# facebookresearch/vsc2022

Measured on AMD Instinct MI355X. Metric: query-videos localized/sec @ 512-d SSCD, higher is better.
Workload: dtype fp32 results; int8 / fp16 MFMA pre-filters; 1 GPU; BASELINE configs[3]: full pipeline incl. score normalisation + TN localisation, 40000 query videos split over 1 GPU(s), 2000000 reference + 2000000 noise frames; query_videos_per_gpu=40000, query_frames_per_gpu=1000000, ref_frames=2000000, dim=512, global_k=48000000, candidates=1000000, pairs_localized=200000, matches=446939, hits=48000000, score_normalisation_in_step=True, parallelism=single GPU

## Files before the change

### vsc2022_amd/csrc/api.hip

```cpp
#include "api_internal.h"

namespace vscmi {

static thread_local std::string g_err;
void set_error(const char* fmt, ...) {
    char buf[1024];
    va_list ap;
    va_start(ap, fmt);
    vsnprintf(buf, sizeof(buf), fmt, ap);
    va_end(ap);
    g_err = buf;
}

bool poison_mode() {
    static const bool on = [] {
        const char* e = getenv("VSC_POISON_ALLOC");
        return e && e[0] == '1';
    }();
    return on;
}

int check_device(int device) {
    int n = 0;
    if (hipGetDeviceCount(&n) != hipSuccess || n <= 0) {
        set_error("no HIP device visible (libvscmi needs an MI355X / gfx950 GPU)");
        return VSC_ERR_NODEVICE;
    }
    if (device < 0 || device >= n) {
        set_error("device %d out of range (have %d)", device, n);
        return VSC_ERR_INVALID;
    }
    hipDeviceProp_t p;
    VSC_HIP(hipGetDeviceProperties(&p, device));
    if (strncmp(p.gcnArchName, "gfx950", 6) != 0) {
        set_error("device %d is %s; libvscmi is built for gfx950 only", device, p.gcnArchName);
        return VSC_ERR_NODEVICE;
    }
    return VSC_OK;
}


int pack_half_any(const float* x, int64_t n, int dim, const HalfImage& h, int64_t r0, int64_t rows_out,
                         hipStream_t stream) {
    if (h.frag)
        return launch_pack_half_frag(x, n, dim, h.rows, h.norms + r0, h.row0 + r0, rows_out, h.dpadh, stream);
    return launch_pack_half(x, n, dim, h.rows + r0 * h.dpadh, h.norms + r0, rows_out, h.dpadh, stream);
}

int pack_into(const float* x, int64_t n, int dim, int mem, float* dst, int64_t rows_out, int dpad,
                     Workspace& ws, hipStream_t stream, const HalfImage& h) {
    if (mem == VSC_MEM_DEVICE || n == 0) {
        VSC_TRY(launch_pack_rows(x, n, dim, dst, rows_out, dpad, stream));
        if (h.rows) VSC_TRY(pack_half_any(x, n, dim, h, 0, h.rows_out, stream));
        return VSC_OK;
    }
    const int64_t chunk_rows = std::max<int64_t>(1, (int64_t)(256ll << 20) / ((int64_t)dim * 4));
    VSC_TRY(ws.stage.reserve((size_t)std::min(chunk_rows, n) * dim * 4));
    for (int64_t r0 = 0; r0 < n; r0 += chunk_rows) {
        const int64_t rows = std::min(chunk_rows, n - r0);
        VSC_HIP(hipMemcpyAsync(ws.stage.p, x + r0 * dim, (size_t)rows * dim * 4, hipMemcpyHostToDevice, stream));
        const bool last = (r0 + rows == n);
        const int64_t out_rows = last ? rows_out - r0 : rows;
        VSC_TRY(launch_pack_rows(ws.stage.as<float>(), rows, dim, dst + r0 * dpad, out_rows, dpad, stream));
        if (h.rows) VSC_TRY(pack_half_any(ws.stage.as<float>(), rows, dim, h, r0, last ? h.rows_out - r0 : rows, stream));
        VSC_HIP(hipStreamSynchronize(stream));
    }
    return VSC_OK;
}

}

int prof_begin(vsc_index* idx, hipEvent_t* stop_out, int cls) {
    *stop_out = nullptr;
    if (!idx->prof) return VSC_OK;
    if (idx->ev_used == idx->ev_pool.size()) {
        hipEvent_t a, b;
        VSC_HIP(hipEventCreate(&a));
        VSC_HIP(hipEventCreate(&b));
        idx->ev_pool.emplace_back(a, b);
        idx->ev_class.push_back(0);
    }
    idx->ev_class[idx->ev_used] = cls;
    auto& e = idx->ev_pool[idx->ev_used++];
    VSC_HIP(hipEventRecord(e.first, idx->stream));
    *stop_out = e.second;
    return VSC_OK;
}
int prof_end(vsc_index* idx, hipEvent_t stop, double work, int cls) {
    if (!stop) return VSC_OK;
    VSC_HIP(hipEventRecord(stop, idx->stream));
    idx->pending_work[cls] += work;
    return VSC_OK;
}
int prof_collect(vsc_index* idx) {
    for (size_t e = 0; e < idx->ev_used; ++e) {
        float ms = 0.0f;
        VSC_HIP(hipEventElapsedTime(&ms, idx->ev_pool[e].first, idx->ev_pool[e].second));
        idx->prof_ms[idx->ev_class[e]] += ms;
        idx->prof_launches[idx->ev_class[e]] += 1;
    }
    for (int c = 0; c < 7; ++c) {
        idx->prof_work[c] += idx->pending_work[c];
        idx->pending_work[c] = 0.0;
    }
    idx->ev_used = 0;
    return VSC_OK;
}


AuxProf g_aux;

struct OptionName { const char* name; const char* env; };
static const OptionName kOptions[] = {
    {"prefilter", "VSC_PREFILTER"}, {"prefilter_density", "VSC_PREFILTER_DENSITY"}, {"f16_kernel", "VSC_F16_KERNEL"},
    {"i8", "VSC_I8"}, {"i8_density", "VSC_I8_DENSITY"}, {"i8_max_rel", "VSC_I8_MAX_REL"}, {"i8_exclude", "VSC_I8_EXCLUDE"},
    {"i8_sort", "VSC_I8_SORT"}, {"i8_center", "VSC_I8_CENTER"}, {"i8_group", "VSC_I8_GROUP"}, {"i8p_order", "VSC_I8P_ORDER"}, {"i8p_slice", "VSC_I8P_SLICE"},
    {"i8p_pair", "VSC_I8P_PAIR"}, {"i8_screen", "VSC_I8_SCREEN"}, {"i8_knn", "VSC_I8_KNN"}, {"knn_step", "VSC_KNN_STEP"},
    {"knn_step_max", "VSC_KNN_STEP_MAX"}, {"knn_step_work", "VSC_KNN_STEP_WORK"}, {"rescore_sort", "VSC_RESCORE_SORT"},
    {"knn_levels", "VSC_KNN_LEVELS"}, {"knn_subset", "VSC_KNN_SUBSET"}, {"knn_s0div", "VSC_KNN_S0DIV"},
    {"knn_s0min", "VSC_KNN_S0MIN"}, {"knn_ratio", "VSC_KNN_RATIO"}, {"knn_nchunk", "VSC_KNN_NCHUNK"}, {"knn_first_tile", "VSC_KNN_FIRST_TILE"},
    {"cand_budget", "VSC_CAND_BUDGET"}, {"debug_i8", "VSC_DEBUG_I8"}, {"debug_screen", "VSC_DEBUG_SCREEN"},
    {"topk_shortcut", "VSC_TOPK_SHORTCUT"}, {"topk_sample", "VSC_TOPK_SAMPLE"}, {"sort_hits", "VSC_SORT_HITS"}, {"density_hint", "VSC_DENSITY_HINT"},
};

static int option_needs_empty(const vsc_index* idx, const char* name) {
    if (idx->ntotal == 0) return VSC_OK;
    set_error("vsc_index_set_option: '%s' decides which images of the reference rows exist and can only be set while "
              "the index is empty", name);
    return VSC_ERR_INVALID;
}

static int apply_option(vsc_index* idx, const char* name, double v) {
    auto is = [&](const char* n) { return strcmp(name, n) == 0; };
    const bool ip = idx->metric == VSC_METRIC_INNER_PRODUCT;
    if (is("prefilter")) {
        const int m = (int)v;
        if (m < 0 || m > 2) goto bad;
        if ((m != 0) != idx->prefilter) VSC_TRY(option_needs_empty(idx, name));
        idx->prefilter = ip && m != 0;
        idx->prefilter_force = idx->prefilter && m == 2;
        if (!idx->prefilter) idx->i8_mode = 0;
        return VSC_OK;
    }
    if (is("i8")) {
        const int m = (int)v;
        if (m < 0 || m > 2) goto bad;
        const int want = (idx->prefilter && idx->dpad8 <= I8P_MAX_DPAD8) ? m : 0;
        if ((want != 0) != (idx->i8_mode != 0)) VSC_TRY(option_needs_empty(idx, name));
        idx->i8_mode = want;
        return VSC_OK;
    }
    if (is("f16_kernel")) {
        const bool frag = !(v != 0.0) && idx->dpadh <= F16P_MAX_DPADH;
        if (frag != idx->frag) VSC_TRY(option_needs_empty(idx, name));
        idx->frag = frag;
        return VSC_OK;
    }
    if (is("i8_exclude")) {
        const bool e = v != 0.0;
        if (e != idx->i8_exclude) VSC_TRY(option_needs_empty(idx, name));
        idx->i8_exclude = e;
        return VSC_OK;
    }
    if (is("i8_center")) {
        const int m = (int)v;
        if (m < 0 || m > 2) goto bad;
        if (m != idx->i8_center) VSC_TRY(option_needs_empty(idx, name));
        idx->i8_center = m;
        return VSC_OK;
    }
    if (is("prefilter_density")) { if (!(v > 0.0)) goto bad; idx->prefilter_density = v; return VSC_OK; }
    if (is("i8_density")) { if (!(v > 0.0)) goto bad; idx->i8_density = v; return VSC_OK; }
    if (is("i8_max_rel")) { if (!(v > 0.0)) goto bad; idx->i8_max_rel = v; return VSC_OK; }
    if (is("i8_sort")) { idx->i8_sort_rows = v != 0.0; return VSC_OK; }
    if (is("i8_group")) { idx->i8_group_shift = std::max(0, std::min(16, (int)v)); return VSC_OK; }
    if (is("i8p_order")) { idx->i8p_order = (int)v == 1 ? 1 : 0; return VSC_OK; }
    if (is("i8p_slice")) { if (v < 0.0) goto bad; idx->i8p_slice = (int)v; return VSC_OK; }
    if (is("i8p_pair")) { idx->i8p_pair = std::max(0, std::min(2, (int)v)); return VSC_OK; }
    if (is("i8_screen")) { idx->i8_screen = v == 1.0; return VSC_OK; }
    if (is("i8_knn")) { idx->knn_i8 = v != 0.0; return VSC_OK; }
    if (is("knn_step")) { idx->knn_step = std::max<int64_t>(0, (int64_t)v) / 256 * 256; return VSC_OK; }
    if (is("knn_step_max")) { idx->knn_step_max = std::max<int64_t>(32768, (int64_t)v); return VSC_OK; }
    if (is("knn_step_work")) { idx->knn_step_work = std::max(0.0, v); return VSC_OK; }
    if (is("rescore_sort")) { idx->rescore_by_ref = v != 0.0; return VSC_OK; }
    if (is("knn_levels")) { idx->knn_two_level = v != 1.0; return VSC_OK; }
    if (is("knn_subset")) { if (!(v > 0.0)) goto bad; idx->knn_subset_factor = v; return VSC_OK; }
    if (is("knn_s0div")) { idx->knn_s0_div = v > 0.0 ? (int)v : 28; return VSC_OK; }
    if (is("knn_s0min")) { idx->knn_s0_min = v >= 64.0 ? (int)v : 1024; return VSC_OK; }
    if (is("knn_ratio")) { idx->knn_ratio = v; return VSC_OK; }
    if (is("knn_nchunk")) { idx->knn_nchunk = (int)v; return VSC_OK; }
    if (is("knn_first_tile")) { idx->knn_first_tile = v != 0.0; return VSC_OK; }
    if (is("cand_budget")) { if (!(v >= 1048576.0)) goto bad; idx->cand_budget = (int64_t)v; return VSC_OK; }
    if (is("debug_i8")) { idx->debug_i8 = v != 0.0; return VSC_OK; }
    if (is("debug_screen")) { idx->debug_screen = v != 0.0; return VSC_OK; }
    if (is("topk_shortcut")) { const int m = (int)v; if (m < 0 || m > 2) goto bad; idx->topk_shortcut = m; return VSC_OK; }
    if (is("topk_sample")) { if (!(v >= 2.0)) goto bad; idx->topk_sample_rows = (int64_t)v; return VSC_OK; }
    if (is("sort_hits")) { idx->sort_hits = v != 0.0; return VSC_OK; }
    if (is("density_hint")) { if (!(v >= 0.0)) goto bad; idx->density_hint = v; return VSC_OK; }
    set_error("vsc_index_set_option: unknown option '%s'", name);
    return VSC_ERR_INVALID;
bad:
    set_error("vsc_index_set_option: value %g is out of range for '%s'", v, name);
    return VSC_ERR_INVALID;
}

static int read_option(const vsc_index* idx, const char* name, double* out) {
    auto is = [&](const char* n) { return strcmp(name, n) == 0; };
    if (is("prefilter")) *out = idx->prefilter ? (idx->prefilter_force ? 2 : 1) : 0;
    else if (is("i8")) *out = idx->i8_mode;
    else if (is("f16_kernel")) *out = idx->frag ? 0 : 1;
    else if (is("i8_exclude")) *out = idx->i8_exclude;
    else if (is("prefilter_density")) *out = idx->prefilter_density;
    else if (is("i8_density")) *out = idx->i8_density;
    else if (is("i8_max_rel")) *out = idx->i8_max_rel;
    else if (is("i8_sort")) *out = idx->i8_sort_rows;
    else if (is("i8_group")) *out = idx->i8_group_shift;
    else if (is("i8p_order")) *out = idx->i8p_order;
    else if (is("i8p_slice")) *out = idx->i8p_slice;
    else if (is("i8p_pair")) *out = idx->i8p_pair;
    else if (is("i8_screen")) *out = idx->i8_screen;
    else if (is("i8_knn")) *out = idx->knn_i8;
    else if (is("knn_step")) *out = (double)idx->knn_step;
    else if (is("knn_step_max")) *out = (double)idx->knn_step_max;
    else if (is("knn_step_work")) *out = idx->knn_step_work;
    else if (is("rescore_sort")) *out = idx->rescore_by_ref;
    else if (is("knn_levels")) *out = idx->knn_two_level ? 0 : 1;
    else if (is("knn_subset")) *out = idx->knn_subset_factor;
    else if (is("knn_s0div")) *out = idx->knn_s0_div;
    else if (is("knn_s0min")) *out = idx->knn_s0_min;
    else if (is("knn_ratio")) *out = idx->knn_ratio;
    else if (is("knn_nchunk")) *out = idx->knn_nchunk;
    else if (is("knn_first_tile")) *out = idx->knn_first_tile;
    else if (is("cand_budget")) *out = (double)idx->cand_budget;
    else if (is("debug_i8")) *out = idx->debug_i8;
    else if (is("debug_screen")) *out = idx->debug_screen;
    else if (is("topk_shortcut")) *out = idx->topk_shortcut;
    else if (is("topk_sample")) *out = (double)idx->topk_sample_rows;
    else if (is("sort_hits")) *out = idx->sort_hits;
    else if (is("density_hint")) *out = idx->density_hint;
    else if (is("last_topk_route")) *out = idx->last_topk_route;
    else if (is("i8_center")) *out = idx->i8_center;
    else if (is("i8_center_on")) *out = idx->i8_mu_on;
    else if (is("i8_center_share")) *out = idx->i8_mu_ratio;
    else if (is("i8_fallbacks")) *out = (double)idx->stat_i8_fallbacks;
    else if (is("codec")) *out = idx->codec;
    else if (is("ref_bytes")) *out = (double)(idx->ref.bytes + idx->refh.bytes + idx->refn.bytes + idx->ref8.bytes + idx->ref8m.bytes);
    else {
        set_error("vsc_index_get_option: unknown option '%s'", name);
        return VSC_ERR_INVALID;
    }
    return VSC_OK;
}

extern "C" {

int vsc_aux_profile(int enable) {
    g_aux.on = enable != 0;
    return VSC_OK;
}
int vsc_aux_profile_read(int cls, double* ms, int64_t* calls, double* bytes, int reset) {
    if (cls < 0 || cls >= AUX_CLASSES) return VSC_ERR_INVALID;
    std::lock_guard<std::mutex> lk(g_aux.mu);
    if (ms) *ms = g_aux.ms[cls];
    if (calls) *calls = g_aux.n[cls];
    if (bytes) *bytes = g_aux.bytes[cls];
    if (reset) { g_aux.ms[cls] = 0.0; g_aux.bytes[cls] = 0.0; g_aux.n[cls] = 0; }
    return VSC_OK;
}

const char* vsc_last_error(void) { return g_err.c_str(); }
int vsc_version(void) { return 100; }

int vsc_device_count(void) {
    int n = 0;
    if (hipGetDeviceCount(&n) != hipSuccess) return 0;
    int ok = 0;
    for (int d = 0; d < n; ++d) {
        hipDeviceProp_t p;
        if (hipGetDeviceProperties(&p, d) == hipSuccess && strncmp(p.gcnArchName, "gfx950", 6) == 0) ++ok;
    }
    return ok;
}

int vsc_index_create(int dim, int metric, int device, vsc_index_t** out) {
    return vsc_index_create_codec(dim, metric, device, VSC_CODEC_FLAT, out);
}

int vsc_index_create_codec(int dim, int metric, int device, int codec, vsc_index_t** out) {
    if (!out || dim <= 0 || (metric != VSC_METRIC_INNER_PRODUCT && metric != VSC_METRIC_L2) ||
        (codec != VSC_CODEC_FLAT && codec != VSC_CODEC_SQFP16)) {
        set_error("vsc_index_create: invalid argument (dim=%d metric=%d codec=%d)", dim, metric, codec);
        return VSC_ERR_INVALID;
    }
    VSC_TRY(check_device(device));
    VSC_HIP(hipSetDevice(device));
    vsc_index* idx = new vsc_index();
    idx->dim = dim;
    idx->codec = codec;
    idx->dpad = round_up(dim, K_PAD);
    idx->dpadh = round_up(dim, 128);
    idx->frag = idx->dpadh <= F16P_MAX_DPADH;
    idx->metric = metric;
    idx->dpad8 = round_up(dim, 256);
    idx->prefilter = metric == VSC_METRIC_INNER_PRODUCT;
    idx->i8_mode = (idx->prefilter && idx->dpad8 <= I8P_MAX_DPAD8) ? 1 : 0;
    for (const OptionName& o : kOptions) {
        const char* v = getenv(o.env);
        if (!v || !v[0]) continue;
        double x = atof(v);
        if (strcmp(o.name, "f16_kernel") == 0) x = v[0] == 'r' ? 1.0 : 0.0;
        if (strcmp(o.name, "debug_i8") == 0 || strcmp(o.name, "debug_screen") == 0) x = 1.0;
        (void)apply_option(idx, o.name, x);
    }
    idx->device = device;
    hipError_t e = hipStreamCreateWithFlags(&idx->own_stream, hipStreamNonBlocking);
    if (e != hipSuccess) {
        set_error("hipStreamCreate failed: %s", hipGetErrorString(e));
        delete idx;
        return VSC_ERR_HIP;
    }
    idx->stream = idx->own_stream;
    int rc = set_thresh_kernel_attrs();
    if (rc != VSC_OK) {
        (void)hipStreamDestroy(idx->own_stream);
        delete idx;
        return rc;
    }
    *out = idx;
    return VSC_OK;
}

int vsc_index_destroy(vsc_index_t* idx) {
    if (!idx) return VSC_OK;
    (void)hipSetDevice(idx->device);
    if (idx->stream == idx->own_stream) (void)hipStreamSynchronize(idx->own_stream);
    else (void)hipDeviceSynchronize();
    idx->ref.release();
    idx->refh.release();
    idx->refn.release();
    idx->ref8.release();
    idx->ref8m.release();
    idx->i8_mu.release();
    for (auto& b : idx->cand) b.release();
    idx->ws.release();
    for (auto& e : idx->ev_pool) {
        (void)hipEventDestroy(e.first);
        (void)hipEventDestroy(e.second);
    }
    (void)hipStreamDestroy(idx->own_stream);
    delete idx;
    return VSC_OK;
}

int vsc_index_set_stream(vsc_index_t* idx, void* hip_stream, int own) {
    if (!idx) {
        set_error("vsc_index_set_stream: invalid argument");
        return VSC_ERR_INVALID;
    }
    VSC_HIP(hipSetDevice(idx->device));
    if (idx->stream == idx->own_stream) VSC_HIP(hipStreamSynchronize(idx->own_stream));
    else (void)hipDeviceSynchronize();
    VSC_TRY(prof_collect(idx));
    idx->stream = own ? idx->own_stream : (hipStream_t)hip_stream;
    return VSC_OK;
}

int vsc_index_set_option(vsc_index_t* idx, const char* name, double value) {
    if (!idx || !name) {
        set_error("vsc_index_set_option: invalid argument");
        return VSC_ERR_INVALID;
    }
    return apply_option(idx, name, value);
}

int vsc_index_get_option(const vsc_index_t* idx, const char* name, double* value) {
    if (!idx || !name || !value) {
        set_error("vsc_index_get_option: invalid argument");
        return VSC_ERR_INVALID;
    }
    return read_option(idx, name, value);
}

int64_t vsc_index_ntotal(const vsc_index_t* idx) { return idx ? idx->ntotal : 0; }
int vsc_index_dim(const vsc_index_t* idx) { return idx ? idx->dim : 0; }
int vsc_index_metric(const vsc_index_t* idx) { return idx ? idx->metric : 0; }

int vsc_index_set_hit_capacity(vsc_index_t* idx, int64_t cap) {
    if (!idx || cap < 0) {
        set_error("vsc_index_set_hit_capacity: invalid argument");
        return VSC_ERR_INVALID;
    }
    idx->hit_cap_user = cap;
    return VSC_OK;
}

int vsc_index_sync(vsc_index_t* idx) {
    if (!idx) return VSC_ERR_INVALID;
    VSC_HIP(hipSetDevice(idx->device));
    VSC_HIP(hipStreamSynchronize(idx->stream));
    return VSC_OK;
}

}

int decode_range(vsc_index* idx, int64_t r0, int64_t rows, float** out) {
    const int64_t rows_out = round_up64(rows, ROW_PAD_REF) + ROW_PAD_REF;
    VSC_TRY(idx->ws.dec.reserve((size_t)rows_out * idx->dpad * sizeof(float)));
    VSC_TRY(launch_decode_rows(idx->refh.as<_Float16>(), idx->dpadh, idx->frag, r0, rows_out,
                               std::min(r0 + rows, round_up64(idx->ntotal, ROW_PAD_REF)), idx->ws.dec.as<float>(), idx->dpad, true,
                               idx->stream));
    *out = idx->ws.dec.as<float>();
    return VSC_OK;
}

int ref_range_count(const vsc_index* idx, int64_t, int64_t rows) {
    return sq16(idx) ? (int)((rows + DEC_CHUNK_ROWS - 1) / DEC_CHUNK_ROWS) : 1;
}
int for_ref_ranges(vsc_index* idx, int64_t r0, int64_t rows, const RefRangeFn& fn) {
    if (!sq16(idx)) return fn(idx->ref.as<float>() + r0 * idx->dpad, r0, rows);
    for (int64_t c0 = r0; c0 < r0 + rows; c0 += DEC_CHUNK_ROWS) {
        const int64_t rc = std::min(DEC_CHUNK_ROWS, r0 + rows - c0);
        float* dec = nullptr;
        VSC_TRY(decode_range(idx, c0, rc, &dec));
        VSC_TRY(fn(dec, c0, rc));
    }
    return VSC_OK;
}

static int i8_upload_centre(vsc_index* idx) {
    if (!idx->i8_mu_on) return VSC_OK;
    std::vector<float> eff(idx->i8_mu_host);
    for (int c = 0; c < idx->i8_ex.n; ++c) eff[(size_t)k_slot(idx->i8_ex.idx[c])] = 0.0f;
    VSC_TRY(idx->i8_mu.reserve((size_t)idx->dpad * sizeof(float)));
    VSC_HIP(hipMemcpyAsync(idx->i8_mu.p, eff.data(), (size_t)idx->dpad * sizeof(float), hipMemcpyHostToDevice, idx->stream));
    VSC_HIP(hipStreamSynchronize(idx->stream));
    idx->i8_mu_ex = idx->i8_ex;
    return VSC_OK;
}

static int i8_decide_centre(vsc_index* idx, int64_t rows) {
    idx->i8_mu_decided = true;
    idx->i8_mu_on = false;
    if (idx->i8_center == 0 || rows <= 0) return VSC_OK;
    const int dpad = idx->dpad;
    VSC_TRY(idx->ws.sort.tmp.reserve((size_t)2 * dpad * sizeof(double)));
    double* d_sum = idx->ws.sort.tmp.as<double>();
    std::vector<double> h((size_t)2 * dpad), part(h.size());
    VSC_TRY(for_ref_ranges(idx, 0, rows, [&](const float* src, int64_t first, int64_t n) -> int {
        std::vector<double>& dst = first == 0 ? h : part;
        VSC_TRY(launch_col_sums(src, n, dpad, d_sum, d_sum + dpad, idx->stream));
        VSC_HIP(hipMemcpyAsync(dst.data(), d_sum, dst.size() * sizeof(double), hipMemcpyDeviceToHost, idx->stream));
        VSC_HIP(hipStreamSynchronize(idx->stream));
        if (first > 0)
            for (size_t e = 0; e < h.size(); ++e) h[e] += part[e];
        return VSC_OK;
    }));
    idx->i8_mu_host.assign((size_t)dpad, 0.0f);
    double mu2 = 0.0, e2 = 0.0;
    bool finite = true;
    for (int k = 0; k < idx->dim; ++k) {
        if (idx->i8_ex.holds(k)) continue;
        const int p = k_slot(k);
        const double m = h[(size_t)p] / (double)rows;
        finite = finite && std::isfinite(m) && std::isfinite(h[(size_t)dpad + p]);
        idx->i8_mu_host[(size_t)p] = (float)m;
        mu2 += m * m;
        e2 += h[(size_t)dpad + p] / (double)rows;
    }
    idx->i8_mu_ratio = e2 > 0.0 ? mu2 / e2 : 0.0;
    if (!finite) return VSC_OK;
    idx->i8_mu_on = idx->i8_center == 2 || idx->i8_mu_ratio >= 0.02;
    if (idx->debug_i8)
        fprintf(stderr, "[vscmi] int8 reference image: mean carries %.4f of the rows' energy over %lld rows -> %s\n", idx->i8_mu_ratio,
                (long long)rows, idx->i8_mu_on ? "centred" : "not centred");
    return i8_upload_centre(idx);
}

static int i8_quantise(vsc_index* idx, int64_t row0, int64_t rows, int64_t count_rows) {
    if (rows <= 0) return VSC_OK;
    if (idx->i8_mu_on) {
        bool same = idx->i8_mu_ex.n == idx->i8_ex.n;
        for (int c = 0; same && c < idx->i8_ex.n; ++c) same = idx->i8_mu_ex.idx[c] == idx->i8_ex.idx[c];
        if (!same) VSC_TRY(i8_upload_centre(idx));
    }
    VSC_TRY(for_ref_ranges(idx, row0, rows, [&](const float* src, int64_t first, int64_t n) -> int {
        return launch_quant_ref_frag(src - first * idx->dpad, idx->dpad, idx->ref8.p, idx->ref8m.as<float4>(), first, n, idx->dpad8,
                                     idx->i8_ex, idx->i8_mu_on ? idx->i8_mu.as<float>() : nullptr, idx->stream);
    }));
    const int64_t real = std::max<int64_t>(0, std::min(row0 + rows, count_rows) - row0);
    VSC_TRY(idx->ws.cnt.reserve(2 * sizeof(double)));
    VSC_TRY(launch_meta_looseness(idx->ref8m.as<float4>() + row0, real, idx->ws.cnt.as<double>(), idx->stream));
    double h2[2] = {0.0, 0.0};
    VSC_HIP(hipMemcpyAsync(h2, idx->ws.cnt.p, sizeof(h2), hipMemcpyDeviceToHost, idx->stream));
    VSC_HIP(hipStreamSynchronize(idx->stream));
    idx->i8_loose_sum += h2[0];
    idx->i8_loose_cnt += h2[1];
    idx->i8_rows = std::max(idx->i8_rows, row0 + rows);
    return VSC_OK;
}

static int i8_after_add(vsc_index* idx, int64_t first_new, int64_t n, int64_t need_rows) {
    const int dpad = idx->dpad;
    VSC_TRY(idx->ws.sort.tmp.reserve((size_t)2 * dpad * sizeof(unsigned)));
    unsigned* d_mn = idx->ws.sort.tmp.as<unsigned>();
    unsigned* d_mx = d_mn + dpad;
    std::vector<unsigned> mn((size_t)dpad), mx((size_t)dpad), pmn((size_t)dpad), pmx((size_t)dpad);
    VSC_TRY(for_ref_ranges(idx, first_new, n, [&](const float* src, int64_t first, int64_t rows) -> int {
        const bool head = first == first_new;
        VSC_TRY(launch_dim_minmax(src, rows, dpad, d_mn, d_mx, idx->stream));
        VSC_HIP(hipMemcpyAsync((head ? mn : pmn).data(), d_mn, (size_t)dpad * sizeof(unsigned), hipMemcpyDeviceToHost, idx->stream));
        VSC_HIP(hipMemcpyAsync((head ? mx : pmx).data(), d_mx, (size_t)dpad * sizeof(unsigned), hipMemcpyDeviceToHost, idx->stream));
        VSC_HIP(hipStreamSynchronize(idx->stream));
        if (!head)
            for (int p = 0; p < dpad; ++p) {
                mn[(size_t)p] = std::min(mn[(size_t)p], pmn[(size_t)p]);
                mx[(size_t)p] = std::max(mx[(size_t)p], pmx[(size_t)p]);
            }
        return VSC_OK;
    }));
    if (idx->cmin_key.empty()) {
        idx->cmin_key.assign((size_t)idx->dim, 0xffffffffu);
        idx->cmax_key.assign((size_t)idx->dim, 0u);
    }
    for (int k = 0; k < idx->dim; ++k) {
        const int p = k_slot(k);
        idx->cmin_key[(size_t)k] = std::min(idx->cmin_key[(size_t)k], mn[(size_t)p]);
        idx->cmax_key[(size_t)k] = std::max(idx->cmax_key[(size_t)k], mx[(size_t)p]);
    }
    std::vector<std::pair<float, int>> cst;
    for (int k = 0; k < idx->dim; ++k)
        if (idx->cmin_key[(size_t)k] == idx->cmax_key[(size_t)k]) {
            const float v = key2f(idx->cmin_key[(size_t)k]);
            if (std::isfinite(v) && v != 0.0f) cst.emplace_back(-std::fabs(v), k);
        }
    std::sort(cst.begin(), cst.end());
    ExcludedDims ex;
    const bool no_ex = !idx->i8_exclude;
    for (size_t c = 0; c < cst.size() && ex.n < I8_MAX_EXCLUDED && !no_ex; ++c) {
        ex.idx[ex.n] = cst[c].second;
        ex.val[ex.n] = key2f(idx->cmin_key[(size_t)cst[c].second]);
        ++ex.n;
    }
    bool same = ex.n == idx->i8_ex.n;
    for (int c = 0; same && c < ex.n; ++c) same = ex.idx[c] == idx->i8_ex.idx[c] && ex.val[c] == idx->i8_ex.val[c];
    idx->i8_ex = ex;
    if (!same && first_new > 0) idx->i8_dirty = true;
    if (!idx->i8_mu_decided && (idx->i8_center != 1 || first_new + n >= 1024)) {
        VSC_TRY(i8_decide_centre(idx, first_new + n));
        if (idx->i8_mu_on && first_new > 0) idx->i8_dirty = true;
    }
    if (idx->i8_dirty) return VSC_OK;
    return i8_quantise(idx, first_new, need_rows - first_new, first_new + n);
}

static int store_rows(vsc_index* idx, const void* x, bool src16, int64_t n, int x_mem, int64_t need_rows) {
    const size_t esz = src16 ? 2 : 4;
    Workspace& ws = idx->ws;
    VSC_TRY(ws.flag.reserve(16));
    int* d_bad = ws.flag.as<int>();
    VSC_HIP(hipMemsetAsync(d_bad, 0, sizeof(int), idx->stream));
    _Float16* image = idx->refh.as<_Float16>();
    float* norms = idx->refn.as<float>();
    const int64_t first = idx->ntotal, rows_out = need_rows - first;
    if (x_mem == VSC_MEM_DEVICE) {
        VSC_TRY(launch_encode_rows(x, src16, n, idx->dim, image, norms + first, first, rows_out, idx->dpadh, idx->frag, d_bad, idx->stream));
    } else {
        const int64_t chunk_rows = std::max<int64_t>(1, (int64_t)(256ll << 20) / ((int64_t)idx->dim * (int64_t)esz));
        VSC_TRY(ws.stage.reserve((size_t)std::min(chunk_rows, n) * idx->dim * esz));
        for (int64_t r0 = 0; r0 < n; r0 += chunk_rows) {
            const int64_t rows = std::min(chunk_rows, n - r0);
            VSC_HIP(hipMemcpyAsync(ws.stage.p, static_cast<const char*>(x) + (size_t)r0 * idx->dim * esz, (size_t)rows * idx->dim * esz,
                                   hipMemcpyHostToDevice, idx->stream));
            const bool last = r0 + rows == n;
            VSC_TRY(launch_encode_rows(ws.stage.p, src16, rows, idx->dim, image, norms + first + r0, first + r0,
                                       last ? rows_out - r0 : rows, idx->dpadh, idx->frag, d_bad, idx->stream));
            VSC_HIP(hipStreamSynchronize(idx->stream));
        }
    }
    int bad = 0;
    VSC_HIP(hipMemcpyAsync(&bad, d_bad, sizeof(int), hipMemcpyDeviceToHost, idx->stream));
    VSC_HIP(hipStreamSynchronize(idx->stream));
    if (bad) {
        VSC_TRY(launch_encode_rows(nullptr, src16, 0, idx->dim, image, norms + first, first, rows_out, idx->dpadh, idx->frag, d_bad, idx->stream));
        VSC_HIP(hipStreamSynchronize(idx->stream));
        set_error("vsc_index_add: a row holds NaN, +-inf or a value beyond +-65504, which the SQfp16 codec cannot store; nothing was added");
        return VSC_ERR_INVALID;
    }
    return VSC_OK;
}

static int pack_f16_rows(vsc_index* idx, const uint16_t* x, int64_t n, int x_mem, float* dst, int64_t rows_out, const HalfImage& h) {
    Workspace& ws = idx->ws;
    const int64_t chunk_rows = std::max<int64_t>(1, (int64_t)(64ll << 20) / ((int64_t)idx->dim * 4));
    VSC_TRY(ws.dec.reserve((size_t)std::min(chunk_rows, n) * idx->dim * 4));
    if (x_mem != VSC_MEM_DEVICE) VSC_TRY(ws.stage.reserve((size_t)std::min(chunk_rows, n) * idx->dim * 2));
    for (int64_t r0 = 0; r0 < n; r0 += chunk_rows) {
        const int64_t rows = std::min(chunk_rows, n - r0);
        const uint16_t* src = x + r0 * idx->dim;
        if (x_mem != VSC_MEM_DEVICE) {
            VSC_HIP(hipMemcpyAsync(ws.stage.p, src, (size_t)rows * idx->dim * 2, hipMemcpyHostToDevice, idx->stream));
            src = ws.stage.as<uint16_t>();
        }
        VSC_TRY(launch_half_to_float(reinterpret_cast<const _Float16*>(src), rows * idx->dim, ws.dec.as<float>(), idx->stream));
        const bool last = r0 + rows == n;
        VSC_TRY(launch_pack_rows(ws.dec.as<float>(), rows, idx->dim, dst + r0 * idx->dpad, last ? rows_out - r0 : rows, idx->dpad, idx->stream));
        if (h.rows) VSC_TRY(pack_half_any(ws.dec.as<float>(), rows, idx->dim, h, r0, last ? h.rows_out - r0 : rows, idx->stream));
        VSC_HIP(hipStreamSynchronize(idx->stream));
    }
    return VSC_OK;
}

static int index_add(vsc_index_t* idx, const void* x, bool src16, int64_t n, int x_mem) {
    if (!idx || n < 0 || (n > 0 && !x)) {
        set_error("vsc_index_add: invalid argument");
        return VSC_ERR_INVALID;
    }
    if (n == 0) return VSC_OK;
    if (idx->ntotal + n >= 0x7fffff00LL) {
        set_error("vsc_index_add: more than 2^31 reference rows");
        return VSC_ERR_INVALID;
    }
    VSC_HIP(hipSetDevice(idx->device));
    const int64_t need_rows = round_up64(idx->ntotal + n, ROW_PAD_REF);
    const bool keep_half = idx->prefilter || sq16(idx);
    if (need_rows > idx->cap_rows) {
        int64_t cap = std::max<int64_t>(need_rows, idx->cap_rows + idx->cap_rows / 2);
        cap = round_up64(cap, ROW_PAD_REF);
        DevBuf nb, nh, nn, n8, n8m;
        if (!sq16(idx)) VSC_TRY(nb.reserve((size_t)cap * idx->dpad * 4));
        if (keep_half) {
            VSC_TRY(nh.reserve((size_t)(cap + F16P_COL_STEP) * idx->dpadh * 2));
            VSC_TRY(nn.reserve((size_t)(cap + F16P_COL_STEP) * 4));
        }
        if (idx->i8_mode) {
            VSC_TRY(n8.reserve((size_t)(cap + F16P_COL_STEP) * idx->dpad8));
            VSC_TRY(n8m.reserve((size_t)(cap + F16P_COL_STEP) * sizeof(float4)));
        }
        if (idx->ntotal > 0) {
            if (!sq16(idx))
                VSC_HIP(hipMemcpyAsync(nb.p, idx->ref.p, (size_t)idx->ntotal * idx->dpad * 4,
                                       hipMemcpyDeviceToDevice, idx->stream));
            if (keep_half) {
                VSC_HIP(hipMemcpyAsync(nh.p, idx->refh.p, (size_t)round_up64(idx->ntotal, 64) * idx->dpadh * 2,
                                       hipMemcpyDeviceToDevice, idx->stream));
                VSC_HIP(hipMemcpyAsync(nn.p, idx->refn.p, (size_t)idx->ntotal * 4, hipMemcpyDeviceToDevice,
                                       idx->stream));
            }
            if (idx->i8_mode) {
                VSC_HIP(hipMemcpyAsync(n8.p, idx->ref8.p, (size_t)round_up64(idx->ntotal, 64) * idx->dpad8,
                                       hipMemcpyDeviceToDevice, idx->stream));
                VSC_HIP(hipMemcpyAsync(n8m.p, idx->ref8m.p, (size_t)idx->ntotal * sizeof(float4), hipMemcpyDeviceToDevice,
                                       idx->stream));
            }
            VSC_HIP(hipStreamSynchronize(idx->stream));
        }
        idx->ref.release();
        idx->refh.release();
        idx->refn.release();
        idx->ref8.release();
        idx->ref8m.release();
        idx->ref = nb;
        idx->refh = nh;
        idx->refn = nn;
        idx->ref8 = n8;
        idx->ref8m = n8m;
        idx->cap_rows = cap;
    }
    if (sq16(idx)) {
        VSC_TRY(store_rows(idx, x, src16, n, x_mem, need_rows));
        idx->ntotal += n;
        return VSC_OK;
    }
    float* dst = idx->ref.as<float>() + idx->ntotal * idx->dpad;
    HalfImage h;
    if (idx->prefilter) {
        h.frag = idx->frag;
        h.row0 = idx->ntotal;
        h.rows = idx->frag ? idx->refh.as<_Float16>() : idx->refh.as<_Float16>() + idx->ntotal * idx->dpadh;
        h.norms = idx->refn.as<float>() + idx->ntotal;
        h.rows_out = need_rows - idx->ntotal;
        h.dpadh = idx->dpadh;
    }
    if (src16) VSC_TRY(pack_f16_rows(idx, static_cast<const uint16_t*>(x), n, x_mem, dst, need_rows - idx->ntotal, h));
    else VSC_TRY(pack_into(static_cast<const float*>(x), n, idx->dim, x_mem, dst, need_rows - idx->ntotal, idx->dpad, idx->ws, idx->stream, h));
    VSC_HIP(hipStreamSynchronize(idx->stream));
    idx->ntotal += n;
    return VSC_OK;
}

extern "C" {

int vsc_index_add(vsc_index_t* idx, const float* x, int64_t n, int x_mem) { return index_add(idx, x, false, n, x_mem); }

int vsc_index_add_f16(vsc_index_t* idx, const uint16_t* x, int64_t n, int x_mem) { return index_add(idx, x, true, n, x_mem); }

int vsc_index_reconstruct(vsc_index_t* idx, int64_t i0, int64_t n, float* out, int out_mem) {
    if (!idx || i0 < 0 || n < 0 || i0 + n > idx->ntotal || (n > 0 && !out)) {
        set_error("vsc_index_reconstruct: invalid argument (rows [%lld, %lld) of %lld)", (long long)i0, (long long)(i0 + n),
                  (long long)(idx ? idx->ntotal : 0));
        return VSC_ERR_INVALID;
    }
    if (n == 0) return VSC_OK;
    VSC_HIP(hipSetDevice(idx->device));
    const int dim = idx->dim;
    for (int64_t c0 = 0; c0 < n; c0 += DEC_CHUNK_ROWS) {
        const int64_t rc = std::min(DEC_CHUNK_ROWS, n - c0);
        float* dst = out + c0 * dim;
        if (out_mem == VSC_MEM_HOST) {
            VSC_TRY(idx->ws.dec.reserve((size_t)rc * dim * sizeof(float)));
            dst = idx->ws.dec.as<float>();
        }
        if (sq16(idx))
            VSC_TRY(launch_decode_rows(idx->refh.as<_Float16>(), idx->dpadh, idx->frag, i0 + c0, rc, idx->ntotal, dst, dim, false, idx->stream));
        else
            VSC_TRY(launch_unpack_rows(idx->ref.as<float>() + (i0 + c0) * idx->dpad, idx->dpad, rc, dim, dst, idx->stream));
        if (out_mem == VSC_MEM_HOST)
            VSC_HIP(hipMemcpyAsync(out + c0 * dim, dst, (size_t)rc * dim * sizeof(float), hipMemcpyDeviceToHost, idx->stream));
        VSC_HIP(hipStreamSynchronize(idx->stream));
    }
    return VSC_OK;
}

}

int i8_prepare(vsc_index* idx) {
    if (!idx->i8_mode) return VSC_OK;
    if (idx->i8_seen < idx->ntotal) {
        const int64_t first_new = idx->i8_seen;
        const int rc = i8_after_add(idx, first_new, idx->ntotal - first_new, round_up64(idx->ntotal, ROW_PAD_REF));
        if (rc != VSC_OK) {
            idx->i8_dirty = true;
            return rc;
        }
        idx->i8_seen = idx->ntotal;
    }
    if (!idx->i8_dirty) return VSC_OK;
    idx->i8_loose_sum = idx->i8_loose_cnt = 0.0;
    VSC_TRY(i8_quantise(idx, 0, round_up64(idx->ntotal, ROW_PAD_REF), idx->ntotal));
    idx->i8_dirty = false;
    return VSC_OK;
}

bool i8_usable(const vsc_index* idx) {
    if (idx->i8_mode == 2) return true;
    if (idx->i8_mode != 1) return false;
    if (idx->i8_loose_cnt <= 0.0) return true;
    return std::sqrt((double)idx->dim) * (idx->i8_loose_sum / idx->i8_loose_cnt) <= idx->i8_max_rel;
}

int pack_queries(vsc_index* idx, const float* q, int64_t nq, int q_mem, float** out, bool with_half) {
    const int64_t rows = round_up64(nq, ROW_PAD) + ROW_PAD;
    VSC_TRY(idx->ws.qbuf.reserve((size_t)rows * idx->dpad * 4));
    HalfImage h;
    if (with_half) {
        h.rows_out = round_up64(nq, ROW_PAD_H) + ROW_PAD_H;
        h.dpadh = idx->dpadh;
        VSC_TRY(idx->ws.qh.reserve((size_t)h.rows_out * idx->dpadh * 2));
        VSC_TRY(idx->ws.qn.reserve((size_t)h.rows_out * 4));
        h.rows = idx->ws.qh.as<_Float16>();
        h.norms = idx->ws.qn.as<float>();
    }
    VSC_TRY(pack_into(q, nq, idx->dim, q_mem, idx->ws.qbuf.as<float>(), rows, idx->dpad, idx->ws, idx->stream, h));
    *out = idx->ws.qbuf.as<float>();
    return VSC_OK;
}

int ensure_hit_buffers(vsc_index* idx, int64_t cap, int64_t ccap, bool need_b) {
    if (ccap < 0) ccap = cap;
    for (int c = 0; c < 3; ++c) {
        VSC_TRY(idx->ws.hA[c].reserve((size_t)cap * 4 + 16));
        if (need_b) VSC_TRY(idx->ws.hB[c].reserve((size_t)cap * 4 + 16));
    }
    if (idx->prefilter) {
        VSC_TRY(idx->ws.ci.reserve((size_t)cand_entries(ccap) * 4));
        VSC_TRY(idx->ws.cj.reserve((size_t)cand_entries(ccap) * 4));
        VSC_TRY(idx->ws.segcnt.reserve(2048 * sizeof(int)));
    }
    VSC_TRY(idx->ws.ctl.reserve(sizeof(SelectCtl)));
    return VSC_OK;
}


extern "C" {

int vsc_index_profile(vsc_index_t* idx, int enable) {
    if (!idx) return VSC_ERR_INVALID;
    idx->prof = enable != 0;
    return VSC_OK;
}

int vsc_index_profile_read_class(vsc_index_t* idx, int cls, double* ms, int64_t* launches, double* work,
                                 int reset) {
    if (!idx || cls < 0 || cls > 6) return VSC_ERR_INVALID;
    if (ms) *ms = idx->prof_ms[cls];
    if (launches) *launches = idx->prof_launches[cls];
    if (work) *work = idx->prof_work[cls];
    if (reset) {
        idx->prof_ms[cls] = 0.0;
        idx->prof_work[cls] = 0.0;
        idx->prof_launches[cls] = 0;
    }
    return VSC_OK;
}

int vsc_index_profile_read(vsc_index_t* idx, double* sim_ms, int64_t* sim_launches, double* sim_flops,
                           int reset) {
    return vsc_index_profile_read_class(idx, 0, sim_ms, sim_launches, sim_flops, reset);
}

int vsc_index_search_stats(vsc_index_t* idx, int64_t* candidates, int64_t* hits) {
    if (!idx) return VSC_ERR_INVALID;
    if (candidates) *candidates = (int64_t)idx->stat_candidates;
    if (hits) *hits = (int64_t)idx->stat_hits;
    return VSC_OK;
}

}
```

### vsc2022_amd/csrc/api_internal.h

```cpp
#pragma once
#include <algorithm>
#include <cmath>
#include <cstdarg>
#include <cstring>
#include <functional>
#include <mutex>
#include <string>
#include <vector>

#include "kernels.h"

namespace vscmi {

int check_device(int device);

struct Workspace {
    DevBuf stage;
    DevBuf qbuf;
    DevBuf hA[3], hB[3];
    DevBuf ctl;
    SortScratch sort;
    DevBuf cnt;
    DevBuf out[4];
    DevBuf parts, partj, mat, maps0, maps1;
    DevBuf qh, qn;
    DevBuf ci, cj, segcnt;
    DevBuf rowthr;
    DevBuf slices;
    DevBuf q8, pstat;
    DevBuf cs[4], cstmp, csn;
    DevBuf tailfill;
    DevBuf rt8c;
    DevBuf rt8d;
    DevBuf rt8, rt8b;
    DevBuf dec, flag, kparts, kpartj;
    DevBuf sample, sk[3], tk[3];
    HitView hits_a() const { return {hA[0].as<int32_t>(), hA[1].as<int32_t>(), hA[2].as<float>()}; }
    HitView hits_b() const { return {hB[0].as<int32_t>(), hB[1].as<int32_t>(), hB[2].as<float>()}; }
    HitView hits_out() const { return {out[0].as<int32_t>(), out[1].as<int32_t>(), out[2].as<float>()}; }
    void release() {
        stage.release(); qbuf.release(); sample.release();
        dec.release(); flag.release(); kparts.release(); kpartj.release();
        for (auto& b : sk) b.release();
        for (auto& b : tk) b.release();
        qh.release(); qn.release(); ci.release(); cj.release(); segcnt.release(); rowthr.release(); slices.release();
        q8.release(); pstat.release(); rt8.release(); rt8b.release(); rt8c.release(); rt8d.release(); tailfill.release();
        for (auto& b : cs) b.release();
        cstmp.release(); csn.release();
        for (auto& b : hA) b.release();
        for (auto& b : hB) b.release();
        ctl.release(); sort.release(); cnt.release();
        for (auto& b : out) b.release();
        parts.release(); partj.release(); mat.release(); maps0.release(); maps1.release();
    }
};

struct HalfImage {
    _Float16* rows = nullptr;
    float* norms = nullptr;
    int64_t rows_out = 0;
    int dpadh = 0;
    bool frag = false;
    int64_t row0 = 0;
};

int pack_half_any(const float* x, int64_t n, int dim, const HalfImage& h, int64_t r0, int64_t rows_out, hipStream_t stream);
int pack_into(const float* x, int64_t n, int dim, int mem, float* dst, int64_t rows_out, int dpad, Workspace& ws,
              hipStream_t stream, const HalfImage& h = HalfImage());

}

using namespace vscmi;

struct vsc_index {
    int dim = 0, dpad = 0, metric = 0, device = 0;
    int codec = VSC_CODEC_FLAT;
    int64_t ntotal = 0, cap_rows = 0;
    DevBuf ref;
    DevBuf refh, refn;
    int dpadh = 0;
    bool frag = false;
    DevBuf ref8, ref8m;
    int dpad8 = 0, i8_mode = 0;
    double i8_density = 5e-4;
    double i8_loose_sum = 0.0, i8_loose_cnt = 0.0, i8_max_rel = 0.35;
    std::vector<unsigned> cmin_key, cmax_key;
    ExcludedDims i8_ex;
    int i8_center = 1;
    bool i8_mu_decided = false, i8_mu_on = false;
    double i8_mu_ratio = 0.0;
    std::vector<float> i8_mu_host;
    DevBuf i8_mu;
    ExcludedDims i8_mu_ex;
    bool i8_dirty = false;
    int64_t i8_rows = 0;
    int64_t i8_seen = 0;
    unsigned long long stat_i8_fallbacks = 0;
    bool i8_exclude = true;
    int i8p_order = 1;
    int i8p_pair = 1;
    int64_t knn_step = 0;
    double knn_step_work = 64.0;
    int64_t knn_step_max = 262144;
    int i8p_slice = 0;
    bool i8_sort_rows = true;
    int i8_group_shift = 9;
    bool rescore_by_ref = true;
    bool i8_screen = false;
    bool knn_i8 = true;
    bool knn_two_level = true;
    double knn_subset_factor = 300.0;
    int knn_s0_div = 28;
    int knn_s0_min = 1024;
    double knn_ratio = 0.0;
    bool knn_first_tile = true;
    int knn_nchunk = 0;
    bool debug_i8 = false, debug_screen = false;
    int topk_shortcut = 0;
    double density_hint = 0.0;
    bool sort_hits = true;
    int64_t topk_sample_rows = 4096;
    int last_topk_route = 0;
    bool prefilter = false, prefilter_force = false;
    double prefilter_density = 0.05;
    unsigned long long stat_candidates = 0, stat_hits = 0;
    DevBuf cand[3];
    hipStream_t stream = nullptr;
    hipStream_t own_stream = nullptr;
    int64_t cand_budget = (int64_t)1 << 28;
    Workspace ws;
    int64_t hit_cap_user = 0;
    int64_t hit_cap_learned = 0;
    bool prof = false;
    std::vector<std::pair<hipEvent_t, hipEvent_t>> ev_pool;
    std::vector<int> ev_class;
    size_t ev_used = 0;
    double prof_ms[7] = {}, prof_work[7] = {}, pending_work[7] = {};
    int64_t prof_launches[7] = {};
};

int prof_begin(vsc_index* idx, hipEvent_t* stop_out, int cls = 0);
int prof_end(vsc_index* idx, hipEvent_t stop, double work, int cls = 0);
int prof_collect(vsc_index* idx);

constexpr int AUX_CLASSES = 4;
struct AuxProf {
    bool on = false;
    std::mutex mu;
    double ms[AUX_CLASSES] = {}, bytes[AUX_CLASSES] = {};
    int64_t n[AUX_CLASSES] = {};
};
extern AuxProf g_aux;
struct AuxTimer {
    hipEvent_t a = nullptr, b = nullptr;
    int cls = 0;
    double bytes = 0.0;
    void begin(int c, hipStream_t s) {
        cls = c;
        if (!g_aux.on) return;
        if (hipEventCreate(&a) != hipSuccess || hipEventCreate(&b) != hipSuccess) { a = b = nullptr; return; }
        (void)hipEventRecord(a, s);
    }
    void end(double by, hipStream_t s) {
        if (a && b) { (void)hipEventRecord(b, s); bytes += by; }
    }
    void collect() {
        if (!a || !b) return;
        float t = 0.0f;
        if (hipEventElapsedTime(&t, a, b) == hipSuccess) {
            std::lock_guard<std::mutex> lk(g_aux.mu);
            g_aux.ms[cls] += t;
            g_aux.bytes[cls] += bytes;
            g_aux.n[cls] += 1;
        }
        (void)hipEventDestroy(a);
        (void)hipEventDestroy(b);
        a = b = nullptr;
    }
};

constexpr int64_t DEC_CHUNK_ROWS = 65536;
inline bool sq16(const vsc_index* idx) { return idx->codec == VSC_CODEC_SQFP16; }
int decode_range(vsc_index* idx, int64_t r0, int64_t rows, float** out);
using RefRangeFn = std::function<int(const float* packed_rows, int64_t first_row, int64_t n_rows)>;
int for_ref_ranges(vsc_index* idx, int64_t r0, int64_t rows, const RefRangeFn& fn);
int ref_range_count(const vsc_index* idx, int64_t r0, int64_t rows);

int i8_prepare(vsc_index* idx);
bool i8_usable(const vsc_index* idx);
int pack_queries(vsc_index* idx, const float* q, int64_t nq, int q_mem, float** out, bool with_half = false);
inline int64_t cand_entries(int64_t ccap) { return 4 * ccap + 2048 * 128; }
int ensure_hit_buffers(vsc_index* idx, int64_t cap, int64_t ccap = -1, bool need_b = true);

int enqueue_f16(vsc_index* idx, const float* qpacked, int64_t i0, int64_t i1, int64_t cap, const float* row_thr,
                int64_t ccap = -1, int64_t nr_limit = -1, bool use_i8 = false, int64_t nr_begin = 0);
int init_ctl(vsc_index* idx, float radius_score_space);
```

### vsc2022_amd/csrc/api_search.hip

```cpp
#include "api_internal.h"

struct F16Batch {
    const float* qpacked;
    int64_t i0;
    int nq;
    const float* row_thr;
    int64_t nr_begin, nr_end;
    int64_t nrefs() const { return nr_end - nr_begin; }
};

struct F16Bound { float c1, c2, c3; };
static F16Bound f16_bound(int dpadh) {
    const double D = (double)dpadh;
    return {(float)(ldexp(1.0, -10) + ldexp(1.0, -22) + (2.0 * D + D / 16.0 + 16.0) * ldexp(1.0, -23)),
            (float)(ldexp(1.0, -25) * 1.001 * sqrt(D)), (float)(D * ldexp(1.0, -50))};
}

static int cand_list_plan(vsc_index* idx, int64_t ccap, int grid, CandList& l) {
    SelectCtl* ctl = idx->ws.ctl.as<SelectCtl>();
    l.i = idx->ws.ci.as<int32_t>();
    l.j = idx->ws.cj.as<int32_t>();
    l.n_seg = grid * 8;
    l.seg_cap = (int)std::min<int64_t>(ccap / l.n_seg, 0x7fffffff);
    l.seg_count = idx->ws.segcnt.as<int>();
    l.tail_base = (int64_t)l.seg_cap * l.n_seg;
    l.tail_cap = cand_entries(ccap) - l.tail_base;
    l.tail_shift = tail_chunk_shift_for(l.tail_cap, l.n_seg);
    VSC_TRY(idx->ws.tailfill.reserve((size_t)((l.tail_cap >> l.tail_shift) + 2) * sizeof(int)));
    l.tail_fill = idx->ws.tailfill.as<int>();
    l.tail_count = &ctl->n_tail;
    l.overflow = &ctl->overflow;
    return VSC_OK;
}


static int prefilter_f16_ring(vsc_index* idx, const F16Batch& b, int64_t ccap, const F16Bound& fb, CandList& cl, hipEvent_t* stop) {
    SimF16Args f;
    f.Q = idx->ws.qh.as<_Float16>() + b.i0 * idx->dpadh;
    f.R = idx->refh.as<_Float16>() + b.nr_begin * idx->dpadh;
    f.qn = idx->ws.qn.as<float>() + b.i0;
    f.rn = idx->refn.as<float>() + b.nr_begin;
    f.dpadh = idx->dpadh;
    f.nq = b.nq;
    f.i0 = (int)b.i0;
    f.nr = (int)b.nrefs();
    f.tq = (b.nq + 255) / 256;
    f.tr = (int)((b.nrefs() + 255) / 256);
    f.c1 = fb.c1; f.c2 = fb.c2; f.c3 = fb.c3;
    f.radius = &idx->ws.ctl.as<SelectCtl>()->radius;
    f.row_thr = b.row_thr ? b.row_thr + b.i0 : nullptr;
    VSC_TRY(cand_list_plan(idx, ccap, sim_f16_grid(f.tq, f.tr), cl));
    f.list = cl;
    VSC_TRY(prof_begin(idx, stop, 1));
    return launch_sim_f16(f, idx->stream);
}

static int prefilter_f16_panel(vsc_index* idx, const F16Batch& b, int64_t ccap, const F16Bound& fb, CandList& cl, hipEvent_t* stop) {
    SimF16PArgs f;
    int grid = 0;
    sim_f16p_plan(b.nq, b.nrefs(), &f.npanel, &f.nsteps, &f.slice, &grid);
    VSC_TRY(idx->ws.slices.reserve((size_t)f.npanel * sizeof(int)));
    f.Q = idx->ws.qh.as<_Float16>() + b.i0 * idx->dpadh;
    f.Rf = static_cast<const char*>(idx->refh.p) + b.nr_begin * idx->dpadh * 2;
    f.qn = idx->ws.qn.as<float>() + b.i0;
    f.rn = idx->refn.as<float>() + b.nr_begin;
    f.dpadh = idx->dpadh;
    f.nq = b.nq;
    f.i0 = (int)b.i0;
    f.nr = (int)b.nrefs();
    f.next_slice = idx->ws.slices.as<int>();
    f.c1 = fb.c1; f.c2 = fb.c2; f.c3 = fb.c3;
    f.radius = &idx->ws.ctl.as<SelectCtl>()->radius;
    f.row_thr = b.row_thr ? b.row_thr + b.i0 : nullptr;
    VSC_TRY(cand_list_plan(idx, ccap, grid, cl));
    f.list = cl;
    VSC_TRY(prof_begin(idx, stop, 1));
    return launch_sim_f16p(f, grid, idx->stream);
}

static int i8_preamble(vsc_index* idx, const F16Batch& b, int npanel_q, const int32_t** perm_out, float** rt_pos_out) {
    SelectCtl* ctl = idx->ws.ctl.as<SelectCtl>();
    Workspace& ws = idx->ws;
    const float* q = b.qpacked + b.i0 * idx->dpad;
    const int nqb = b.nq;
    const int32_t* perm = nullptr;
    float* rt_pos = nullptr;
    const float* thr_src = b.row_thr ? b.row_thr + b.i0 : nullptr;
    if (idx->i8_ex.n > 0 || idx->i8_mu_on) {
        VSC_TRY(ws.rt8b.reserve((size_t)nqb * sizeof(float)));
        const float *cen = nullptr, *cmag = nullptr;
        if (idx->i8_mu_on) {
            VSC_TRY(ws.rt8d.reserve((size_t)2 * nqb * sizeof(float)));
            VSC_TRY(launch_row_center(q, idx->dpad, nqb, idx->i8_mu.as<float>(), ws.rt8d.as<float>(), ws.rt8d.as<float>() + nqb,
                                      idx->stream));
            cen = ws.rt8d.as<float>();
            cmag = cen + nqb;
        }
        VSC_TRY(launch_row_bias_thresholds(q, idx->dpad, nqb, thr_src, &ctl->radius, idx->i8_ex, cen, cmag, ws.rt8b.as<float>(),
                                           idx->stream));
        thr_src = ws.rt8b.as<float>();
    }
    const bool sort_rows = idx->i8_sort_rows;
    if (thr_src) {
        VSC_TRY(ws.rt8.reserve((size_t)npanel_q * F16P_PANEL_ROWS * sizeof(float)));
        rt_pos = ws.rt8.as<float>();
    }
    if (thr_src && sort_rows) {
        if (idx->i8_group_shift > 0 && !b.row_thr && nqb >= (4 << idx->i8_group_shift)) {
            VSC_TRY(ws.rt8c.reserve((size_t)nqb * sizeof(float)));
            VSC_TRY(launch_row_absmax(q, idx->dpad, nqb, idx->i8_ex, ws.rt8c.as<float>(), idx->stream));
            VSC_TRY(sort_rows_by_threshold_then_scale(thr_src, ws.rt8c.as<float>(), nqb, idx->i8_group_shift, ws.sort, &perm,
                                                      idx->stream));
        } else {
            VSC_TRY(sort_rows_by_threshold(thr_src, nqb, ws.sort, &perm, idx->stream));
        }
    } else if (!thr_src && sort_rows && nqb >= 2 * F16P_PANEL_ROWS) {
        VSC_TRY(ws.rt8b.reserve((size_t)nqb * sizeof(float)));
        VSC_TRY(launch_row_absmax(q, idx->dpad, nqb, idx->i8_ex, ws.rt8b.as<float>(), idx->stream));
        VSC_TRY(sort_rows_by_threshold(ws.rt8b.as<float>(), nqb, ws.sort, &perm, idx->stream));
    }
    VSC_TRY(launch_quant_query_panels(q, idx->dpad, nqb, npanel_q, ws.q8.p, idx->dpad8, ws.pstat.as<float4>(), perm, thr_src,
                                      rt_pos, idx->i8_ex, idx->stream));
    *perm_out = perm;
    *rt_pos_out = rt_pos;
    return VSC_OK;
}

static int prefilter_i8(vsc_index* idx, const F16Batch& b, int64_t ccap, CandList& cl, const int32_t** perm, hipEvent_t* stop) {
    SimI8PArgs f;
    int grid = 0;
    sim_f16p_plan(b.nq, b.nrefs(), &f.npanel, &f.nsteps, &f.slice, &grid);
    {
        const int slice_env = idx->i8p_slice;
        f.order = idx->i8p_order;
        if (f.order == 1) f.slice = std::max(1, std::min(f.nsteps, slice_env > 0 ? slice_env : 32));
        else if (slice_env > 0) f.slice = std::max(1, std::min(f.nsteps, slice_env));
    }
    f.pair = idx->i8p_pair && sim_i8p_pairs(idx->dpad8, f.npanel, f.nsteps, f.slice, idx->i8p_pair == 2) ? 1 : 0;
    const int npanel_q = f.pair ? (f.npanel + 1) & ~1 : f.npanel;
    VSC_TRY(idx->ws.slices.reserve(((size_t)f.npanel + 1) * sizeof(int)));
    VSC_TRY(idx->ws.q8.reserve((size_t)npanel_q * F16P_PANEL_ROWS * idx->dpad8));
    VSC_TRY(idx->ws.pstat.reserve((size_t)npanel_q * sizeof(float4)));
    hipEvent_t prep_stop;
    VSC_TRY(prof_begin(idx, &prep_stop, 6));
    float* rt_pos = nullptr;
    VSC_TRY(i8_preamble(idx, b, npanel_q, perm, &rt_pos));
    f.Q = idx->ws.q8.p;
    f.pstat = idx->ws.pstat.as<float4>();
    f.Rf = static_cast<const char*>(idx->ref8.p) + b.nr_begin * idx->dpad8;
    f.rmeta = idx->ref8m.as<float4>() + b.nr_begin;
    f.dpad8 = idx->dpad8;
    f.nq = b.nq;
    f.i0 = (int)b.i0;
    f.nr = (int)b.nrefs();
    f.next_slice = idx->ws.slices.as<int>();
    f.c_acc = (float)(((double)idx->dpad + 2.0) * ldexp(1.0, -23));
    f.radius = &idx->ws.ctl.as<SelectCtl>()->radius;
    f.row_thr = rt_pos;
    VSC_TRY(cand_list_plan(idx, ccap, grid, cl));
    f.list = cl;
    VSC_TRY(prof_end(idx, prep_stop, 0.0, 6));
    VSC_TRY(prof_begin(idx, stop, 5));
    return launch_sim_i8p(f, grid, idx->stream);
}

static int exact_stage(vsc_index* idx, const F16Batch& b, int64_t cap, const CandList& cl, const int32_t* perm,
                       const F16Bound& fb, bool from_i8) {
    SelectCtl* ctl = idx->ws.ctl.as<SelectCtl>();
    Workspace& ws = idx->ws;
    const HitView kept = ws.hits_a();
    RescoreArgs r;
    r.Q = b.qpacked;
    r.R = idx->ref.as<float>();
    r.dpad = idx->dpad;
    r.list = cl;
    r.perm = perm;
    r.perm_i0 = (int)b.i0;
    r.n_cand_total = &ctl->n_cand_total;
    r.radius = &ctl->radius;
    r.out_i = kept.i;
    r.out_j = kept.j;
    r.out_s = kept.s;
    r.counter = &ctl->n;
    r.cap = cap;
    r.row_thr = b.row_thr;
    r.j0 = (int)b.nr_begin;
    if (sq16(idx)) {
        r.R = nullptr;
        r.Rh = idx->refh.as<_Float16>();
        r.dpadh = idx->dpadh;
        r.rsrc = idx->frag ? 2 : 1;
    }
    if (!idx->rescore_by_ref) return launch_rescore(r, idx->stream);
    VSC_TRY(ws.csn.reserve(3 * sizeof(unsigned long long)));
    unsigned long long* csn = ws.csn.as<unsigned long long>();
    const int n_chunks_max = (int)std::min<long long>((cl.tail_cap >> cl.tail_shift) + 1, 1 << 20);
    VSC_TRY(launch_cand_count(r, n_chunks_max, csn + 2, idx->stream));
    unsigned long long n_c = 0;
    VSC_HIP(hipMemcpyAsync(&n_c, csn + 2, sizeof(n_c), hipMemcpyDeviceToHost, idx->stream));
    VSC_HIP(hipStreamSynchronize(idx->stream));
    const size_t cap_e = (size_t)(n_c + n_c / 4 + 4096);
    for (auto& buf : ws.cs)
        if (buf.bytes < (size_t)(n_c + 1) * sizeof(uint32_t)) VSC_TRY(buf.reserve(cap_e * sizeof(uint32_t)));
    uint32_t* cs[4] = {ws.cs[0].as<uint32_t>(), ws.cs[1].as<uint32_t>(), ws.cs[2].as<uint32_t>(), ws.cs[3].as<uint32_t>()};
    VSC_TRY(launch_cand_compact(r, n_chunks_max, cs[0], cs[2], csn, idx->stream));
    const uint32_t *sj = nullptr, *si = nullptr;
    VSC_TRY(sort_candidates_by_ref(cs[0], cs[1], cs[2], cs[3], (int64_t)n_c, b.nr_end, ws.cstmp, &sj, &si, idx->stream));
    if (!(from_i8 && idx->i8_screen && n_c > 0)) return launch_rescore_dense(r, sj, si, (long long)n_c, idx->stream);
    ScreenArgs sa;
    sa.Qh = ws.qh.as<_Float16>();
    sa.qn = ws.qn.as<float>();
    sa.Rh = idx->refh.as<_Float16>();
    sa.rn = idx->refn.as<float>();
    sa.dpadh = idx->dpadh;
    sa.frag = idx->frag ? 1 : 0;
    sa.c1 = fb.c1; sa.c2 = fb.c2; sa.c3 = fb.c3;
    sa.radius = &ctl->radius;
    sa.row_thr = b.row_thr;
    sa.sj = sj;
    sa.si = si;
    sa.n = (long long)n_c;
    sa.out_j = sj == cs[0] ? cs[1] : cs[0];
    sa.out_i = si == cs[2] ? cs[3] : cs[2];
    sa.n_out = csn + 1;
    sa.n_cand_total = &ctl->n_cand_total;
    sa.overflow = &ctl->overflow;
    VSC_TRY(launch_f16_screen(sa, idx->stream));
    VSC_TRY(launch_rescore_dense(r, sa.out_j, sa.out_i, (long long)n_c, idx->stream, sa.n_out));
    if (idx->debug_screen) {
        unsigned long long n_s = 0;
        VSC_HIP(hipMemcpyAsync(&n_s, sa.n_out, sizeof(n_s), hipMemcpyDeviceToHost, idx->stream));
        VSC_HIP(hipStreamSynchronize(idx->stream));
        fprintf(stderr, "[vscmi] fp16 screen: %llu of %llu int8 candidates left (rows %d)\n", n_s, n_c, b.nq);
    }
    return VSC_OK;
}

int enqueue_f16(vsc_index* idx, const float* qpacked, int64_t i0, int64_t i1, int64_t cap,
                const float* row_thr, int64_t ccap, int64_t nr_limit, bool use_i8, int64_t nr_begin) {
    if (ccap < 0) ccap = cap;
    const int64_t nr_end = nr_limit >= 0 ? std::min<int64_t>(nr_limit, idx->ntotal) : idx->ntotal;
    if (nr_begin < 0 || nr_begin % 64 != 0 || nr_begin > nr_end) {
        set_error("enqueue_f16: reference range [%lld, %lld) does not start on a 64-row tile", (long long)nr_begin, (long long)nr_end);
        return VSC_ERR_INVALID;
    }
    const F16Batch b{qpacked, i0, (int)(i1 - i0), row_thr, nr_begin, nr_end};
    const F16Bound fb = f16_bound(idx->dpadh);
    const bool i8 = use_i8 && idx->i8_mode;
    CandList cl;
    const int32_t* perm = nullptr;
    hipEvent_t stop;
    if (i8) VSC_TRY(prefilter_i8(idx, b, ccap, cl, &perm, &stop));
    else if (idx->frag) VSC_TRY(prefilter_f16_panel(idx, b, ccap, fb, cl, &stop));
    else VSC_TRY(prefilter_f16_ring(idx, b, ccap, fb, cl, &stop));
    VSC_TRY(prof_end(idx, stop, 2.0 * (double)b.nq * (double)b.nrefs() * (double)idx->dim, i8 ? 5 : 1));
    VSC_TRY(prof_begin(idx, &stop, 2));
    VSC_TRY(exact_stage(idx, b, cap, cl, perm, fb, i8));
    return prof_end(idx, stop, 0.0, 2);
}

static int enqueue_batch(vsc_index* idx, const float* qpacked, int64_t i0, int64_t i1, int64_t cap,
                         bool use_f16 = false, bool use_i8 = false) {
    SelectCtl* ctl = idx->ws.ctl.as<SelectCtl>();
    const int nqb = (int)(i1 - i0);
    const HitView kept = idx->ws.hits_a();
    if (use_f16) return enqueue_f16(idx, qpacked, i0, i1, cap, nullptr, -1, -1, use_i8);
    if (idx->metric == VSC_METRIC_INNER_PRODUCT) {
        SimThreshArgs a;
        a.Q = qpacked + i0 * idx->dpad;
        a.dpad = idx->dpad;
        a.nq = nqb;
        a.i0 = (int)i0;
        a.tq = (nqb + 127) / 128;
        a.radius = &ctl->radius;
        a.out_i = kept.i;
        a.out_j = kept.j;
        a.out_s = kept.s;
        a.counter = &ctl->n;
        a.cap = cap;
        a.overflow = &ctl->overflow;
        return for_ref_ranges(idx, 0, idx->ntotal, [&](const float* rows, int64_t j0, int64_t n) -> int {
            unsigned long long* mark = nullptr;
            if (j0 > 0) {
                VSC_TRY(idx->ws.flag.reserve(16));
                mark = idx->ws.flag.as<unsigned long long>() + 1;
                VSC_TRY(launch_hits_mark(&ctl->n, mark, idx->stream));
            }
            a.R = rows;
            a.nr = (int)n;
            a.tr = (int)((n + 127) / 128);
            hipEvent_t stop;
            VSC_TRY(prof_begin(idx, &stop));
            VSC_TRY(launch_sim_thresh(a, idx->stream));
            VSC_TRY(prof_end(idx, stop, 2.0 * (double)nqb * (double)n * (double)idx->dim));
            if (j0 > 0) VSC_TRY(launch_hits_add_offset(a.out_j, mark, &ctl->n, cap, (int)j0, idx->stream));
            return VSC_OK;
        });
    }
    const int64_t nr = idx->ntotal;
    const int64_t chunk = std::max<int64_t>(1, std::min<int64_t>(nqb, (int64_t)(1ll << 28) / std::max<int64_t>(nr, 1)));
    VSC_TRY(idx->ws.mat.reserve((size_t)chunk * nr * 4));
    for (int64_t r0 = i0; r0 < i1; r0 += chunk) {
        const int rows = (int)std::min(chunk, i1 - r0);
        ScoreMatArgs m{qpacked + r0 * idx->dpad, idx->ref.as<float>(), idx->dpad, idx->dim, rows, (int)nr,
                       idx->metric, idx->ws.mat.as<float>()};
        if (sq16(idx)) VSC_TRY(launch_score_matrix_h16(m, idx->refh.as<_Float16>(), idx->dpadh, idx->frag, idx->stream));
        else VSC_TRY(launch_score_matrix(m, idx->stream));
        MatThreshArgs t{idx->ws.mat.as<float>(), rows, (int)nr, (int)r0, &ctl->radius, kept.i, kept.j, kept.s,
                        &ctl->n, cap, &ctl->overflow};
        VSC_TRY(launch_matrix_thresh(t, idx->stream));
    }
    return VSC_OK;
}

int init_ctl(vsc_index* idx, float radius_score_space) {
    return launch_ctl_init(idx->ws.ctl.as<SelectCtl>(), radius_score_space, idx->stream);
}


static int global_topk_impl(vsc_index_t* idx, const float* q, int64_t nq, int q_mem, int64_t K, bool seeded,
                            float radius0, int32_t* out_i, int32_t* out_j, float* out_s, int64_t cap_out, int out_mem,
                            int64_t* n_out, float* final_radius) {
    if (!idx || nq < 0 || K < 0 || !n_out || (nq > 0 && !q)) {
        set_error("vsc_index_global_topk: invalid argument");
        return VSC_ERR_INVALID;
    }
    *n_out = 0;
    const bool ip = idx->metric == VSC_METRIC_INNER_PRODUCT;
    if (final_radius) *final_radius = ip ? -1e10f : 1e10f;
    if (nq == 0 || idx->ntotal == 0) return VSC_OK;
    VSC_HIP(hipSetDevice(idx->device));
    float* qp = nullptr;
    VSC_TRY(pack_queries(idx, q, nq, q_mem, &qp, idx->prefilter));
    VSC_TRY(i8_prepare(idx));
    const int64_t cap_max = nq * idx->ntotal + 1024;
    int64_t cap = idx->hit_cap_user;
    if (cap <= 0) cap = std::max(std::max<int64_t>(32 * idx->ntotal, 2 * K) + 2 * K + 1024, idx->hit_cap_learned);
    cap = std::min<int64_t>(cap, cap_max);
    SelectCtl h;
    bool allow_i8 = i8_usable(idx);
    for (;;) {
        bool used_i8 = false;
        VSC_TRY(ensure_hit_buffers(idx, cap));
        VSC_TRY(init_ctl(idx, seeded ? (ip ? radius0 : -radius0) : -1e10f));
        SelectCtl* ctl = idx->ws.ctl.as<SelectCtl>();
        int64_t bs = seeded ? 32768 : 32, i0 = 0;
        while (i0 < nq) {
            const int64_t i1 = std::min(nq, i0 + bs);
            const double seen = seeded ? (double)nq : (double)i0;
            const double dens = idx->density_hint > 0.0 ? idx->density_hint
                                                         : (seen > 0 ? (double)K / (seen * (double)idx->ntotal) : 1.0);
            const bool f16 = idx->prefilter_force || (idx->prefilter && (seen > 0 || idx->density_hint > 0.0) && dens < idx->prefilter_density);
            const bool i8 = f16 && allow_i8 && (idx->i8_mode == 2 || dens < idx->i8_density);
            used_i8 |= i8;
            VSC_TRY(enqueue_batch(idx, qp, i0, i1, cap, f16, i8));
            if (i1 < nq) {
                hipEvent_t stop;
                VSC_TRY(prof_begin(idx, &stop, 3));
                VSC_TRY(enqueue_rethreshold(ctl, idx->ws.hits_a(), idx->ws.hits_b(), (unsigned long long)K, idx->stream));
                VSC_TRY(prof_end(idx, stop, 0.0, 3));
            }
            if (!seeded && bs < 20000) bs *= 2;
            i0 = i1;
        }
        VSC_HIP(hipMemcpyAsync(&h, ctl, sizeof(h), hipMemcpyDeviceToHost, idx->stream));
        VSC_HIP(hipStreamSynchronize(idx->stream));
        if (!h.overflow && h.n > 2ull * (unsigned long long)K) {
            hipEvent_t stop;
            VSC_TRY(prof_begin(idx, &stop, 3));
            VSC_TRY(enqueue_rethreshold(ctl, idx->ws.hits_a(), idx->ws.hits_b(), (unsigned long long)K, idx->stream));
            VSC_TRY(prof_end(idx, stop, 0.0, 3));
            VSC_HIP(hipMemcpyAsync(&h, ctl, sizeof(h), hipMemcpyDeviceToHost, idx->stream));
            VSC_HIP(hipStreamSynchronize(idx->stream));
        }
        VSC_TRY(prof_collect(idx));
        idx->stat_candidates = h.n_cand_total;
        if (!h.overflow) break;
        if (used_i8 && (h.overflow & 2) && idx->i8_mode != 2) {
            allow_i8 = false;
            idx->stat_i8_fallbacks += 1;
            if (idx->debug_i8)
                fprintf(stderr, "[vscmi] int8 batches overflowed the candidate list (cap %lld, candidates so far %llu, tail %llu, "
                        "kept %llu): fp16 pre-filter for this search\n", (long long)cap, h.n_cand_total, h.n_tail, h.n);
            continue;
        }
        if (idx->hit_cap_user > 0 || cap >= cap_max) {
            set_error("global_topk: kept-hit buffer (%lld entries) overflowed; raise it with "
                      "vsc_index_set_hit_capacity", (long long)cap);
            return VSC_ERR_OVERFLOW;
        }
        cap = std::min<int64_t>(cap * 4, cap_max);
        idx->hit_cap_learned = cap;
    }
    if (final_radius) *final_radius = ip ? h.radius : -h.radius;
    const int64_t n = (int64_t)h.n;
    const int64_t m = std::min(n, K);
    if (m > cap_out) {
        *n_out = m;
        set_error("global_topk: output capacity %lld < %lld", (long long)cap_out, (long long)m);
        return VSC_ERR_CAPACITY;
    }
    HitView d{out_i, out_j, out_s};
    if (out_mem == VSC_MEM_HOST) {
        for (int c = 0; c < 3; ++c) VSC_TRY(idx->ws.out[c].reserve((size_t)std::max<int64_t>(m, 1) * 4));
        d = idx->ws.hits_out();
    }
    int64_t mm = 0;
    hipEvent_t sort_stop;
    VSC_TRY(prof_begin(idx, &sort_stop, 4));
    if (idx->sort_hits || !ip) {
        VSC_TRY(sort_hits_topk(idx->ws.hits_a(), n, K, nq, idx->ntotal, idx->ws.sort, d, ip ? 0 : 1, &mm, idx->stream));
    } else {
        mm = m;
        if (mm > 0) {
            VSC_HIP(hipMemcpyAsync(d.i, idx->ws.hA[0].p, (size_t)mm * 4, hipMemcpyDeviceToDevice, idx->stream));
            VSC_HIP(hipMemcpyAsync(d.j, idx->ws.hA[1].p, (size_t)mm * 4, hipMemcpyDeviceToDevice, idx->stream));
            VSC_HIP(hipMemcpyAsync(d.s, idx->ws.hA[2].p, (size_t)mm * 4, hipMemcpyDeviceToDevice, idx->stream));
        }
    }
    VSC_TRY(prof_end(idx, sort_stop, 12.0 * (double)n, 4));
    if (out_mem == VSC_MEM_HOST && mm > 0) {
        VSC_HIP(hipMemcpyAsync(out_i, d.i, (size_t)mm * 4, hipMemcpyDeviceToHost, idx->stream));
        VSC_HIP(hipMemcpyAsync(out_j, d.j, (size_t)mm * 4, hipMemcpyDeviceToHost, idx->stream));
        VSC_HIP(hipMemcpyAsync(out_s, d.s, (size_t)mm * 4, hipMemcpyDeviceToHost, idx->stream));
    }
    VSC_HIP(hipStreamSynchronize(idx->stream));
    VSC_TRY(prof_collect(idx));
    *n_out = mm;
    return VSC_OK;
}


static int global_topk_proven(vsc_index_t* idx, const float* q, int64_t nq, int q_mem, int64_t K, int32_t* out_i,
                              int32_t* out_j, float* out_s, int64_t cap_out, int out_mem, int64_t* n_out,
                              float* final_radius, bool* done) {
    *done = false;
    const int64_t nr = idx->ntotal;
    const bool force = idx->topk_shortcut == 2;
    if (idx->metric != VSC_METRIC_INNER_PRODUCT || idx->hit_cap_user > 0 || K < 1 || nq < 4 || nr < 1) return VSC_OK;
    const double pairs = (double)nq * (double)nr;
    if ((double)K + 1.0 > (force ? pairs - 1.0 : 0.25 * pairs) || cap_out < K) return VSC_OK;
    if (!force && (nq < 65536 || pairs < 4e10 || nq < 16 * idx->topk_sample_rows)) return VSC_OK;
    VSC_HIP(hipSetDevice(idx->device));
    Workspace& ws = idx->ws;
    const int64_t stride = std::max<int64_t>(2, nq / std::max<int64_t>(2, std::min(idx->topk_sample_rows, nq / 2)));
    const int64_t ns = (nq + stride - 1) / stride;
    VSC_TRY(ws.sample.reserve((size_t)ns * idx->dim * sizeof(float)));
    VSC_HIP(hipMemcpy2DAsync(ws.sample.p, (size_t)idx->dim * sizeof(float), q, (size_t)stride * idx->dim * sizeof(float),
                             (size_t)idx->dim * sizeof(float), (size_t)ns, q_mem == VSC_MEM_HOST ? hipMemcpyHostToDevice : hipMemcpyDeviceToDevice,
                             idx->stream));
    const double share = (double)ns / (double)nq;
    const double x = (double)K * share;
    const int64_t k_tot = std::max<int64_t>(1, (int64_t)std::ceil(1.25 * x + 4.0 * std::sqrt(x) + 8.0));
    const int64_t k_s = (int64_t)std::min((double)ns * (double)nr, std::ceil(2.0 * x + 8.0 * std::sqrt(x)) + 1024.0);
    for (auto& b : ws.sk) VSC_TRY(b.reserve((size_t)std::max<int64_t>(k_s, 1) * 4));
    int64_t n_s = 0;
    float r_s = -1e10f;
    int rc = global_topk_impl(idx, ws.sample.as<float>(), ns, VSC_MEM_DEVICE, k_s, false, 0.0f, ws.sk[0].as<int32_t>(),
                              ws.sk[1].as<int32_t>(), ws.sk[2].as<float>(), k_s, VSC_MEM_DEVICE, &n_s, &r_s);
    if (rc == VSC_ERR_OVERFLOW || rc == VSC_ERR_CAPACITY) return VSC_OK;
    VSC_TRY(rc);
    const unsigned long long cand_sample = idx->stat_candidates;
    float seed = -1e10f;
    if (n_s >= k_tot) {
        float tau = 0.0f;
        VSC_HIP(hipMemcpyAsync(&tau, ws.sk[2].as<float>() + (k_tot - 1), sizeof(float), hipMemcpyDeviceToHost, idx->stream));
        VSC_HIP(hipStreamSynchronize(idx->stream));
        if (tau == tau && std::fabs(tau) < 1e10f) seed = std::nextafterf(tau, -INFINITY);
    } else if (r_s == r_s && std::fabs(r_s) < 1e10f) {
        seed = r_s;
    }
    for (auto& b : ws.tk) VSC_TRY(b.reserve((size_t)(K + 1) * 4));
    int64_t n2 = 0;
    float r2 = -1e10f;
    rc = global_topk_impl(idx, q, nq, q_mem, K + 1, true, seed, ws.tk[0].as<int32_t>(), ws.tk[1].as<int32_t>(),
                          ws.tk[2].as<float>(), K + 1, VSC_MEM_DEVICE, &n2, &r2);
    idx->stat_candidates += cand_sample;
    idx->last_topk_route = 2;
    if (rc == VSC_ERR_OVERFLOW || rc == VSC_ERR_CAPACITY) return VSC_OK;
    VSC_TRY(rc);
    if (idx->debug_i8)
        fprintf(stderr, "[vscmi] proven top-K route: %lld sample rows (stride %lld), %lld sample hits, seed %.9g (the %lld-th best); "
                "steady run: %lld hits, radius %.9g (K = %lld)\n", (long long)ns, (long long)stride, (long long)n_s, (double)seed,
                (long long)k_tot, (long long)n2, (double)r2, (long long)K);
    if (n2 < K + 1) return VSC_OK;
    float cut[2] = {0.0f, 0.0f};
    VSC_HIP(hipMemcpyAsync(cut, ws.tk[2].as<float>() + (K - 1), 2 * sizeof(float), hipMemcpyDeviceToHost, idx->stream));
    VSC_HIP(hipStreamSynchronize(idx->stream));
    if (idx->debug_i8) fprintf(stderr, "[vscmi] proven top-K route: s_K = %.9g, s_(K+1) = %.9g\n", (double)cut[0], (double)cut[1]);
    if (!(cut[0] > cut[1])) return VSC_OK;
    const hipMemcpyKind kind = out_mem == VSC_MEM_HOST ? hipMemcpyDeviceToHost : hipMemcpyDeviceToDevice;
    VSC_HIP(hipMemcpyAsync(out_i, ws.tk[0].p, (size_t)K * 4, kind, idx->stream));
    VSC_HIP(hipMemcpyAsync(out_j, ws.tk[1].p, (size_t)K * 4, kind, idx->stream));
    VSC_HIP(hipMemcpyAsync(out_s, ws.tk[2].p, (size_t)K * 4, kind, idx->stream));
    VSC_HIP(hipStreamSynchronize(idx->stream));
    *n_out = K;
    if (final_radius) *final_radius = r2;
    idx->last_topk_route = 1;
    *done = true;
    return VSC_OK;
}

extern "C" {

int vsc_index_global_topk(vsc_index_t* idx, const float* q, int64_t nq, int q_mem, int64_t K,
                          int32_t* out_i, int32_t* out_j, float* out_s, int64_t cap_out, int out_mem,
                          int64_t* n_out, float* final_radius) {
    if (idx) idx->last_topk_route = 0;
    if (idx && idx->topk_shortcut && nq > 0 && q && n_out && K >= 0 && out_i && out_j && out_s) {
        bool done = false;
        VSC_TRY(global_topk_proven(idx, q, nq, q_mem, K, out_i, out_j, out_s, cap_out, out_mem, n_out, final_radius, &done));
        if (done) return VSC_OK;
    }
    return global_topk_impl(idx, q, nq, q_mem, K, false, 0.0f, out_i, out_j, out_s, cap_out, out_mem, n_out, final_radius);
}

int vsc_index_global_topk_seeded(vsc_index_t* idx, const float* q, int64_t nq, int q_mem, int64_t K, float radius0,
                                 int32_t* out_i, int32_t* out_j, float* out_s, int64_t cap_out, int out_mem,
                                 int64_t* n_out, float* final_radius) {
    if (!(radius0 == radius0) || std::fabs(radius0) > 1e10f) {
        set_error("vsc_index_global_topk_seeded: the seed radius must be a finite score (got %g)", (double)radius0);
        return VSC_ERR_INVALID;
    }
    return global_topk_impl(idx, q, nq, q_mem, K, true, radius0, out_i, out_j, out_s, cap_out, out_mem, n_out, final_radius);
}

int vsc_index_candidates(vsc_index_t* idx, const float* q, int64_t nq, int q_mem, int64_t K,
                         const int32_t* row2q, const int32_t* row2r, int32_t* out_q, int32_t* out_r,
                         float* out_s, int64_t cap_out, int64_t* n_pairs, int64_t* n_hits) {
    if (!idx || nq < 0 || K < 0 || !n_pairs || (nq > 0 && (!q || !row2q || !row2r))) {
        set_error("vsc_index_candidates: invalid argument");
        return VSC_ERR_INVALID;
    }
    *n_pairs = 0;
    if (n_hits) *n_hits = 0;
    if (idx->metric != VSC_METRIC_INNER_PRODUCT) {
        set_error("vsc_index_candidates: max aggregation needs a larger-is-better metric (inner product)");
        return VSC_ERR_INVALID;
    }
    if (nq == 0 || idx->ntotal == 0 || K == 0) return VSC_OK;
    VSC_HIP(hipSetDevice(idx->device));
    const int64_t hcap = std::max<int64_t>(1, std::min<int64_t>(K, nq * idx->ntotal));
    for (int c = 0; c < 3; ++c) VSC_TRY(idx->cand[c].reserve((size_t)hcap * 4));
    int64_t n = 0;
    float radius = 0.0f;
    VSC_TRY(vsc_index_global_topk(idx, q, nq, q_mem, K, idx->cand[0].as<int32_t>(), idx->cand[1].as<int32_t>(),
                                  idx->cand[2].as<float>(), hcap, VSC_MEM_DEVICE, &n, &radius));
    if (n_hits) *n_hits = n;
    if (n == 0) return VSC_OK;
    Workspace& ws = idx->ws;
    VSC_TRY(ws.maps0.reserve((size_t)nq * 4));
    VSC_TRY(ws.maps1.reserve((size_t)idx->ntotal * 4));
    VSC_HIP(hipMemcpyAsync(ws.maps0.p, row2q, (size_t)nq * 4, hipMemcpyHostToDevice, idx->stream));
    VSC_HIP(hipMemcpyAsync(ws.maps1.p, row2r, (size_t)idx->ntotal * 4, hipMemcpyHostToDevice, idx->stream));
    for (int c = 0; c < 3; ++c) VSC_TRY(ws.out[c].reserve((size_t)n * 4));
    VSC_TRY(ws.out[3].reserve((size_t)n * 8));
    int64_t np = 0;
    VSC_TRY(pair_max_device(idx->cand[0].as<int32_t>(), idx->cand[1].as<int32_t>(), idx->cand[2].as<float>(), n,
                            ws.maps0.as<int32_t>(), ws.maps1.as<int32_t>(), nq, idx->ntotal, ws.sort,
                            ws.cnt, ws.out[0].as<int32_t>(), ws.out[1].as<int32_t>(), ws.out[2].as<float>(),
                            ws.out[3].as<int64_t>(), n, &np, idx->stream));
    *n_pairs = np;
    if (np > cap_out) {
        set_error("vsc_index_candidates: output capacity %lld < %lld pairs", (long long)cap_out, (long long)np);
        return VSC_ERR_CAPACITY;
    }
    if (np > 0) {
        VSC_HIP(hipMemcpyAsync(out_q, ws.out[0].p, (size_t)np * 4, hipMemcpyDeviceToHost, idx->stream));
        VSC_HIP(hipMemcpyAsync(out_r, ws.out[1].p, (size_t)np * 4, hipMemcpyDeviceToHost, idx->stream));
        VSC_HIP(hipMemcpyAsync(out_s, ws.out[2].p, (size_t)np * 4, hipMemcpyDeviceToHost, idx->stream));
    }
    VSC_HIP(hipStreamSynchronize(idx->stream));
    return VSC_OK;
}

int vsc_index_range_search(vsc_index_t* idx, const float* q, int64_t nq, int q_mem, float radius,
                           int64_t* lims, float* D, int64_t* I, int64_t cap_out, int64_t* n_out) {
    if (!idx || nq < 0 || !lims || !n_out || (nq > 0 && !q)) {
        set_error("vsc_index_range_search: invalid argument");
        return VSC_ERR_INVALID;
    }
    *n_out = 0;
    for (int64_t i = 0; i <= nq; ++i) lims[i] = 0;
    if (nq == 0 || idx->ntotal == 0) return VSC_OK;
    const bool ip = idx->metric == VSC_METRIC_INNER_PRODUCT;
    VSC_HIP(hipSetDevice(idx->device));
    float* qp = nullptr;
    VSC_TRY(pack_queries(idx, q, nq, q_mem, &qp, idx->prefilter));
    VSC_TRY(i8_prepare(idx));
    int64_t cap = idx->hit_cap_user > 0 ? idx->hit_cap_user : std::min<int64_t>(nq * idx->ntotal, (int64_t)1 << 28);
    cap = std::max<int64_t>(cap, 1024);
    VSC_TRY(ensure_hit_buffers(idx, cap));
    VSC_TRY(init_ctl(idx, ip ? radius : -radius));
    SelectCtl* ctl = idx->ws.ctl.as<SelectCtl>();
    const int64_t step = 32768;
    for (int64_t i0 = 0; i0 < nq; i0 += step)
        VSC_TRY(enqueue_batch(idx, qp, i0, std::min(nq, i0 + step), cap, idx->prefilter, idx->i8_mode == 2));
    SelectCtl h;
    VSC_HIP(hipMemcpyAsync(&h, ctl, sizeof(h), hipMemcpyDeviceToHost, idx->stream));
    VSC_HIP(hipStreamSynchronize(idx->stream));
    VSC_TRY(prof_collect(idx));
    if (h.overflow) {
        set_error("range_search: more than %lld hits; raise vsc_index_set_hit_capacity", (long long)cap);
        return VSC_ERR_OVERFLOW;
    }
    const int64_t n = (int64_t)h.n;
    *n_out = n;
    if (n == 0) return VSC_OK;
    VSC_TRY(sort_hits_rowcol(idx->ws.hits_a(), n, idx->ws.sort, idx->ws.hits_b(), ip ? 0 : 1, idx->stream));
    std::vector<int32_t> hi((size_t)n);
    VSC_HIP(hipMemcpyAsync(hi.data(), idx->ws.hB[0].p, (size_t)n * 4, hipMemcpyDeviceToHost, idx->stream));
    VSC_HIP(hipStreamSynchronize(idx->stream));
    for (int64_t x = 0; x < n; ++x) lims[hi[(size_t)x] + 1] += 1;
    for (int64_t i = 0; i < nq; ++i) lims[i + 1] += lims[i];
    if (!D || !I || cap_out < n) {
        if (D || I) {
            set_error("range_search: output capacity %lld < %lld", (long long)cap_out, (long long)n);
            return VSC_ERR_CAPACITY;
        }
        return VSC_OK;
    }
    std::vector<int32_t> hj((size_t)n);
    VSC_HIP(hipMemcpyAsync(hj.data(), idx->ws.hB[1].p, (size_t)n * 4, hipMemcpyDeviceToHost, idx->stream));
    VSC_HIP(hipMemcpyAsync(D, idx->ws.hB[2].p, (size_t)n * 4, hipMemcpyDeviceToHost, idx->stream));
    VSC_HIP(hipStreamSynchronize(idx->stream));
    for (int64_t x = 0; x < n; ++x) I[x] = hj[(size_t)x];
    return VSC_OK;
}


}
```

### vsc2022_amd/csrc/kernels.h

```cpp
#pragma once
#include "vscmi_common.h"
#include "cand_list.h"

namespace vscmi {

struct SortScratch {
    DevBuf w0, w1, w2, w3, tmp;
    void release() { w0.release(); w1.release(); w2.release(); w3.release(); tmp.release(); }
};
struct HitView { int32_t* i; int32_t* j; float* s; };
struct ConstHitView {
    const int32_t* i; const int32_t* j; const float* s;
    ConstHitView(const int32_t* i_, const int32_t* j_, const float* s_) : i(i_), j(j_), s(s_) {}
    ConstHitView(const HitView& v) : i(v.i), j(v.j), s(v.s) {}
};

struct SimThreshArgs {
    const float* Q; const float* R; int dpad; int nq; int i0; int nr; int tq; int tr;
    const float* radius; int32_t* out_i; int32_t* out_j; float* out_s;
    unsigned long long* counter; long long cap; int* overflow;
};
struct SimF16Args {
    const _Float16* Q; const _Float16* R;
    const float* qn; const float* rn;
    int dpadh; int nq; int i0; int nr; int tq; int tr;
    float c1, c2, c3;
    const float* radius;
    const float* row_thr;
    CandList list;
};
constexpr int F16P_PANEL_ROWS = 128;
constexpr int F16P_COL_STEP = 512;
constexpr int F16P_MAX_DPADH = 512;
template <typename Row>
__host__ __device__ __forceinline__ int64_t frag_piece(Row row, int piece, int dpadh) {
    return (int64_t)(row >> 6) * (dpadh / 16) * 128 + ((row >> 5) & 1) * 64 + (row & 31) + (piece >> 1) * 128 + (piece & 1) * 32;
}
struct SimF16PArgs {
    const _Float16* Q; const void* Rf;
    const float* qn; const float* rn;
    int dpadh; int nq; int i0; int nr;
    int npanel; int nsteps; int slice;
    int* next_slice;
    float c1, c2, c3;
    const float* radius; const float* row_thr;
    CandList list;
};
constexpr int I8P_MAX_DPAD8 = 1024;
constexpr int I8_MAX_EXCLUDED = 8;
struct ExcludedDims {
    int n = 0;
    int idx[I8_MAX_EXCLUDED] = {};
    float val[I8_MAX_EXCLUDED] = {};
    __host__ __device__ bool holds(int k) const {
        bool h = false;
#pragma unroll
        for (int c = 0; c < I8_MAX_EXCLUDED; ++c) h |= c < n && idx[c] == k;
        return h;
    }
};
struct SimI8PArgs {
    const void* Q; const float4* pstat;
    const void* Rf; const float4* rmeta;
    int dpad8; int nq; int i0; int nr;
    int npanel; int nsteps; int slice;
    int* next_slice;
    int order;
    int pair;
    float c_acc;
    const float* radius; const float* row_thr;
    CandList list;
};
struct RescoreArgs {
    const float* Q; const float* R; int dpad;
    CandList list;
    const int32_t* perm; int perm_i0;
    unsigned long long* n_cand_total;
    const float* radius; int32_t* out_i; int32_t* out_j; float* out_s;
    unsigned long long* counter; long long cap;
    const float* row_thr;
    int j0 = 0;
    const _Float16* Rh = nullptr; int dpadh = 0; int rsrc = 0;
};
struct ScreenArgs {
    const _Float16* Qh; const float* qn;
    const _Float16* Rh; const float* rn;
    int dpadh; int frag;
    float c1, c2, c3;
    const float* radius; const float* row_thr;
    const uint32_t* sj; const uint32_t* si; long long n;
    uint32_t* out_j; uint32_t* out_i; unsigned long long* n_out;
    unsigned long long* n_cand_total;
    const int* overflow;
};
struct SimKnnArgs {
    const float* Q; const float* R; int dpad; int nq; int nr; int tq; int tr; int nchunk; int k;
    float* part_s; int32_t* part_j;
    int no_first_tile_select;
};
struct KnnMergeArgs {
    const float* part_s; const int32_t* part_j; int nq; int nchunk; int k; float* out_s; int64_t* out_j; int l2;
};
struct ScoreMatArgs { const float* Q; const float* R; int dpad; int dim; int nq; int nr; int metric; float* S; };
struct MatThreshArgs {
    const float* S; int nq; int nr; int i0; const float* radius; int32_t* out_i; int32_t* out_j; float* out_s;
    unsigned long long* counter; long long cap; int* overflow;
};
struct MatKnnArgs { const float* S; int nq; int nr; int k; float* part_s; int32_t* part_j; };
struct SelectCtl {
    unsigned long long n; unsigned long long n_tmp; float radius; int overflow; int active;
    unsigned int prefix; unsigned int prefix_mask; unsigned long long rank; unsigned int hist[256];
    unsigned long long n_rethreshold;
    unsigned long long n_cand_total;
    unsigned long long n_tail;
};
struct TnPairArgs {
    const float* qfeat; const float* rfeat; const int64_t* q_off; const int64_t* r_off; int dpad;
    const int32_t* pair_q; const int32_t* pair_r; const int32_t* work; int n_work; vsc_tn_params prm;
    float bias; int max_lq; int lds_tile_floats; float* slab; int64_t slab_floats;
    int32_t* out_nbox; int32_t* out_boxes; float* out_boxmax;
    const float* sims_in; const int64_t* sims_off; const int32_t* sims_lq; const int32_t* sims_lr;
    char* state; int64_t state_bytes;
    const _Float16* rfeat_h;
};
struct TnSimsArgs {
    const float* qfeat; const float* rfeat; int64_t qrow0, rrow0; int lq, lr, dpad; float bias; float* out;
    const _Float16* rfeat_h;
};

struct AlignArgs {
    const float* qfeat; const float* rfeat; const int64_t* q_off; const int64_t* r_off; int dpad;
    const int32_t* pair_q; const int32_t* pair_r; const int32_t* work; int n_work; vsc_align_params prm;
    float bias;
    int32_t* out_nbox; int32_t* out_boxes; float* out_boxmax; int32_t* out_status;
    const float* sims_in; const int64_t* sims_off; const int32_t* sims_lq; const int32_t* sims_lr;
    const _Float16* rfeat_h;
};
struct MatchRowsArgs {
    const int32_t* pair_q; const int32_t* pair_r; int64_t n_pairs;
    const int32_t* nbox; const int32_t* boxes; const float* boxmax;
    const int64_t* q_off; const int64_t* r_off; int64_t n_qvid, n_rvid;
    const double* q_ts; const double* r_ts;
    int32_t* pair_off;
    int64_t* tile_off;
    int64_t* ctl;
    int32_t* out_pair; int32_t* out_box; float* out_score; double* out_times;
};
struct MetricScratch {
    DevBuf buf[24];
};
struct MetricIn {
    const int32_t* gt_pair; const double* gt_times; int64_t n_gt;
    const int32_t* gt_first; int64_t n_gt_pairs;
    const int32_t* pred_pair; const double* pred_score; const double* pred_times; int64_t n_pred;
    int64_t n_pairs;
};
struct MetricOut {
    double* scores; double* sums; int64_t cap;
    int64_t n_groups;
    double* gt_len;
    int64_t stats[8];
};
struct AlignLayout { size_t f64, runs, tile, kept, u16, bytes, total; };
__host__ __device__ inline AlignLayout align_layout(int method, int lq, int lr, bool tile_in_lds) {
    const size_t cells = (size_t)lq * lr, edge = (size_t)lq + lr;
    const bool dtw = method == VSC_ALIGN_DTW;
    AlignLayout L;
    size_t off = 0;
    L.f64 = off;
    off += dtw ? 3 * ((size_t)(lq < lr ? lq : lr) + 1) * 8 : cells * 8;
    L.runs = off;
    off += dtw ? (edge / 2 + 1) * 16 : (size_t)VSC_TN_MAX_BOXES * 16;
    L.tile = off;
    off += tile_in_lds ? cells * 4 : 0;
    L.kept = off;
    off += (size_t)VSC_TN_MAX_BOXES * 16;
    L.u16 = off;
    off += dtw ? 0 : cells * 2;
    L.bytes = off;
    off += dtw ? cells + edge : edge;
    L.total = (off + 15) & ~(size_t)15;
    return L;
}
constexpr size_t ALIGN_LDS_MAX = 150 * 1024;
static_assert(14 * (size_t)VSC_ALIGN_MAX_CELLS + (VSC_ALIGN_MAX_CELLS + 1) + 3072 <= ALIGN_LDS_MAX, "DP state of the largest pair");
static_assert(5 * (size_t)VSC_ALIGN_MAX_CELLS + 9 * (VSC_ALIGN_MAX_CELLS + 1) + 3072 <= ALIGN_LDS_MAX, "DTW state of the largest pair");
static_assert(VSC_ALIGN_MAX_CELLS < 32768, "frame indices are kept in 16 bits");

int launch_sim_thresh(const SimThreshArgs&, hipStream_t);
int launch_sim_f16(const SimF16Args&, hipStream_t);
int sim_f16_grid(int tq, int tr);
int launch_rescore(const RescoreArgs&, hipStream_t);
int launch_cand_count(const RescoreArgs&, int, unsigned long long*, hipStream_t);
int launch_cand_compact(const RescoreArgs&, int, uint32_t*, uint32_t*, unsigned long long*, hipStream_t);
int launch_rescore_dense(const RescoreArgs&, const uint32_t*, const uint32_t*, long long, hipStream_t,
                         const unsigned long long* n_dev = nullptr);
int launch_f16_screen(const ScreenArgs&, hipStream_t);
int sort_candidates_by_ref(uint32_t*, uint32_t*, uint32_t*, uint32_t*, int64_t, int64_t, DevBuf&, const uint32_t**,
                           const uint32_t**, hipStream_t);
void sim_f16p_plan(int64_t nq, int64_t nr, int* npanel, int* nsteps, int* slice, int* grid);
int launch_sim_f16p(const SimF16PArgs&, int grid, hipStream_t);
int launch_sim_i8p(const SimI8PArgs&, int grid, hipStream_t);
bool sim_i8p_pairs(int dpad8, int npanel, int nsteps, int slice, bool force);
int launch_quant_ref_frag(const float*, int, void*, float4*, int64_t, int64_t, int, const ExcludedDims&, const float*, hipStream_t);
int launch_col_sums(const float*, int64_t, int, double*, double*, hipStream_t);
int launch_row_center(const float*, int, int, const float*, float*, float*, hipStream_t);
int launch_dim_minmax(const float*, int64_t, int, unsigned*, unsigned*, hipStream_t);
int launch_meta_looseness(const float4*, int64_t, double*, hipStream_t);
int launch_quant_query_panels(const float*, int, int, int, void*, int, float4*, const int32_t*, const float*, float*,
                              const ExcludedDims&, hipStream_t);
int launch_row_absmax(const float*, int, int, const ExcludedDims&, float*, hipStream_t);
int launch_row_bias_thresholds(const float*, int, int, const float*, const float*, const ExcludedDims&, const float*, const float*, float*,
                               hipStream_t);
int sort_rows_by_threshold(const float*, int64_t, SortScratch&, const int32_t**, hipStream_t);
int argsort_scores_desc(const float*, int64_t, SortScratch&, const int32_t**, hipStream_t);
int launch_ctl_init(SelectCtl*, float, hipStream_t);
int launch_filter_hits(ConstHitView, long long, float, HitView, unsigned long long*, hipStream_t);
int launch_score_hist(const float*, long long, const long long*, int, long long*, hipStream_t);
int launch_score_pick(const long long*, long long*, int, hipStream_t);
int launch_merge_topk(const float*, const long long*, long long, int, int, float*, long long*, hipStream_t);
int sort_rows_by_threshold_then_scale(const float*, const float*, int64_t, int, SortScratch&, const int32_t**, hipStream_t);
int launch_pack_half_frag(const float*, int64_t, int, _Float16*, float*, int64_t, int64_t, int, hipStream_t);
int launch_pack_half(const float*, int64_t, int, _Float16*, float*, int64_t, int, hipStream_t);
int launch_sim_knn(const SimKnnArgs&, hipStream_t);
int launch_knn_merge(const KnnMergeArgs&, hipStream_t);
int knn_from_hits(ConstHitView, int64_t, int64_t, int, SortScratch&, float*, int64_t*, hipStream_t);
int launch_knn_row_thr(const float*, int64_t, int, float*, int64_t, hipStream_t);
int launch_knn_seed_hits(const float*, const int64_t*, int64_t, int, HitView, unsigned long long*, hipStream_t);
int launch_score_matrix(const ScoreMatArgs&, hipStream_t);
int launch_matrix_thresh(const MatThreshArgs&, hipStream_t);
int launch_matrix_knn(const MatKnnArgs&, hipStream_t);
int set_thresh_kernel_attrs();
int enqueue_rethreshold(SelectCtl*, HitView, HitView, unsigned long long, hipStream_t);
int sort_hits_topk(ConstHitView, int64_t, int64_t, int64_t, int64_t, SortScratch&, HitView, int, int64_t*, hipStream_t);
int sort_hits_rowcol(ConstHitView, int64_t, SortScratch&, HitView, int, hipStream_t);
int pair_max_device(const int32_t*, const int32_t*, const float*, int64_t, const int32_t*, const int32_t*, int64_t, int64_t,
                    SortScratch&, DevBuf&, int32_t*, int32_t*, float*, int64_t*, int64_t, int64_t*, hipStream_t);
int launch_pack_rows(const float*, int64_t, int, float*, int64_t, int, hipStream_t);
int launch_row_normalize(const float*, int64_t, int, float*, hipStream_t);
size_t tn_state_bytes_host(int, int, int, int idx_bytes = 2);
int launch_tn_pairs(const TnPairArgs&, size_t, hipStream_t);
int launch_tn_sims(const TnSimsArgs&, hipStream_t);
int launch_align_pairs(const AlignArgs&, size_t, hipStream_t);
int64_t match_rows_tiles(int64_t n_pairs);
int launch_match_rows_scan(const MatchRowsArgs&, hipStream_t);
int launch_match_rows_emit(const MatchRowsArgs&, hipStream_t);
int match_metric_device(const MetricIn&, MetricScratch&, MetricOut&, hipStream_t);
int launch_encode_rows(const void*, bool, int64_t, int, _Float16*, float*, int64_t, int64_t, int, bool, int*, hipStream_t);
int launch_decode_rows(const _Float16*, int, bool, int64_t, int64_t, int64_t, float*, int, bool, hipStream_t);
int launch_unpack_rows(const float*, int, int64_t, int, float*, hipStream_t);
int launch_half_to_float(const _Float16*, int64_t, float*, hipStream_t);
int launch_score_matrix_h16(const ScoreMatArgs&, const _Float16*, int, bool, hipStream_t);
int launch_hits_mark(const unsigned long long*, unsigned long long*, hipStream_t);
int launch_hits_add_offset(int32_t*, const unsigned long long*, const unsigned long long*, long long, int, hipStream_t);
int launch_knn_parts_scatter(const float*, const int32_t*, int64_t, int, int, int, int, int, float*, int32_t*, hipStream_t);


}
```

### vsc2022_amd/csrc/rescore.hip

```cpp
#include <algorithm>

#include "prefilter_dev.h"

namespace vscmi {

__device__ __forceinline__ float quad_rotate(float v) {
    return __builtin_bit_cast(float, __builtin_amdgcn_mov_dpp(__builtin_bit_cast(int, v), 0x93, 0xf, 0xf, true));
}

struct WaveHits {
    int i[64];
    int j[64];
    float s[64];
};

__device__ __forceinline__ void flush_hits(const RescoreArgs& a, WaveHits& buf, int& pend) {
    if (pend == 0) return;
    const int lane = threadIdx.x & 63;
    asm volatile("s_waitcnt lgkmcnt(0)" ::: "memory");
    unsigned long long base = 0;
    if (lane == 0) base = atomicAdd(a.counter, (unsigned long long)pend);
    base = __shfl(base, 0);
    if ((long long)(base + pend) > a.cap) {
        if (lane == 0) atomicOr(a.list.overflow, 1);
    } else if (lane < pend) {
        a.out_i[base + lane] = buf.i[lane];
        a.out_j[base + lane] = buf.j[lane];
        a.out_s[base + lane] = buf.s[lane];
    }
    asm volatile("s_waitcnt lgkmcnt(0)" ::: "memory");
    pend = 0;
}

__device__ __forceinline__ void half_piece(const f16x8 h, f32x4& even, f32x4& odd) {
#pragma unroll
    for (int s = 0; s < 4; ++s) {
        even[s] = (float)h[2 * s];
        odd[s] = (float)h[2 * s + 1];
    }
}

template <int SRC>
__device__ __forceinline__ void rescore_list(const RescoreArgs& a, float radius, const int32_t* ci,
                                             const int32_t* cj, long long n, long long x0, long long step,
                                             WaveHits& buf, int& pend, const int* fill = nullptr, int shift = 0) {
    const int lane = threadIdx.x & 63, g = lane & 3;
    const long long n_thr = (4 * n + 63) & ~63ll;
    const int rounds = a.dpad / 32;
    for (long long x = x0; x < n_thr; x += step) {
        const long long c = x >> 2;
        const bool valid = c < n && (fill == nullptr || (int)(c & ((1ll << shift) - 1)) < fill[c >> shift]);
        int i = valid ? ci[c] : 0;
        const int j = valid ? cj[c] + a.j0 : 0;
        if (a.perm && valid) i = a.perm_i0 + a.perm[i - a.perm_i0];
        const f32x4* q = reinterpret_cast<const f32x4*>(a.Q + (int64_t)i * a.dpad) + 2 * g;
        const f32x4* r = reinterpret_cast<const f32x4*>(a.R + (int64_t)j * a.dpad) + 2 * g;
        const f16x8* rh = reinterpret_cast<const f16x8*>(a.Rh) +
                            (SRC == 2 ? (int64_t)(j >> 6) * (a.dpadh / 16) * 128 + ((j >> 5) & 1) * 64 + (j & 31) + (g >> 1) * 128 + (g & 1) * 32
                                      : (int64_t)j * (a.dpadh / 8) + g);
        constexpr int RH_STEP = SRC == 2 ? 256 : 4;
        float acc = 0.0f;
        f32x4 qe = q[0], qo = q[1], re, ro;
        if constexpr (SRC == 0) {
            re = r[0];
            ro = r[1];
        } else {
            half_piece(rh[0], re, ro);
        }
        for (int rd = 0; rd < rounds; ++rd) {
            const int nx = rd + 1 < rounds ? rd + 1 : rd;
            const f32x4 nqe = q[8 * nx], nqo = q[8 * nx + 1];
            f32x4 nre, nro;
            f16x8 nrh;
            if constexpr (SRC == 0) {
                nre = r[8 * nx];
                nro = r[8 * nx + 1];
            } else {
                nrh = rh[(int64_t)RH_STEP * nx];
            }
#pragma unroll
            for (int gp = 0; gp < 4; ++gp) {
                float v = acc;
#pragma unroll
                for (int s = 0; s < 4; ++s) {
                    v = __fmaf_rn(qe[s], re[s], v);
                    v = __fmaf_rn(qo[s], ro[s], v);
                }
                const float passed = quad_rotate(v);
                acc = (g == ((gp + 1) & 3)) ? passed : acc;
            }
            qe = nqe;
            qo = nqo;
            if constexpr (SRC == 0) {
                re = nre;
                ro = nro;
            } else {
                half_piece(nrh, re, ro);
            }
        }
        const bool hit = valid && g == 0 && (a.row_thr ? acc >= a.row_thr[i] : acc > radius);
        const unsigned long long m = __ballot(hit);
        if (hit) {
            const int p = pend + __popcll(m & ((1ull << lane) - 1));
            buf.i[p] = i;
            buf.j[p] = j;
            buf.s[p] = acc;
        }
        pend += __popcll(m);
        if (pend > 48) flush_hits(a, buf, pend);
    }
}

#ifndef VSC_RESCORE_SHARE
#define VSC_RESCORE_SHARE 4
#endif
constexpr int RESCORE_SHARE = VSC_RESCORE_SHARE;

template <int SRC>
__global__ __launch_bounds__(256) void rescore_kernel(RescoreArgs a) {
    if (*a.list.overflow) return;
    __shared__ WaveHits wave_hits[4];
    WaveHits& buf = wave_hits[threadIdx.x >> 6];
    int pend = 0;
    const float radius = a.row_thr ? 0.0f : *a.radius;
    unsigned long long seen = 0;
    {
        const int seg = blockIdx.x / RESCORE_SHARE, part = blockIdx.x % RESCORE_SHARE;
        const int n = min(a.list.seg_count[seg], a.list.seg_cap);
        if (part == 0) seen += (unsigned long long)n;
        rescore_list<SRC>(a, radius, a.list.i + (int64_t)seg * a.list.seg_cap, a.list.j + (int64_t)seg * a.list.seg_cap, n,
                     part * 256 + threadIdx.x, 256 * RESCORE_SHARE, buf, pend);
    }
    const unsigned long long nt_all = *a.list.tail_count;
    const long long nt = nt_all < (unsigned long long)a.list.tail_cap ? (long long)nt_all : a.list.tail_cap;
    if (nt > 0) {
        rescore_list<SRC>(a, radius, a.list.i + a.list.tail_base, a.list.j + a.list.tail_base, nt,
                     (long long)blockIdx.x * 256 + threadIdx.x, (long long)gridDim.x * 256, buf, pend, a.list.tail_fill,
                     a.list.tail_shift);
        if (blockIdx.x == 0) seen += (unsigned long long)nt;
    }
    flush_hits(a, buf, pend);
    if (threadIdx.x == 0 && seen) atomicAdd(a.n_cand_total, seen);
}

__global__ void tail_reset_kernel(unsigned long long* tail_count) { *tail_count = 0; }

__global__ __launch_bounds__(256) void cand_compact_kernel(RescoreArgs a, uint32_t* __restrict__ key_j,
                                                           uint32_t* __restrict__ val_i, unsigned long long* n_out) {
    __shared__ unsigned long long base_sh;
    if (*a.list.overflow) return;
    const int b = blockIdx.x;
    const int32_t *ci, *cj;
    int n;
    if (b < a.list.n_seg) {
        n = min(a.list.seg_count[b], a.list.seg_cap);
        ci = a.list.i + (int64_t)b * a.list.seg_cap;
        cj = a.list.j + (int64_t)b * a.list.seg_cap;
    } else {
        const long long chunk = b - a.list.n_seg;
        const unsigned long long nt = *a.list.tail_count;
        if ((unsigned long long)(chunk << a.list.tail_shift) >= nt || (long long)nt > a.list.tail_cap) return;
        n = a.list.tail_fill[chunk];
        ci = a.list.i + a.list.tail_base + (chunk << a.list.tail_shift);
        cj = a.list.j + a.list.tail_base + (chunk << a.list.tail_shift);
    }
    if (n <= 0) return;
    if (threadIdx.x == 0) base_sh = atomicAdd(n_out, (unsigned long long)n);
    __syncthreads();
    const unsigned long long base = base_sh;
    for (int x = threadIdx.x; x < n; x += 256) {
        int i = ci[x];
        if (a.perm) i = a.perm_i0 + a.perm[i - a.perm_i0];
        key_j[base + x] = (uint32_t)(cj[x] + a.j0);
        val_i[base + x] = (uint32_t)i;
    }
}

struct WavePairs {
    uint32_t i[64];
    uint32_t j[64];
};

template <bool FRAG>
__global__ __launch_bounds__(256) void f16_screen_kernel(ScreenArgs a) {
    if (*a.overflow) return;
    __shared__ WavePairs wave_pairs[4];
    WavePairs& buf = wave_pairs[threadIdx.x >> 6];
    int pend = 0;
    const int lane = threadIdx.x & 63, g = lane & 3;
    const long long n_thr = (4 * a.n + 63) & ~63ll;
    const int npiece = a.dpadh / 8, nks = a.dpadh / 16;
    const float radius = a.row_thr ? 0.0f : *a.radius;
    const f16x8* __restrict__ Rp = reinterpret_cast<const f16x8*>(a.Rh);
    auto flush = [&]() {
        if (pend == 0) return;
        asm volatile("s_waitcnt lgkmcnt(0)" ::: "memory");
        unsigned long long base = 0;
        if (lane == 0) base = atomicAdd(a.n_out, (unsigned long long)pend);
        base = __shfl(base, 0);
        if (lane < pend) {
            a.out_i[base + lane] = buf.i[lane];
            a.out_j[base + lane] = buf.j[lane];
        }
        asm volatile("s_waitcnt lgkmcnt(0)" ::: "memory");
        pend = 0;
    };
    for (long long x = (long long)blockIdx.x * 256 + threadIdx.x; x < n_thr; x += (long long)gridDim.x * 256) {
        const long long c = x >> 2;
        const bool valid = c < a.n;
        const uint32_t i = valid ? a.si[c] : 0u, j = valid ? a.sj[c] : 0u;
        const f16x8* __restrict__ q = reinterpret_cast<const f16x8*>(a.Qh + (int64_t)i * a.dpadh);
        const int64_t rbase = FRAG ? (int64_t)(j >> 6) * nks * 128 + ((j >> 5) & 1) * 64 + (j & 31)
                                   : (int64_t)j * npiece;
        float s0 = 0.0f, s1 = 0.0f;
#pragma unroll 8
        for (int p = g; p < npiece; p += 4) {
            const f16x8 qv = q[p];
            const f16x8 rv = FRAG ? Rp[rbase + (int64_t)(p >> 1) * 128 + (p & 1) * 32] : Rp[rbase + p];
#pragma unroll
            for (int e = 0; e < 8; e += 2) {
                s0 = __fmaf_rn((float)qv[e], (float)rv[e], s0);
                s1 = __fmaf_rn((float)qv[e + 1], (float)rv[e + 1], s1);
            }
        }
        float acc = s0 + s1;
        acc += __shfl_xor(acc, 1);
        acc += __shfl_xor(acc, 2);
        const float eps = (a.c1 * a.qn[i] * a.rn[j] + a.c2 * (a.qn[i] + a.rn[j]) + a.c3) * 1.001f;
        const bool pass = valid && g == 0 &&
                          (!(eps < INFINITY) || (a.row_thr ? acc >= candidate_edge(a.row_thr[i], eps) : acc > candidate_edge(radius, eps)));
        const unsigned long long m = __ballot(pass);
        if (pass) {
            const int p = pend + __popcll(m & ((1ull << lane) - 1));
            buf.i[p] = i;
            buf.j[p] = j;
        }
        pend += __popcll(m);
        if (pend > 48) flush();
    }
    flush();
    if (blockIdx.x == 0 && threadIdx.x == 0) atomicAdd(a.n_cand_total, (unsigned long long)a.n);
}

int launch_f16_screen(const ScreenArgs& a, hipStream_t stream) {
    VSC_HIP(hipMemsetAsync(a.n_out, 0, sizeof(unsigned long long), stream));
    if (a.n > 0) {
        const unsigned grid = (unsigned)std::min<long long>(16384, (a.n * 4 + 255) / 256);
        if (a.frag) hipLaunchKernelGGL(f16_screen_kernel<true>, dim3(grid), dim3(256), 0, stream, a);
        else hipLaunchKernelGGL(f16_screen_kernel<false>, dim3(grid), dim3(256), 0, stream, a);
        VSC_HIP(hipGetLastError());
    }
    return VSC_OK;
}

template <int SRC>
__global__ __launch_bounds__(256) void rescore_dense_kernel(RescoreArgs a, const uint32_t* __restrict__ sj,
                                                            const uint32_t* __restrict__ si, long long n,
                                                            const unsigned long long* __restrict__ n_dev) {
    if (*a.list.overflow) return;
    if (n_dev) n = (long long)*n_dev;
    __shared__ WaveHits wave_hits[4];
    WaveHits& buf = wave_hits[threadIdx.x >> 6];
    int pend = 0;
    const float radius = a.row_thr ? 0.0f : *a.radius;
    a.perm = nullptr;
    a.j0 = 0;
    rescore_list<SRC>(a, radius, reinterpret_cast<const int32_t*>(si), reinterpret_cast<const int32_t*>(sj), n,
                 (long long)blockIdx.x * 256 + threadIdx.x, (long long)gridDim.x * 256, buf, pend);
    flush_hits(a, buf, pend);
    if (blockIdx.x == 0 && threadIdx.x == 0 && !n_dev) atomicAdd(a.n_cand_total, (unsigned long long)n);
}

__global__ __launch_bounds__(1024) void cand_count_kernel(RescoreArgs a, int n_chunks_max, unsigned long long* n_out) {
    __shared__ unsigned long long red[16];
    unsigned long long s = 0;
    if (!*a.list.overflow) {
        for (int b = threadIdx.x; b < a.list.n_seg; b += 1024) s += (unsigned long long)max(0, min(a.list.seg_count[b], a.list.seg_cap));
        const unsigned long long nt = *a.list.tail_count;
        if ((long long)nt <= a.list.tail_cap) {
            const long long used = (long long)((nt + (1ull << a.list.tail_shift) - 1) >> a.list.tail_shift);
            for (long long c = threadIdx.x; c < used && c < n_chunks_max; c += 1024) s += (unsigned long long)max(0, a.list.tail_fill[c]);
        }
    }
#pragma unroll
    for (int off = 32; off > 0; off >>= 1) s += __shfl_xor(s, off);
    if ((threadIdx.x & 63) == 0) red[threadIdx.x >> 6] = s;
    __syncthreads();
    if (threadIdx.x == 0) {
        unsigned long long t = 0;
        for (int w = 0; w < 16; ++w) t += red[w];
        *n_out = t;
    }
}

int launch_cand_count(const RescoreArgs& a, int n_chunks_max, unsigned long long* n_out, hipStream_t stream) {
    hipLaunchKernelGGL(cand_count_kernel, dim3(1), dim3(1024), 0, stream, a, n_chunks_max, n_out);
    VSC_HIP(hipGetLastError());
    return VSC_OK;
}

int launch_cand_compact(const RescoreArgs& a, int n_chunks_max, uint32_t* key_j, uint32_t* val_i, unsigned long long* n_out,
                        hipStream_t stream) {
    VSC_HIP(hipMemsetAsync(n_out, 0, sizeof(unsigned long long), stream));
    hipLaunchKernelGGL(cand_compact_kernel, dim3((unsigned)(a.list.n_seg + n_chunks_max)), dim3(256), 0, stream, a, key_j, val_i, n_out);
    VSC_HIP(hipGetLastError());
    return VSC_OK;
}

int launch_rescore_dense(const RescoreArgs& a, const uint32_t* sj, const uint32_t* si, long long n, hipStream_t stream,
                         const unsigned long long* n_dev) {
    if (n > 0) {
        const unsigned grid = (unsigned)std::min<long long>(16384, (n * 4 + 255) / 256);
        if (a.rsrc == 0) hipLaunchKernelGGL(rescore_dense_kernel<0>, dim3(grid), dim3(256), 0, stream, a, sj, si, n, n_dev);
        else if (a.rsrc == 1) hipLaunchKernelGGL(rescore_dense_kernel<1>, dim3(grid), dim3(256), 0, stream, a, sj, si, n, n_dev);
        else hipLaunchKernelGGL(rescore_dense_kernel<2>, dim3(grid), dim3(256), 0, stream, a, sj, si, n, n_dev);
    }
    hipLaunchKernelGGL(tail_reset_kernel, dim3(1), dim3(1), 0, stream, a.list.tail_count);
    VSC_HIP(hipGetLastError());
    return VSC_OK;
}

int launch_rescore(const RescoreArgs& a, hipStream_t stream) {
    if (a.list.n_seg <= 0) return VSC_OK;
    const dim3 grid((unsigned)a.list.n_seg * RESCORE_SHARE);
    if (a.rsrc == 0) hipLaunchKernelGGL(rescore_kernel<0>, grid, dim3(256), 0, stream, a);
    else if (a.rsrc == 1) hipLaunchKernelGGL(rescore_kernel<1>, grid, dim3(256), 0, stream, a);
    else hipLaunchKernelGGL(rescore_kernel<2>, grid, dim3(256), 0, stream, a);
    hipLaunchKernelGGL(tail_reset_kernel, dim3(1), dim3(1), 0, stream, a.list.tail_count);
    VSC_HIP(hipGetLastError());
    return VSC_OK;
}

}
```

### vsc2022_amd/csrc/select.hip

```cpp
#include <cfloat>
#include "kernels.h"

namespace vscmi {


__global__ void select_begin_kernel(SelectCtl* c, unsigned long long max_results,
                                    unsigned long long min_results) {
    if (threadIdx.x < 256) c->hist[threadIdx.x] = 0;
    if (threadIdx.x == 0) {
        const bool act = !c->overflow && c->n > max_results;
        c->active = act ? 1 : 0;
        c->prefix = 0;
        c->prefix_mask = 0;
        c->rank = min_results;
        c->n_tmp = 0;
        if (act) c->n_rethreshold += 1;
    }
}

__global__ __launch_bounds__(256) void select_hist_kernel(SelectCtl* c, const float* s, int shift) {
    if (!c->active) return;
    __shared__ unsigned int lh[256];
    lh[threadIdx.x] = 0;
    __syncthreads();
    const unsigned long long n = c->n;
    const unsigned int prefix = c->prefix, pmask = c->prefix_mask;
    const int lane = threadIdx.x & 63;
    const unsigned long long n4 = (n + 3) / 4;
    for (unsigned long long q = (unsigned long long)blockIdx.x * 256 + threadIdx.x; q < ((n4 + 255) & ~255ull);
         q += (unsigned long long)gridDim.x * 256) {
        float v[4] = {0.0f, 0.0f, 0.0f, 0.0f};
        if (q < n4) {
            const float4 t = *reinterpret_cast<const float4*>(s + q * 4);
            v[0] = t.x; v[1] = t.y; v[2] = t.z; v[3] = t.w;
        }
#pragma unroll
        for (int e = 0; e < 4; ++e) {
            const unsigned int key = f2key(v[e]);
            const bool valid = q * 4 + e < n && (key & pmask) == prefix;
            const unsigned int bin = (key >> shift) & 255u;
            if (shift == 24) {
                unsigned long long todo = __ballot(valid);
                while (todo) {
                    const int leader = __ffsll((long long)todo) - 1;
                    const unsigned int lb = __shfl(bin, leader);
                    const unsigned long long same = __ballot(valid && bin == lb);
                    if (lane == leader) atomicAdd(&lh[lb], (unsigned int)__popcll(same));
                    todo &= ~same;
                }
            } else if (valid) {
                atomicAdd(&lh[bin], 1u);
            }
        }
    }
    __syncthreads();
    if (lh[threadIdx.x]) atomicAdd(&c->hist[threadIdx.x], lh[threadIdx.x]);
}

__global__ void select_pick_kernel(SelectCtl* c, int shift) {
    if (!c->active) return;
    __shared__ unsigned int h[256];
    h[threadIdx.x] = c->hist[threadIdx.x];
    __syncthreads();
    if (threadIdx.x == 0) {
        unsigned long long rank = c->rank;
        int d = 255;
        for (; d > 0; --d) {
            if (rank < h[d]) break;
            rank -= h[d];
        }
        c->rank = rank;
        c->prefix |= (unsigned int)d << shift;
        c->prefix_mask |= 255u << shift;
        if (shift == 0) c->radius = key2f(c->prefix);
    }
    __syncthreads();
    c->hist[threadIdx.x] = 0;
}

__global__ __launch_bounds__(256) void select_compact_kernel(SelectCtl* c, const int32_t* ai,
                                                             const int32_t* aj, const float* as,
                                                             int32_t* bi, int32_t* bj, float* bs) {
    if (!c->active) return;
    constexpr int PER_THREAD = 8, CHUNK = 256 * PER_THREAD;
    __shared__ unsigned int wave_cnt[4];
    __shared__ unsigned long long chunk_base;
    const unsigned long long n = c->n;
    const float radius = c->radius;
    const int lane = threadIdx.x & 63, wave = threadIdx.x >> 6;
    const unsigned long long n_chunks = (n + CHUNK - 1) / CHUNK;
    for (unsigned long long ch = blockIdx.x; ch < n_chunks; ch += gridDim.x) {
        const unsigned long long x0 = ch * CHUNK + threadIdx.x;
        float s[PER_THREAD];
        unsigned int keep_bits = 0;
#pragma unroll
        for (int e = 0; e < PER_THREAD; ++e) {
            const unsigned long long x = x0 + (unsigned long long)e * 256;
            s[e] = x < n ? as[x] : 0.0f;
            keep_bits |= (unsigned int)((x < n) && (s[e] > radius)) << e;
        }
        unsigned long long bal[PER_THREAD];
        unsigned int wave_total = 0;
#pragma unroll
        for (int e = 0; e < PER_THREAD; ++e) {
            bal[e] = __ballot((keep_bits >> e) & 1u);
            wave_total += (unsigned int)__popcll(bal[e]);
        }
        if (lane == 0) wave_cnt[wave] = wave_total;
        __syncthreads();
        if (threadIdx.x == 0) {
            const unsigned int tot = wave_cnt[0] + wave_cnt[1] + wave_cnt[2] + wave_cnt[3];
            chunk_base = tot ? atomicAdd(&c->n_tmp, (unsigned long long)tot) : 0ull;
        }
        __syncthreads();
        unsigned long long pos = chunk_base;
        for (int w = 0; w < wave; ++w) pos += wave_cnt[w];
        const unsigned long long below = (1ull << lane) - 1ull;
#pragma unroll
        for (int e = 0; e < PER_THREAD; ++e) {
            if ((keep_bits >> e) & 1u) {
                const unsigned long long x = x0 + (unsigned long long)e * 256;
                const unsigned long long p = pos + (unsigned int)__popcll(bal[e] & below);
                bi[p] = ai[x];
                bj[p] = aj[x];
                bs[p] = s[e];
            }
            pos += (unsigned int)__popcll(bal[e]);
        }
        __syncthreads();
    }
}

__global__ __launch_bounds__(256) void select_copyback_kernel(SelectCtl* c, const int32_t* bi,
                                                              const int32_t* bj, const float* bs,
                                                              int32_t* ai, int32_t* aj, float* as) {
    if (!c->active) return;
    const unsigned long long n = c->n_tmp;
    for (unsigned long long x = (unsigned long long)blockIdx.x * 256 + threadIdx.x; x < n;
         x += (unsigned long long)gridDim.x * 256) {
        ai[x] = bi[x];
        aj[x] = bj[x];
        as[x] = bs[x];
    }
}

__global__ void select_end_kernel(SelectCtl* c) {
    if (c->active) c->n = c->n_tmp;
}

__global__ void ctl_init_kernel(SelectCtl* c, float radius) {
    unsigned int* w = reinterpret_cast<unsigned int*>(c);
    for (unsigned x = threadIdx.x; x < sizeof(SelectCtl) / 4; x += blockDim.x) w[x] = 0u;
    __syncthreads();
    if (threadIdx.x == 0) c->radius = radius;
}
int launch_ctl_init(SelectCtl* ctl, float radius, hipStream_t stream) {
    static_assert(sizeof(SelectCtl) % 4 == 0, "SelectCtl is cleared word by word");
    hipLaunchKernelGGL(ctl_init_kernel, dim3(1), dim3(256), 0, stream, ctl, radius);
    VSC_HIP(hipGetLastError());
    return VSC_OK;
}

int enqueue_rethreshold(SelectCtl* ctl, HitView a, HitView b, unsigned long long K, hipStream_t stream) {
    constexpr int GRID = 1024;
    hipLaunchKernelGGL(select_begin_kernel, dim3(1), dim3(256), 0, stream, ctl, 2 * K, K);
    for (int shift = 24; shift >= 0; shift -= 8) {
        hipLaunchKernelGGL(select_hist_kernel, dim3(GRID), dim3(256), 0, stream, ctl, a.s, shift);
        hipLaunchKernelGGL(select_pick_kernel, dim3(1), dim3(256), 0, stream, ctl, shift);
    }
    hipLaunchKernelGGL(select_compact_kernel, dim3(GRID), dim3(256), 0, stream, ctl, a.i, a.j, a.s, b.i, b.j, b.s);
    hipLaunchKernelGGL(select_copyback_kernel, dim3(GRID), dim3(256), 0, stream, ctl, b.i, b.j, b.s, a.i, a.j, a.s);
    hipLaunchKernelGGL(select_end_kernel, dim3(1), dim3(1), 0, stream, ctl);
    VSC_HIP(hipGetLastError());
    return VSC_OK;
}

__global__ __launch_bounds__(256) void score_hist_kernel(const float* __restrict__ s, long long n, const long long* __restrict__ state,
                                                         int shift, unsigned long long* __restrict__ hist) {
    __shared__ unsigned int lh[256];
    lh[threadIdx.x] = 0;
    __syncthreads();
    const unsigned int prefix = (unsigned int)state[0], pmask = (unsigned int)state[1];
    const int lane = threadIdx.x & 63;
    const long long head = min(n, (long long)(((16 - ((uintptr_t)s & 15)) & 15) >> 2));
    const long long n4 = (n - head) / 4;
    const float4* s4 = reinterpret_cast<const float4*>(s + head);
    const long long rounds = (n4 + 255) & ~255ll;
    for (long long q = (long long)blockIdx.x * 256 + threadIdx.x; q < rounds; q += (long long)gridDim.x * 256) {
        float v[4] = {0.0f, 0.0f, 0.0f, 0.0f};
        const bool in = q < n4;
        if (in) {
            const float4 t = s4[q];
            v[0] = t.x; v[1] = t.y; v[2] = t.z; v[3] = t.w;
        }
#pragma unroll
        for (int e = 0; e < 4; ++e) {
            const unsigned int key = f2key(v[e] + 0.0f);
            const bool valid = in && (key & pmask) == prefix;
            const unsigned int bin = (key >> shift) & 255u;
            if (shift == 24) {
                unsigned long long todo = __ballot(valid);
                while (todo) {
                    const int leader = __ffsll((long long)todo) - 1;
                    const unsigned int lb = __shfl(bin, leader);
                    const unsigned long long same = __ballot(valid && bin == lb);
                    if (lane == leader) atomicAdd(&lh[lb], (unsigned int)__popcll(same));
                    todo &= ~same;
                }
            } else if (valid) {
                atomicAdd(&lh[bin], 1u);
            }
        }
    }
    if (blockIdx.x == 0) {
        const long long tail0 = head + n4 * 4;
        const long long extra = head + (n - tail0);
        if ((long long)threadIdx.x < extra) {
            const long long x = (long long)threadIdx.x < head ? threadIdx.x : tail0 + (threadIdx.x - head);
            const unsigned int key = f2key(s[x] + 0.0f);
            if ((key & pmask) == prefix) atomicAdd(&lh[(key >> shift) & 255u], 1u);
        }
    }
    __syncthreads();
    if (lh[threadIdx.x]) atomicAdd(&hist[threadIdx.x], (unsigned long long)lh[threadIdx.x]);
}

__global__ void score_pick_kernel(const long long* __restrict__ hist, long long* __restrict__ state, int shift) {
    if (threadIdx.x != 0 || blockIdx.x != 0) return;
    long long need = state[2], above = state[3];
    int d = 255;
    for (; d > 0; --d) {
        if (need <= hist[d]) break;
        need -= hist[d];
        above += hist[d];
    }
    state[0] = (long long)((unsigned int)state[0] | ((unsigned int)d << shift));
    state[1] = (long long)((unsigned int)state[1] | (255u << shift));
    state[2] = need;
    state[3] = above;
}

__global__ __launch_bounds__(256) void filter_hits_kernel(const int32_t* __restrict__ ai, const int32_t* __restrict__ aj,
                                                          const float* __restrict__ as, long long n, float radius,
                                                          int32_t* __restrict__ bi, int32_t* __restrict__ bj, float* __restrict__ bs,
                                                          unsigned long long* __restrict__ n_out) {
    constexpr int PER_THREAD = 8, CHUNK = 256 * PER_THREAD;
    __shared__ unsigned int wave_cnt[4];
    __shared__ unsigned long long chunk_base;
    const int lane = threadIdx.x & 63, wave = threadIdx.x >> 6;
    const long long n_chunks = (n + CHUNK - 1) / CHUNK;
    for (long long ch = blockIdx.x; ch < n_chunks; ch += gridDim.x) {
        const long long x0 = ch * CHUNK + threadIdx.x;
        float s[PER_THREAD];
        unsigned int keep_bits = 0;
#pragma unroll
        for (int e = 0; e < PER_THREAD; ++e) {
            const long long x = x0 + (long long)e * 256;
            s[e] = x < n ? as[x] : 0.0f;
            keep_bits |= (unsigned int)((x < n) && (s[e] > radius)) << e;
        }
        unsigned long long bal[PER_THREAD];
        unsigned int wave_total = 0;
#pragma unroll
        for (int e = 0; e < PER_THREAD; ++e) {
            bal[e] = __ballot((keep_bits >> e) & 1u);
            wave_total += (unsigned int)__popcll(bal[e]);
        }
        if (lane == 0) wave_cnt[wave] = wave_total;
        __syncthreads();
        if (threadIdx.x == 0) {
            const unsigned int tot = wave_cnt[0] + wave_cnt[1] + wave_cnt[2] + wave_cnt[3];
            chunk_base = tot ? atomicAdd(n_out, (unsigned long long)tot) : 0ull;
        }
        __syncthreads();
        unsigned long long pos = chunk_base;
        for (int w = 0; w < wave; ++w) pos += wave_cnt[w];
        const unsigned long long below = (1ull << lane) - 1ull;
#pragma unroll
        for (int e = 0; e < PER_THREAD; ++e) {
            if ((keep_bits >> e) & 1u) {
                const long long x = x0 + (long long)e * 256;
                const unsigned long long p = pos + (unsigned int)__popcll(bal[e] & below);
                bi[p] = ai[x];
                bj[p] = aj[x];
                bs[p] = s[e];
            }
            pos += (unsigned int)__popcll(bal[e]);
        }
        __syncthreads();
    }
}

int launch_filter_hits(ConstHitView a, long long n, float radius, HitView b, unsigned long long* n_out, hipStream_t stream) {
    VSC_HIP(hipMemsetAsync(n_out, 0, sizeof(unsigned long long), stream));
    if (n <= 0) return VSC_OK;
    const int grid = (int)std::min<long long>(1024, (n + 2047) / 2048);
    hipLaunchKernelGGL(filter_hits_kernel, dim3(grid), dim3(256), 0, stream, a.i, a.j, a.s, n, radius, b.i, b.j, b.s, n_out);
    VSC_HIP(hipGetLastError());
    return VSC_OK;
}

int launch_score_hist(const float* s, long long n, const long long* state, int shift, long long* hist, hipStream_t stream) {
    VSC_HIP(hipMemsetAsync(hist, 0, 256 * sizeof(long long), stream));
    if (n > 0) {
        const int grid = (int)std::min<long long>(1024, (n / 4 + 255) / 256 + 1);
        hipLaunchKernelGGL(score_hist_kernel, dim3(grid), dim3(256), 0, stream, s, n, state, shift,
                           reinterpret_cast<unsigned long long*>(hist));
        VSC_HIP(hipGetLastError());
    }
    return VSC_OK;
}

int launch_score_pick(const long long* hist, long long* state, int shift, hipStream_t stream) {
    hipLaunchKernelGGL(score_pick_kernel, dim3(1), dim3(64), 0, stream, hist, state, shift);
    VSC_HIP(hipGetLastError());
    return VSC_OK;
}

__global__ __launch_bounds__(256) void merge_topk_kernel(const float* __restrict__ s, const long long* __restrict__ ids, long long nq,
                                                         int m, int k, float* __restrict__ out_s, long long* __restrict__ out_ids) {
    extern __shared__ unsigned char lds_raw[];
    const int wave = threadIdx.x >> 6, lane = threadIdx.x & 63;
    float* ls = reinterpret_cast<float*>(lds_raw) + (size_t)wave * m;
    long long* li = reinterpret_cast<long long*>(lds_raw + (size_t)4 * m * 4) + (size_t)wave * m;
    const long long row = (long long)blockIdx.x * 4 + wave;
    if (row >= nq) return;
    for (int e = lane; e < m; e += 64) {
        const long long id = ids[row * m + e];
        ls[e] = id < 0 ? -INFINITY : s[row * m + e];
        li[e] = id < 0 ? 0x7fffffffffffffffLL : id;
    }
    __builtin_amdgcn_wave_barrier();
    __builtin_amdgcn_s_waitcnt(0);
    for (int e = lane; e < m; e += 64) {
        const float se = ls[e];
        const long long ie = li[e];
        int rank = 0;
        for (int f = 0; f < m; ++f) {
            const float sf = ls[f];
            const long long jf = li[f];
            rank += (sf > se) || (sf == se && (jf < ie || (jf == ie && f < e)));
        }
        if (rank < k) {
            const bool empty = ie == 0x7fffffffffffffffLL;
            out_s[row * k + rank] = empty ? -FLT_MAX : se;
            out_ids[row * k + rank] = empty ? -1 : ie;
        }
    }
}

int launch_merge_topk(const float* s, const long long* ids, long long nq, int m, int k, float* out_s, long long* out_ids,
                      hipStream_t stream) {
    if (nq <= 0) return VSC_OK;
    const size_t lds = (size_t)4 * m * (4 + 8);
    hipLaunchKernelGGL(merge_topk_kernel, dim3((unsigned)((nq + 3) / 4)), dim3(256), lds, stream, s, ids, nq, m, k, out_s, out_ids);
    VSC_HIP(hipGetLastError());
    return VSC_OK;
}

}
```

### vsc2022_amd/csrc/sim_f16p.hip

```cpp
#include "prefilter_dev.h"

namespace vscmi {

namespace f16p {

constexpr int PR = F16P_PANEL_ROWS;
constexpr int CSW = F16P_COL_STEP;
#ifndef VSC_F16P_PF
#define VSC_F16P_PF 4
#endif
constexpr int PF = VSC_F16P_PF;

__device__ __forceinline__ f16x8 bload(__amdgpu_buffer_rsrc_t rs, int voff, int soff) {
    return __builtin_bit_cast(f16x8, __builtin_amdgcn_raw_buffer_load_b128(rs, voff, soff, 0));
}

template <int NKC>
__device__ __forceinline__ void tile_mma(const char* smem, const int (&abase)[8], f16x8 (&a)[4], f16x8 (&ring)[PF][2],
                                         __amdgpu_buffer_rsrc_t rs, int so_tile, int so_next, int lane16,
                                         f32x16 (&acc)[4][2]) {
    const f32x16 zero = {0.f, 0.f, 0.f, 0.f, 0.f, 0.f, 0.f, 0.f, 0.f, 0.f, 0.f, 0.f, 0.f, 0.f, 0.f, 0.f};
    constexpr int NKS = NKC * 8;
#pragma unroll
    for (int ks = 0; ks < NKS; ++ks) {
        const int t = ks + PF - 1;
        const int so = (t < NKS) ? so_tile + t * 2048 : so_next + (t - NKS) * 2048;
        const int kn = (ks + 1) % NKS;
        const char* anext = smem + (kn >> 3) * 32768 + abase[kn & 7];
#pragma unroll
        for (int m = 0; m < 4; ++m) {
            acc[m][0] = __builtin_amdgcn_mfma_f32_32x32x16_f16(a[m], ring[ks % PF][0], ks == 0 ? zero : acc[m][0], 0, 0, 0);
            acc[m][1] = __builtin_amdgcn_mfma_f32_32x32x16_f16(a[m], ring[ks % PF][1], ks == 0 ? zero : acc[m][1], 0, 0, 0);
            a[m] = *reinterpret_cast<const f16x8*>(anext + m * 8192);
            if (m < 2) ring[(ks + PF - 1) % PF][m] = bload(rs, lane16 + m * 1024, so);
        }
#pragma unroll
        for (int m = 0; m < 4; ++m) {
            __builtin_amdgcn_sched_group_barrier(0x008, 2, 0);
            __builtin_amdgcn_sched_group_barrier(0x100, 1, 0);
            if (m < 2) __builtin_amdgcn_sched_group_barrier(0x020, 1, 0);
        }
    }
}

template <bool ROWTHR>
__device__ __forceinline__ void emit_candidates(const SimF16PArgs& a, const bool (&all)[2], const float (&thr)[2],
                                                const float (&eps)[2], const float* rt, const float (&rtmin)[4],
                                                int row0, int col0, bool interior, const f32x16 (&acc)[4][2],
                                                const float (&bm)[4][2], int64_t seg_base, int& count, TailExt* ext) {
#pragma unroll
    for (int m = 0; m < 4; ++m)
#pragma unroll
        for (int n = 0; n < 2; ++n) {
            const bool blk = all[n] || (ROWTHR ? bm[m][n] >= candidate_edge(rtmin[m], eps[n]) : bm[m][n] > thr[n]);
            if (!__any(blk)) continue;
            const int ln_blk = ROWTHR ? lane_now() : 0;
#pragma unroll
            for (int r = 0; r < 16; ++r) {
                const int rb = m * 32 + (r & 3) + 8 * (r >> 2);
                bool cand;
                if (ROWTHR)
                    cand = acc[m][n][r] >= candidate_edge(rt[rb + 4 * (ln_blk >> 5)], eps[n]);
                else
                    cand = acc[m][n][r] > thr[n];
                const bool hit = all[n] || cand;
                const unsigned long long hits = __ballot(hit);
                if (hits == 0ull) continue;
                const int ln = ROWTHR ? ln_blk : lane_now();
                const int i = row0 + rb + 4 * (ln >> 5);
                const int j = col0 + n * 32 + (ln & 31);
                const bool mine = hit && (interior || (i < a.nq && j < a.nr));
                const unsigned long long ok = interior ? hits : __ballot(mine);
                if (ok == 0ull) continue;
                const int total = __popcll(ok);
                int64_t pos;
                if (!cand_reserve(a.list, seg_base, count, total, ln, ext, pos)) continue;
                if (mine) {
                    pos += lanes_below(ok);
                    a.list.i[pos] = a.i0 + i;
                    a.list.j[pos] = j;
                }
            }
        }
}

__device__ __forceinline__ void emit_candidates_seg(const SimF16PArgs& a, const float (&thr)[2], int row0, int col0,
                                                    const f32x16 (&acc)[4][2], const float (&bm)[4][2],
                                                    __amdgpu_buffer_rsrc_t rs_i, __amdgpu_buffer_rsrc_t rs_j, int& count) {
#pragma unroll
    for (int m = 0; m < 4; ++m)
#pragma unroll
        for (int n = 0; n < 2; ++n) {
            if (!__any(bm[m][n] > thr[n])) continue;
            const int ln = lane_now();
            const int ibase = a.i0 + row0 + m * 32 + 4 * (ln >> 5);
            const int j = col0 + n * 32 + (ln & 31);
#pragma unroll
            for (int r = 0; r < 16; ++r) {
                const bool cand = acc[m][n][r] > thr[n];
                const unsigned long long hits = __ballot(cand);
                if (hits == 0ull) continue;
                if (cand) {
                    const int off = (count + (int)lanes_below(hits)) << 2;
                    __builtin_amdgcn_raw_buffer_store_b32(ibase + (r & 3) + 8 * (r >> 2), rs_i, off, 0, 0);
                    __builtin_amdgcn_raw_buffer_store_b32(j, rs_j, off, 0, 0);
                }
                count += __popcll(hits);
            }
        }
}

}

template <int NKC, bool ROWTHR>
__global__ __launch_bounds__(512) void sim_f16p_kernel(SimF16PArgs a) {
    using namespace f16p;
    extern __shared__ __attribute__((aligned(16))) char smem[];
    __shared__ float qn_max_w[8];
    __shared__ float rt_sh[ROWTHR ? PR : 1];
    __shared__ int item_sh[2];
    __shared__ TailExt tail_sh[8];
    const int tid = threadIdx.x, lane = tid & 63;
    const int wave = __builtin_amdgcn_readfirstlane(tid >> 6);
    constexpr int NKS = NKC * 8;
    constexpr int ROWB = NKC * 256;
    constexpr int TILEB = NKS * 2048;
    const int lane16 = lane * 16;
    int abase[8];
    {
        const int hi = lane >> 5, r15 = lane & 15, rl = lane & 31;
#pragma unroll
        for (int u = 0; u < 8; ++u) abase[u] = rl * 256 + ((((2 * u) | hi) ^ r15) << 4);
    }
    const float radius = ROWTHR ? 0.0f : *a.radius;
    const int seg = blockIdx.x * 8 + wave;
    const int64_t seg_base = (int64_t)seg * a.list.seg_cap;
    int count = 0;
    tail_init(&tail_sh[wave], lane);
    const __amdgpu_buffer_rsrc_t rs_ci = __builtin_amdgcn_make_buffer_rsrc(
        (void*)uniform_ptr(reinterpret_cast<const char*>(a.list.i + seg_base)), 0, a.list.seg_cap * 4, 0x00020000);
    const __amdgpu_buffer_rsrc_t rs_cj = __builtin_amdgcn_make_buffer_rsrc(
        (void*)uniform_ptr(reinterpret_cast<const char*>(a.list.j + seg_base)), 0, a.list.seg_cap * 4, 0x00020000);
    const int nslice = (a.nsteps + a.slice - 1) / a.slice;
    int cur_panel = -1;
    float nq_max = 0.f;
    float rtmin[4] = {0.f, 0.f, 0.f, 0.f};
    int panel = blockIdx.x % a.npanel;
    for (;;) {
        __syncthreads();
        if (wave == 0) {
            int p = panel, s = 0;
            const bool lost = __hip_atomic_load(a.list.overflow, __ATOMIC_RELAXED, __HIP_MEMORY_SCOPE_AGENT) != 0;
            for (;;) {
                if (lost) { p = -1; break; }
                if (lane == 0) s = atomicAdd(&a.next_slice[p], 1);
                s = __shfl(s, 0);
                if (s < nslice) break;
                int best = 0x7fffffff, bp = 0x7fffffff;
                for (int q0 = 0; q0 < a.npanel; q0 += 64) {
                    const int q = q0 + lane;
                    const int pp = (q + (int)blockIdx.x) % a.npanel;
                    const int v = q < a.npanel ? __hip_atomic_load(&a.next_slice[pp], __ATOMIC_RELAXED, __HIP_MEMORY_SCOPE_AGENT)
                                               : 0x7fffffff;
                    if (v < best) { best = v; bp = pp; }
                }
#pragma unroll
                for (int off = 32; off > 0; off >>= 1) {
                    const int ob = __shfl_xor(best, off), op = __shfl_xor(bp, off);
                    if (ob < best || (ob == best && op < bp)) { best = ob; bp = op; }
                }
                if (best >= nslice) { p = -1; break; }
                p = bp;
            }
            if (lane == 0) { item_sh[0] = p; item_sh[1] = s; }
        }
        __syncthreads();
        panel = item_sh[0];
        const int sl = item_sh[1];
        if (panel < 0) break;
        const int cs0 = sl * a.slice, cs1 = min(a.nsteps, cs0 + a.slice);
        if (panel != cur_panel) {
            __syncthreads();
            const __amdgpu_buffer_rsrc_t qrs = __builtin_amdgcn_make_buffer_rsrc(
                (void*)uniform_ptr(reinterpret_cast<const char*>(a.Q) + (int64_t)panel * PR * ROWB), 0, PR * ROWB, 0x00020000);
#pragma unroll
            for (int n = 0; n < NKC * 4; ++n) {
                const int p = n * 512 + tid;
                const int kc = p >> 11, row = (p >> 4) & 127, slot = p & 15;
                const int c = kc * 16 + (slot ^ (row & 15));
                dma16(qrs, row * ROWB + c * 16, 0, smem + (n * 512 + wave * 64) * 16);
            }
            const bool in_batch = tid < PR && panel * PR + tid < a.nq;
            float nv = in_batch ? a.qn[(int64_t)panel * PR + tid] : 0.f;
#pragma unroll
            for (int off = 32; off > 0; off >>= 1) nv = fmaxf(nv, __shfl_xor(nv, off));
            if (lane == 0) qn_max_w[wave] = nv;
            if (ROWTHR && tid < PR) rt_sh[tid] = in_batch ? a.row_thr[(int64_t)panel * PR + tid] : INFINITY;
            asm volatile("s_waitcnt vmcnt(0)" ::: "memory");
            __syncthreads();
            nq_max = fmaxf(qn_max_w[0], qn_max_w[1]);
            if (ROWTHR) {
                float v0 = rt_sh[lane], v1 = rt_sh[64 + lane];
#pragma unroll
                for (int off = 16; off > 0; off >>= 1) {
                    v0 = fminf(v0, __shfl_xor(v0, off));
                    v1 = fminf(v1, __shfl_xor(v1, off));
                }
                rtmin[0] = __builtin_bit_cast(float, __builtin_amdgcn_readlane(__builtin_bit_cast(int, v0), 0));
                rtmin[1] = __builtin_bit_cast(float, __builtin_amdgcn_readlane(__builtin_bit_cast(int, v0), 32));
                rtmin[2] = __builtin_bit_cast(float, __builtin_amdgcn_readlane(__builtin_bit_cast(int, v1), 0));
                rtmin[3] = __builtin_bit_cast(float, __builtin_amdgcn_readlane(__builtin_bit_cast(int, v1), 32));
            }
            cur_panel = panel;
        }
        const __amdgpu_buffer_rsrc_t rs = __builtin_amdgcn_make_buffer_rsrc(
            (void*)uniform_ptr(reinterpret_cast<const char*>(a.Rf) + (int64_t)cs0 * 8 * TILEB), 0, (cs1 - cs0) * 8 * TILEB,
            0x00020000);
        int so_tile = wave * TILEB;
        f16x8 ring[PF][2];
#pragma unroll
        for (int dd = 0; dd < PF - 1; ++dd) {
            ring[dd][0] = bload(rs, lane16, so_tile + dd * 2048);
            ring[dd][1] = bload(rs, lane16 + 1024, so_tile + dd * 2048);
        }
        f16x8 afr[4];
#pragma unroll
        for (int m = 0; m < 4; ++m) afr[m] = *reinterpret_cast<const f16x8*>(smem + abase[0] + m * 8192);
        for (int cs = cs0; cs < cs1; ++cs) {
            const int col0 = cs * CSW + wave * 64;
            const float rn0 = a.rn[col0 + (lane & 31)], rn1 = a.rn[col0 + 32 + (lane & 31)];
            f32x16 acc[4][2];
            tile_mma<NKC>(smem, abase, afr, ring, rs, so_tile, so_tile + 8 * TILEB, lane16, acc);
            so_tile += 8 * TILEB;
            const float eps[2] = {(a.c1 * nq_max * rn0 + a.c2 * (nq_max + rn0) + a.c3) * 1.001f,
                                  (a.c1 * nq_max * rn1 + a.c2 * (nq_max + rn1) + a.c3) * 1.001f};
            const bool all[2] = {!(eps[0] < INFINITY), !(eps[1] < INFINITY)};
            const float thr[2] = {candidate_edge(radius, eps[0]), candidate_edge(radius, eps[1])};
            float bm[4][2];
#pragma unroll
            for (int m = 0; m < 4; ++m)
#pragma unroll
                for (int n = 0; n < 2; ++n) {
                    float x = fmaxf(fmaxf(acc[m][n][0], acc[m][n][1]), acc[m][n][2]);
#pragma unroll
                    for (int r = 3; r < 15; r += 2) x = fmaxf(fmaxf(x, acc[m][n][r]), acc[m][n][r + 1]);
                    bm[m][n] = fmaxf(x, acc[m][n][15]);
                }
            bool any_blk = all[0] || all[1];
            if (ROWTHR) {
#pragma unroll
                for (int m = 0; m < 4; ++m)
                    any_blk |= bm[m][0] >= candidate_edge(rtmin[m], eps[0]) || bm[m][1] >= candidate_edge(rtmin[m], eps[1]);
            } else {
                const float x0 = fmaxf(fmaxf(bm[0][0], bm[1][0]), fmaxf(bm[2][0], bm[3][0]));
                const float x1 = fmaxf(fmaxf(bm[0][1], bm[1][1]), fmaxf(bm[2][1], bm[3][1]));
                any_blk |= x0 > thr[0] || x1 > thr[1];
            }
            if (__any(any_blk)) {
                const bool interior = panel * PR + PR <= a.nq && col0 + 64 <= a.nr;
                if (!ROWTHR && interior && !all[0] && !all[1] && count + 8192 <= a.list.seg_cap)
                    emit_candidates_seg(a, thr, panel * PR, col0, acc, bm, rs_ci, rs_cj, count);
                else
                    emit_candidates<ROWTHR>(a, all, thr, eps, rt_sh, rtmin, panel * PR, col0, interior, acc, bm,
                                            seg_base, count, &tail_sh[wave]);
            }
        }
    }
    tail_close(a.list, lane, &tail_sh[wave]);
    if (lane == 0) a.list.seg_count[seg] = count;
}

void sim_f16p_plan(int64_t nq, int64_t nr, int* npanel, int* nsteps, int* slice, int* grid) {
    using namespace f16p;
    const int64_t P = (nq + PR - 1) / PR, S = (nr + CSW - 1) / CSW;
    int64_t sl = (S * P) / (256 * 16);
    sl = std::max<int64_t>(4, std::min<int64_t>(64, sl));
    sl = std::min(sl, std::max<int64_t>(S, 1));
    const int64_t items = P * ((S + sl - 1) / sl);
    *npanel = (int)P;
    *nsteps = (int)S;
    *slice = (int)sl;
    *grid = (int)std::max<int64_t>(1, std::min<int64_t>(256, items));
}

template <int NKC>
static int launch_nkc(const SimF16PArgs& a, int grid, hipStream_t stream) {
    const int lds = NKC * 32768;
    static PerDeviceOnce once;
    if (once.first()) {
        VSC_HIP(hipFuncSetAttribute((const void*)sim_f16p_kernel<NKC, false>, hipFuncAttributeMaxDynamicSharedMemorySize, lds));
        VSC_HIP(hipFuncSetAttribute((const void*)sim_f16p_kernel<NKC, true>, hipFuncAttributeMaxDynamicSharedMemorySize, lds));
        once.commit();
    }
    if (a.row_thr)
        hipLaunchKernelGGL((sim_f16p_kernel<NKC, true>), dim3((unsigned)grid), dim3(512), lds, stream, a);
    else
        hipLaunchKernelGGL((sim_f16p_kernel<NKC, false>), dim3((unsigned)grid), dim3(512), lds, stream, a);
    VSC_HIP(hipGetLastError());
    return VSC_OK;
}

int launch_sim_f16p(const SimF16PArgs& a, int grid, hipStream_t stream) {
    if (grid <= 0 || a.npanel <= 0 || a.nsteps <= 0) {
        if (grid > 0) VSC_HIP(hipMemsetAsync(a.list.seg_count, 0, (size_t)a.list.n_seg * sizeof(int), stream));
        return VSC_OK;
    }
    VSC_HIP(hipMemsetAsync(a.next_slice, 0, (size_t)a.npanel * sizeof(int), stream));
    switch (a.dpadh) {
        case 128: return launch_nkc<1>(a, grid, stream);
        case 256: return launch_nkc<2>(a, grid, stream);
        case 384: return launch_nkc<3>(a, grid, stream);
        case 512: return launch_nkc<4>(a, grid, stream);
    }
    set_error("sim_f16p: dpadh %d is not one of 128, 256, 384, 512", a.dpadh);
    return VSC_ERR_INVALID;
}

}
```

### vsc2022_amd/vsc/index.py

```python
import logging
from dataclasses import dataclass
from typing import Iterable, Iterator, List, NamedTuple, Optional, Sequence, Tuple

import ctypes
import numpy as np

from vsc2022_amd import _lib

METRIC_INNER_PRODUCT = _lib.METRIC_INNER_PRODUCT
METRIC_L2 = _lib.METRIC_L2

SearchIndices = Tuple[int, int, float]


@dataclass
class VideoMetadata:

    video_id: str
    timestamps: np.ndarray

    def __len__(self):
        return self.timestamps.shape[0]

    def get_timestamps(self, idx: int) -> Tuple[float, float]:
        t = self.timestamps[idx]
        if len(self.timestamps.shape) == 1:
            return (t, t)
        return (t[0], t[1])


@dataclass
class VideoFeature(VideoMetadata):

    feature: np.ndarray

    def __post_init__(self):
        assert self.feature.shape[0] == len(self.timestamps), "Mismatched timestamps / feature size"

    def metadata(self):
        return VideoMetadata(video_id=self.video_id, timestamps=self.timestamps)

    def dimensions(self):
        return self.feature.shape[1]


class PairMatch(NamedTuple):

    query_timestamps: Tuple[float, float]
    ref_timestamps: Tuple[float, float]
    score: float


class _MatchView(Sequence):

    __slots__ = ("_q_meta", "_r_meta", "_q_idx", "_r_idx", "_scores")

    def __init__(self, q_meta, r_meta, q_idx, r_idx, scores):
        self._q_meta, self._r_meta = q_meta, r_meta
        self._q_idx, self._r_idx, self._scores = q_idx, r_idx, scores

    def __len__(self):
        return len(self._scores)

    def __getitem__(self, k):
        if isinstance(k, slice):
            return [self[x] for x in range(*k.indices(len(self)))]
        return PairMatch(
            query_timestamps=self._q_meta.get_timestamps(self._q_idx[k]),
            ref_timestamps=self._r_meta.get_timestamps(self._r_idx[k]),
            score=self._scores[k],
        )

    def __eq__(self, other):
        return list(self) == list(other)

    def __repr__(self):
        return repr(list(self))

    @property
    def scores(self) -> np.ndarray:
        return self._scores


@dataclass
class PairMatches:

    query_id: str
    ref_id: str
    matches: List[PairMatch]

    def records(self):
        for match in self.matches:
            yield {
                "query_id": self.query_id,
                "ref_id": self.ref_id,
                "query_start": match.query_timestamps[0],
                "query_end": match.query_timestamps[1],
                "ref_start": match.ref_timestamps[0],
                "ref_end": match.ref_timestamps[1],
                "score": match.score,
            }


class FlatIndex:

    def __init__(self, d: int, metric: int = METRIC_INNER_PRODUCT, device: Optional[int] = None,
                 options: Optional[dict] = None, codec: str = "Flat"):
        if metric not in (METRIC_INNER_PRODUCT, METRIC_L2):
            raise ValueError(f"unsupported metric {metric}")
        codec_id = _lib.codec_id(codec)
        self.codec = codec
        self.d = int(d)
        self.metric_type = metric
        self.device = _lib.default_device() if device is None else int(device)
        self._h = ctypes.c_void_p()
        self._stream = None
        _lib.check(_lib.lib().vsc_index_create_codec(self.d, metric, self.device, codec_id, ctypes.byref(self._h)))
        for name, value in (options or {}).items():
            self.set_option(name, value)

    def __del__(self):
        h = getattr(self, "_h", None)
        if h is not None and h.value:
            try:
                _lib.lib().vsc_index_destroy(h)
            except Exception:
                pass
            self._h = None

    @property
    def handle(self):
        return self._h

    @property
    def ntotal(self) -> int:
        return int(_lib.lib().vsc_index_ntotal(self._h))

    def set_option(self, name: str, value: float):
        _lib.check(_lib.lib().vsc_index_set_option(self._h, name.encode(), float(value)))

    def get_option(self, name: str) -> float:
        v = ctypes.c_double(0.0)
        _lib.check(_lib.lib().vsc_index_get_option(self._h, name.encode(), ctypes.byref(v)))
        return v.value

    def use_stream(self, hip_stream: Optional[int]):
        if hip_stream is None:
            _lib.check(_lib.lib().vsc_index_set_stream(self._h, None, 1))
        else:
            _lib.check(_lib.lib().vsc_index_set_stream(self._h, ctypes.c_void_p(int(hip_stream)), 0))
        self._stream = None if hip_stream is None else int(hip_stream)

    def use_torch_stream(self):
        import torch

        self.use_stream(torch.cuda.current_stream(torch.device("cuda", self.device)).cuda_stream)

    def _after_torch(self, dev=None):
        import torch

        dev = torch.device("cuda", self.device) if dev is None else dev
        if self._stream is not None and torch.cuda.current_stream(dev).cuda_stream == self._stream:
            return
        torch.cuda.synchronize(dev)

    def _rows(self, x):
        if isinstance(x, np.ndarray) or not hasattr(x, "data_ptr"):
            x = _lib.f32c(x)
        else:
            import torch

            x = x.to(torch.float32).contiguous()
            if x.is_cuda:
                self._after_torch(x.device)
        if x.ndim != 2 or x.shape[1] != self.d:
            raise ValueError(f"expected [n, {self.d}] features, got {tuple(x.shape)}")
        p, mem = _lib.ptr(x)
        return p, mem, int(x.shape[0]), x

    def _half_rows(self, x):
        if isinstance(x, np.ndarray):
            if x.dtype != np.float16:
                return None
            x = np.ascontiguousarray(x)
        elif hasattr(x, "data_ptr"):
            import torch

            if x.dtype != torch.float16:
                return None
            x = x.contiguous()
            if x.is_cuda:
                self._after_torch(x.device)
        else:
            return None
        if x.ndim != 2 or x.shape[1] != self.d:
            raise ValueError(f"expected [n, {self.d}] features, got {tuple(x.shape)}")
        p, mem = _lib.ptr(x)
        return p, mem, int(x.shape[0]), x

    def add(self, x):
        half = self._half_rows(x)
        if half is not None:
            p, mem, n, keep = half
            _lib.check(_lib.lib().vsc_index_add_f16(self._h, p, n, mem))
            return
        p, mem, n, keep = self._rows(x)
        _lib.check(_lib.lib().vsc_index_add(self._h, p, n, mem))

    def reconstruct_n(self, i0: int = 0, n: Optional[int] = None) -> np.ndarray:
        i0 = int(i0)
        n = self.ntotal - i0 if n is None else int(n)
        if i0 < 0 or n < 0 or i0 + n > self.ntotal:
            raise ValueError(f"rows [{i0}, {i0 + n}) are not inside the index ({self.ntotal} rows)")
        out = np.empty((n, self.d), dtype=np.float32)
        _lib.check(_lib.lib().vsc_index_reconstruct(self._h, i0, n, out.ctypes.data, _lib.MEM_HOST))
        return out

    def search(self, x, k: int, device_out: bool = False):
        p, mem, n, keep = self._rows(x)
        if device_out:
            import torch

            dev = torch.device("cuda", self.device)
            D = torch.empty((n, k), dtype=torch.float32, device=dev)
            I = torch.empty((n, k), dtype=torch.int64, device=dev)
            self._after_torch(dev)
            _lib.check(_lib.lib().vsc_index_knn(self._h, p, n, mem, int(k), D.data_ptr(), I.data_ptr(),
                                                _lib.MEM_DEVICE))
            return D, I
        D = np.empty((n, k), dtype=np.float32)
        I = np.empty((n, k), dtype=np.int64)
        _lib.check(_lib.lib().vsc_index_knn(self._h, p, n, mem, int(k), D.ctypes.data, I.ctypes.data,
                                            _lib.MEM_HOST))
        return D, I

    def range_search(self, x, radius: float):
        p, mem, n, keep = self._rows(x)
        lims = np.zeros(n + 1, dtype=np.int64)
        need = ctypes.c_int64(0)
        L = _lib.lib()
        _lib.check(L.vsc_index_range_search(self._h, p, n, mem, float(radius), lims.ctypes.data, None,
                                            None, 0, ctypes.byref(need)))
        D = np.empty(need.value, dtype=np.float32)
        I = np.empty(need.value, dtype=np.int64)
        if need.value:
            _lib.check(L.vsc_index_range_search(self._h, p, n, mem, float(radius), lims.ctypes.data,
                                                D.ctypes.data, I.ctypes.data, need.value,
                                                ctypes.byref(need)))
        return lims.astype(np.uint64), D, I

    def global_topk(self, x, K: int, device_out: bool = False, seed_radius=None):
        p, mem, n, keep = self._rows(x)
        K = int(K)
        n_out = ctypes.c_int64(0)
        radius = ctypes.c_float(0.0)
        cap = max(min(K, n * max(self.ntotal, 1)), 1)

        def call(pi, pj, ps, out_mem):
            if seed_radius is None:
                _lib.check(_lib.lib().vsc_index_global_topk(self._h, p, n, mem, K, pi, pj, ps, cap, out_mem,
                                                            ctypes.byref(n_out), ctypes.byref(radius)))
            else:
                _lib.check(_lib.lib().vsc_index_global_topk_seeded(self._h, p, n, mem, K, float(seed_radius), pi, pj, ps, cap,
                                                                   out_mem, ctypes.byref(n_out), ctypes.byref(radius)))

        if device_out:
            import torch

            dev = torch.device("cuda", self.device)
            oi = torch.empty(cap, dtype=torch.int32, device=dev)
            oj = torch.empty(cap, dtype=torch.int32, device=dev)
            os_ = torch.empty(cap, dtype=torch.float32, device=dev)
            self._after_torch(dev)
            call(oi.data_ptr(), oj.data_ptr(), os_.data_ptr(), _lib.MEM_DEVICE)
            m = n_out.value
            return oi[:m], oj[:m], os_[:m], radius.value
        oi = np.empty(cap, dtype=np.int32)
        oj = np.empty(cap, dtype=np.int32)
        os_ = np.empty(cap, dtype=np.float32)
        call(oi.ctypes.data, oj.ctypes.data, os_.ctypes.data, _lib.MEM_HOST)
        m = n_out.value
        return oi[:m], oj[:m], os_[:m], radius.value

    def range_scores(self, x, radius: float, k_hint: int, device_out: bool = False):
        n = int(x.shape[0])
        total = n * max(self.ntotal, 1)
        kk = max(int(k_hint), 1024)
        while True:
            k_try = min(kk, total)
            _, _, s, rad = self.global_topk(x, k_try, device_out=device_out, seed_radius=float(radius))
            if k_try >= total or (np.float32(rad) == np.float32(radius) and len(s) < k_try):
                return s
            kk *= 4

    def set_hit_capacity(self, cap: int):
        _lib.check(_lib.lib().vsc_index_set_hit_capacity(self._h, int(cap)))

    def profile(self, enable: bool):
        _lib.check(_lib.lib().vsc_index_profile(self._h, 1 if enable else 0))

    def profile_read(self, reset: bool = True):
        ms, n, fl = ctypes.c_double(0), ctypes.c_int64(0), ctypes.c_double(0)
        _lib.check(_lib.lib().vsc_index_profile_read(self._h, ctypes.byref(ms), ctypes.byref(n),
                                                     ctypes.byref(fl), 1 if reset else 0))
        out = {"sim_ms": ms.value, "sim_launches": n.value, "sim_flops": fl.value}
        for cls, name in ((1, "f16"), (2, "rescore"), (3, "select"), (4, "sort"), (5, "i8"), (6, "i8_prep")):
            _lib.check(_lib.lib().vsc_index_profile_read_class(self._h, cls, ctypes.byref(ms), ctypes.byref(n),
                                                               ctypes.byref(fl), 1 if reset else 0))
            out.update({f"{name}_ms": ms.value, f"{name}_launches": n.value, f"{name}_flops": fl.value})
        cand, hits = ctypes.c_int64(0), ctypes.c_int64(0)
        _lib.check(_lib.lib().vsc_index_search_stats(self._h, ctypes.byref(cand), ctypes.byref(hits)))
        out["candidates"] = cand.value
        return out


class _RowToVideoId(Sequence):

    def __init__(self, row2vid: np.ndarray, video_ids: list):
        self._row2vid, self._ids = row2vid, video_ids

    def __len__(self):
        return len(self._row2vid)

    def __getitem__(self, k):
        if isinstance(k, slice):
            return [self._ids[v] for v in self._row2vid[k]]
        return self._ids[self._row2vid[k]]


class VideoLayout:

    def __init__(self, videos: Sequence[VideoFeature]):
        self.video_ids = [v.video_id for v in videos]
        lens = np.fromiter((len(v) for v in videos), dtype=np.int64, count=len(videos))
        self.offsets = np.zeros(len(videos) + 1, dtype=np.int64)
        np.cumsum(lens, out=self.offsets[1:])
        self.n_rows = int(self.offsets[-1])
        self.row2vid = np.repeat(np.arange(len(videos), dtype=np.int32), lens)
        self.row2frame = (np.arange(self.n_rows, dtype=np.int64) - np.repeat(self.offsets[:-1], lens)).astype(np.int32)
        self.metadata = [v.metadata() for v in videos]

    @staticmethod
    def features(videos: Sequence[VideoFeature]) -> np.ndarray:
        if len(videos) == 0:
            return np.zeros((0, 0), dtype=np.float32)
        return np.concatenate([_lib.f32c(v.feature) for v in videos], axis=0)


class SearchHits:

    def __init__(self, i, j, s, q_layout: VideoLayout, index: "VideoIndex"):
        self.i, self.j, self.s = i, j, s
        self.q_layout, self.index = q_layout, index

    def __len__(self):
        return len(self.s)


class VideoIndex:

    def __init__(self, dim: int, codec_str: str = "Flat", metric: int = METRIC_INNER_PRODUCT,
                 device: Optional[int] = None):
        _lib.codec_id(codec_str)
        self.dim = dim
        self.codec_str = codec_str
        self.index = FlatIndex(dim, metric, device, codec=codec_str)
        self.video_metadata = {}
        self._video_ids: list = []
        self._vid_ordinal = {}
        self._row2vid = np.zeros(0, dtype=np.int32)
        self._row2frame = np.zeros(0, dtype=np.int32)

    @property
    def video_clip_idx(self) -> np.ndarray:
        return self._row2frame

    @property
    def video_clip_to_video_ids(self) -> Sequence:
        return _RowToVideoId(self._row2vid, self._video_ids)

    def add(self, db: List[VideoFeature]):
        if len(db) == 0:
            return
        layout = VideoLayout(db)
        base = len(self._video_ids)
        ordinals = np.empty(len(db), dtype=np.int32)
        for k, vf in enumerate(db):
            o = self._vid_ordinal.get(vf.video_id)
            if o is None:
                o = len(self._video_ids)
                self._vid_ordinal[vf.video_id] = o
                self._video_ids.append(vf.video_id)
            ordinals[k] = o
            self.video_metadata[vf.video_id] = layout.metadata[k]
        del base
        self._row2vid = np.concatenate([self._row2vid, ordinals[layout.row2vid]])
        self._row2frame = np.concatenate([self._row2frame, layout.row2frame])
        if all(isinstance(v.feature, np.ndarray) and v.feature.dtype == np.float16 for v in db):
            self.index.add(np.concatenate([v.feature for v in db], axis=0))
        else:
            self.index.add(VideoLayout.features(db))

    def search_hits(self, queries: List[VideoFeature], global_k: int, device_out: bool = False):
        layout = VideoLayout(queries)
        feats = VideoLayout.features(queries)
        if global_k < 0:
            k = -global_k
            logging.warning(
                "Using local k for KNN search. Warning: this is against the "
                "VSC rules, since predictions for a query-ref pair are not "
                "independent of other references. KNN search is provided for "
                "comparison."
            )
            D, I = self.index.search(feats, k)
            i = np.repeat(np.arange(D.shape[0], dtype=np.int32), k)
            return SearchHits(i, I.reshape(-1).astype(np.int32), D.reshape(-1), layout, self)
        i, j, s, _ = self.index.global_topk(feats, global_k, device_out=device_out)
        return SearchHits(i, j, s, layout, self)

    def search(self, queries: List[VideoFeature], global_k: int) -> List[PairMatches]:
        hits = self.search_hits(queries, global_k)
        if len(hits) == 0:
            return []
        q_vid = hits.q_layout.row2vid[hits.i].astype(np.int64)
        r_vid = self._row2vid[hits.j].astype(np.int64)
        key = q_vid * max(len(self._video_ids), 1) + r_vid
        _, first, inverse = np.unique(key, return_index=True, return_inverse=True)
        pair_rank = np.empty(len(first), dtype=np.int64)
        pair_rank[np.argsort(first, kind="stable")] = np.arange(len(first))
        order = np.argsort(pair_rank[inverse], kind="stable")
        bounds = np.r_[0, np.cumsum(np.bincount(pair_rank[inverse], minlength=len(first)))]
        q_frame = hits.q_layout.row2frame[hits.i][order]
        r_frame = self._row2frame[hits.j][order]
        scores = hits.s[order]
        q_vid, r_vid = q_vid[order], r_vid[order]
        out = []
        for p in range(len(first)):
            a, b = bounds[p], bounds[p + 1]
            qv, rv = int(q_vid[a]), int(r_vid[a])
            q_id, r_id = hits.q_layout.video_ids[qv], self._video_ids[rv]
            out.append(
                PairMatches(
                    q_id,
                    r_id,
                    _MatchView(hits.q_layout.metadata[qv], self.video_metadata[r_id], q_frame[a:b],
                               r_frame[a:b], scores[a:b]),
                )
            )
        return out

    def _global_threshold_knn_search(self, query_features: np.ndarray, global_k: int) -> Iterable[SearchIndices]:
        i, j, s, _ = self.index.global_topk(query_features, global_k)
        return list(zip(i.tolist(), j.tolist(), s))

    def _knn_search(self, query_features: np.ndarray, k) -> Iterator[SearchIndices]:
        D, I = self.index.search(query_features, k)
        for a in range(I.shape[0]):
            for b in range(I.shape[1]):
                yield (a, I[a, b], D[a, b])
```

Measured before the change: 20030 query-videos/s.

## Defer exact rescoring of candidates between radius and a predicted future floor

Adds deferred rescoring to the global top-k search. A floor score is picked by rank selection, predicting where the threshold will sit by a later rethreshold event. Candidates whose prefilter score falls between the radius and that floor are marked and set aside instead of being rescored exactly right away. A modified rethreshold then checks whether the deferred pairs can still matter, and rescores them only when they can. This cuts exact fp32/fp16 rescoring of candidates the tightening threshold would drop anyway, at the cost of extra host syncs, floor-selection passes and possible forced rescoring. It is enabled by default.

```diff
diff --git a/vsc2022_amd/csrc/api.hip b/vsc2022_amd/csrc/api.hip
--- a/vsc2022_amd/csrc/api.hip
+++ b/vsc2022_amd/csrc/api.hip
@@ -121,6 +121,7 @@
     {"knn_s0min", "VSC_KNN_S0MIN"}, {"knn_ratio", "VSC_KNN_RATIO"}, {"knn_nchunk", "VSC_KNN_NCHUNK"}, {"knn_first_tile", "VSC_KNN_FIRST_TILE"},
     {"cand_budget", "VSC_CAND_BUDGET"}, {"debug_i8", "VSC_DEBUG_I8"}, {"debug_screen", "VSC_DEBUG_SCREEN"},
     {"topk_shortcut", "VSC_TOPK_SHORTCUT"}, {"topk_sample", "VSC_TOPK_SAMPLE"}, {"sort_hits", "VSC_SORT_HITS"}, {"density_hint", "VSC_DENSITY_HINT"},
+    {"defer", "VSC_DEFER"}, {"defer_margin", "VSC_DEFER_MARGIN"}, {"defer_i8", "VSC_DEFER_I8"},
 };
 
 static int option_needs_empty(const vsc_index* idx, const char* name) {
@@ -197,6 +198,9 @@
     if (is("topk_sample")) { if (!(v >= 2.0)) goto bad; idx->topk_sample_rows = (int64_t)v; return VSC_OK; }
     if (is("sort_hits")) { idx->sort_hits = v != 0.0; return VSC_OK; }
     if (is("density_hint")) { if (!(v >= 0.0)) goto bad; idx->density_hint = v; return VSC_OK; }
+    if (is("defer")) { const int m = (int)v; if (m < 0 || m > 2) goto bad; idx->defer = m; return VSC_OK; }
+    if (is("defer_i8")) { idx->defer_i8 = v != 0.0; return VSC_OK; }
+    if (is("defer_margin")) { if (!(v > -1.0 && v < 100.0)) goto bad; idx->defer_margin = v; return VSC_OK; }
     set_error("vsc_index_set_option: unknown option '%s'", name);
     return VSC_ERR_INVALID;
 bad:
@@ -238,6 +242,14 @@
     else if (is("topk_sample")) *out = (double)idx->topk_sample_rows;
     else if (is("sort_hits")) *out = idx->sort_hits;
     else if (is("density_hint")) *out = idx->density_hint;
+    else if (is("defer")) *out = idx->defer;
+    else if (is("defer_margin")) *out = idx->defer_margin;
+    else if (is("defer_i8")) *out = idx->defer_i8;
+    else if (is("deferred")) *out = (double)idx->stat_deferred;
+    else if (is("defer_forced")) *out = (double)idx->stat_defer_forced;
+    else if (is("defer_events_ok")) *out = (double)idx->stat_defer_events_ok;
+    else if (is("defer_events_forced")) *out = (double)idx->stat_defer_events_forced;
+    else if (is("n_rethreshold")) *out = (double)idx->stat_n_rethreshold;
     else if (is("last_topk_route")) *out = idx->last_topk_route;
     else if (is("i8_center")) *out = idx->i8_center;
     else if (is("i8_center_on")) *out = idx->i8_mu_on;
diff --git a/vsc2022_amd/csrc/api_internal.h b/vsc2022_amd/csrc/api_internal.h
--- a/vsc2022_amd/csrc/api_internal.h
+++ b/vsc2022_amd/csrc/api_internal.h
@@ -30,6 +30,7 @@
     DevBuf q8, pstat;
     DevBuf cs[4], cstmp, csn;
     DevBuf tailfill;
+    DevBuf dd[2];
     DevBuf rt8c;
     DevBuf rt8d;
     DevBuf rt8, rt8b;
@@ -47,6 +48,7 @@
         q8.release(); pstat.release(); rt8.release(); rt8b.release(); rt8c.release(); rt8d.release(); tailfill.release();
         for (auto& b : cs) b.release();
         cstmp.release(); csn.release();
+        for (auto& b : dd) b.release();
         for (auto& b : hA) b.release();
         for (auto& b : hB) b.release();
         ctl.release(); sort.release(); cnt.release();
@@ -107,6 +109,12 @@
     int i8_group_shift = 9;
     bool rescore_by_ref = true;
     bool i8_screen = false;
+    int defer = 1;
+    bool defer_i8 = true;
+    double defer_margin = 0.05;
+    unsigned long long stat_deferred = 0, stat_defer_forced = 0, stat_defer_events_ok = 0, stat_defer_events_forced = 0;
+    unsigned long long stat_n_rethreshold = 0;
+    bool defer_now = false;
     bool knn_i8 = true;
     bool knn_two_level = true;
     double knn_subset_factor = 300.0;
diff --git a/vsc2022_amd/csrc/api_search.hip b/vsc2022_amd/csrc/api_search.hip
--- a/vsc2022_amd/csrc/api_search.hip
+++ b/vsc2022_amd/csrc/api_search.hip
@@ -72,6 +72,7 @@
     f.c1 = fb.c1; f.c2 = fb.c2; f.c3 = fb.c3;
     f.radius = &idx->ws.ctl.as<SelectCtl>()->radius;
     f.row_thr = b.row_thr ? b.row_thr + b.i0 : nullptr;
+    f.floor = idx->defer_now && !b.row_thr ? &idx->ws.ctl.as<SelectCtl>()->floor : nullptr;
     VSC_TRY(cand_list_plan(idx, ccap, grid, cl));
     f.list = cl;
     VSC_TRY(prof_begin(idx, stop, 1));
@@ -164,18 +165,15 @@
     return launch_sim_i8p(f, grid, idx->stream);
 }
 
-static int exact_stage(vsc_index* idx, const F16Batch& b, int64_t cap, const CandList& cl, const int32_t* perm,
-                       const F16Bound& fb, bool from_i8) {
-    SelectCtl* ctl = idx->ws.ctl.as<SelectCtl>();
-    Workspace& ws = idx->ws;
-    const HitView kept = ws.hits_a();
+static RescoreArgs rescore_args(vsc_index* idx, const float* qpacked, int64_t cap) {
+    SelectCtl* ctl = idx->ws.ctl.as<SelectCtl>();
+    const HitView kept = idx->ws.hits_a();
     RescoreArgs r;
-    r.Q = b.qpacked;
+    r.Q = qpacked;
     r.R = idx->ref.as<float>();
     r.dpad = idx->dpad;
-    r.list = cl;
-    r.perm = perm;
-    r.perm_i0 = (int)b.i0;
+    r.perm = nullptr;
+    r.perm_i0 = 0;
     r.n_cand_total = &ctl->n_cand_total;
     r.radius = &ctl->radius;
     r.out_i = kept.i;
@@ -183,14 +181,26 @@
     r.out_s = kept.s;
     r.counter = &ctl->n;
     r.cap = cap;
-    r.row_thr = b.row_thr;
-    r.j0 = (int)b.nr_begin;
+    r.row_thr = nullptr;
     if (sq16(idx)) {
         r.R = nullptr;
         r.Rh = idx->refh.as<_Float16>();
         r.dpadh = idx->dpadh;
         r.rsrc = idx->frag ? 2 : 1;
     }
+    return r;
+}
+
+static int exact_stage(vsc_index* idx, const F16Batch& b, int64_t cap, const CandList& cl, const int32_t* perm,
+                       const F16Bound& fb, bool from_i8) {
+    SelectCtl* ctl = idx->ws.ctl.as<SelectCtl>();
+    Workspace& ws = idx->ws;
+    RescoreArgs r = rescore_args(idx, b.qpacked, cap);
+    r.list = cl;
+    r.perm = perm;
+    r.perm_i0 = (int)b.i0;
+    r.row_thr = b.row_thr;
+    r.j0 = (int)b.nr_begin;
     if (!idx->rescore_by_ref) return launch_rescore(r, idx->stream);
     VSC_TRY(ws.csn.reserve(3 * sizeof(unsigned long long)));
     unsigned long long* csn = ws.csn.as<unsigned long long>();
@@ -203,11 +213,34 @@
     for (auto& buf : ws.cs)
         if (buf.bytes < (size_t)(n_c + 1) * sizeof(uint32_t)) VSC_TRY(buf.reserve(cap_e * sizeof(uint32_t)));
     uint32_t* cs[4] = {ws.cs[0].as<uint32_t>(), ws.cs[1].as<uint32_t>(), ws.cs[2].as<uint32_t>(), ws.cs[3].as<uint32_t>()};
+    const bool defer = idx->defer_now && !b.row_thr;
+    if (defer) {
+        for (auto& buf : ws.dd) VSC_TRY(buf.reserve((size_t)cap * sizeof(int32_t)));
+        if (!from_i8) {
+            r.d_i = ws.dd[0].as<int32_t>();
+            r.d_j = ws.dd[1].as<int32_t>();
+            r.d_count = &ctl->n_d;
+            r.d_total = &ctl->n_deferred;
+            r.d_cap = cap;
+        }
+    }
     VSC_TRY(launch_cand_compact(r, n_chunks_max, cs[0], cs[2], csn, idx->stream));
+    if (r.d_i) {
+        VSC_HIP(hipMemcpyAsync(&n_c, csn, sizeof(n_c), hipMemcpyDeviceToHost, idx->stream));
+        VSC_HIP(hipStreamSynchronize(idx->stream));
+    }
     const uint32_t *sj = nullptr, *si = nullptr;
     VSC_TRY(sort_candidates_by_ref(cs[0], cs[1], cs[2], cs[3], (int64_t)n_c, b.nr_end, ws.cstmp, &sj, &si, idx->stream));
-    if (!(from_i8 && idx->i8_screen && n_c > 0)) return launch_rescore_dense(r, sj, si, (long long)n_c, idx->stream);
+    if (!(from_i8 && (idx->i8_screen || defer) && n_c > 0)) return launch_rescore_dense(r, sj, si, (long long)n_c, idx->stream);
     ScreenArgs sa;
+    if (defer) {
+        sa.floor = &ctl->floor;
+        sa.d_i = ws.dd[0].as<int32_t>();
+        sa.d_j = ws.dd[1].as<int32_t>();
+        sa.d_count = &ctl->n_d;
+        sa.d_total = &ctl->n_deferred;
+        sa.d_cap = cap;
+    }
     sa.Qh = ws.qh.as<_Float16>();
     sa.qn = ws.qn.as<float>();
     sa.Rh = idx->refh.as<_Float16>();
@@ -313,6 +346,95 @@
     return VSC_OK;
 }
 
+
+static int force_deferred(vsc_index* idx, const float* qpacked, int64_t cap, unsigned long long n_d, unsigned long long n_before) {
+    SelectCtl* ctl = idx->ws.ctl.as<SelectCtl>();
+    Workspace& ws = idx->ws;
+    if (n_d == 0) return launch_defer_reset(ctl, idx->stream);
+    hipEvent_t stop;
+    VSC_TRY(prof_begin(idx, &stop, 2));
+    const size_t cap_e = (size_t)(n_d + n_d / 4 + 4096);
+    for (auto& buf : ws.cs)
+        if (buf.bytes < (size_t)(n_d + 1) * sizeof(uint32_t)) VSC_TRY(buf.reserve(cap_e * sizeof(uint32_t)));
+    uint32_t* cs[4] = {ws.cs[0].as<uint32_t>(), ws.cs[1].as<uint32_t>(), ws.cs[2].as<uint32_t>(), ws.cs[3].as<uint32_t>()};
+    VSC_HIP(hipMemcpyAsync(cs[0], ws.dd[1].p, (size_t)n_d * 4, hipMemcpyDeviceToDevice, idx->stream));
+    VSC_HIP(hipMemcpyAsync(cs[2], ws.dd[0].p, (size_t)n_d * 4, hipMemcpyDeviceToDevice, idx->stream));
+    const uint32_t *sj = nullptr, *si = nullptr;
+    VSC_TRY(sort_candidates_by_ref(cs[0], cs[1], cs[2], cs[3], (int64_t)n_d, idx->ntotal, ws.cstmp, &sj, &si, idx->stream));
+    RescoreArgs r = rescore_args(idx, qpacked, cap);
+    r.list = CandList{};
+    VSC_TRY(ws.csn.reserve(3 * sizeof(unsigned long long)));
+    r.n_cand_total = ws.csn.as<unsigned long long>() + 1;
+    r.list.overflow = &ctl->overflow;
+    r.list.tail_count = &ctl->n_tail;
+    VSC_TRY(launch_rescore_dense(r, sj, si, (long long)n_d, idx->stream));
+    VSC_TRY(launch_defer_reset(ctl, idx->stream));
+    VSC_TRY(prof_end(idx, stop, 0.0, 2));
+    SelectCtl h;
+    VSC_HIP(hipMemcpyAsync(&h, ctl, sizeof(h), hipMemcpyDeviceToHost, idx->stream));
+    VSC_HIP(hipStreamSynchronize(idx->stream));
+    if (!h.overflow && h.n != n_before + n_d) {
+        set_error("global_topk: %llu of %llu deferred pairs did not pass the radius when they were re-scored",
+                  n_before + n_d - h.n, n_d);
+        return VSC_ERR_INVALID;
+    }
+    idx->stat_defer_forced += n_d;
+    return VSC_OK;
+}
+
+static int choose_floor(vsc_index* idx, int64_t K, int64_t nq, int64_t b, int64_t i1, int64_t bs, bool* chosen, bool* no_event_left) {
+    SelectCtl* ctl = idx->ws.ctl.as<SelectCtl>();
+    const bool forced = idx->defer == 2;
+    *chosen = false;
+    SelectCtl h;
+    VSC_HIP(hipMemcpyAsync(&h, ctl, sizeof(h), hipMemcpyDeviceToHost, idx->stream));
+    VSC_HIP(hipStreamSynchronize(idx->stream));
+    if (h.overflow || h.n == 0 || b <= 0) return VSC_OK;
+    int64_t b_next = -1;
+    for (int64_t e = i1, sb = bs;;) {
+        if ((double)e * (double)h.n > 2.0 * (double)K * (double)b) { b_next = e; break; }
+        if (e >= nq) break;
+        if (sb < 20000) sb *= 2;
+        e = std::min(nq, e + sb);
+    }
+    if (b_next < 0) {
+        if (!forced) { *no_event_left = true; return VSC_OK; }
+        b_next = 2 * b;
+    }
+    const double m = std::ceil(((double)K + 1.0) * ((double)b / (double)b_next) * (1.0 + idx->defer_margin));
+    if ((!(m >= 1.0) || m > (double)h.n) && !forced) return VSC_OK;
+    const unsigned long long rank = (unsigned long long)std::min(std::max(m, 1.0), (double)h.n) - 1ull;
+    hipEvent_t stop;
+    VSC_TRY(prof_begin(idx, &stop, 3));
+    VSC_TRY(enqueue_floor_select(ctl, idx->ws.hits_a().s, rank, idx->stream));
+    VSC_TRY(prof_end(idx, stop, 0.0, 3));
+    *chosen = true;
+    return VSC_OK;
+}
+
+static int deferred_event(vsc_index* idx, const float* qpacked, int64_t K, int64_t cap, bool* open) {
+    SelectCtl* ctl = idx->ws.ctl.as<SelectCtl>();
+    hipEvent_t stop;
+    VSC_TRY(prof_begin(idx, &stop, 3));
+    VSC_TRY(enqueue_rethreshold_deferred(ctl, idx->ws.hits_a(), idx->ws.hits_b(), (unsigned long long)K, idx->stream));
+    VSC_TRY(prof_end(idx, stop, 0.0, 3));
+    SelectCtl h;
+    VSC_HIP(hipMemcpyAsync(&h, ctl, sizeof(h), hipMemcpyDeviceToHost, idx->stream));
+    VSC_HIP(hipStreamSynchronize(idx->stream));
+    if (h.overflow) { *open = false; return VSC_OK; }
+    if (h.need_force) {
+        VSC_TRY(force_deferred(idx, qpacked, cap, h.n_d, h.n));
+        idx->stat_defer_events_forced += 1;
+        VSC_TRY(prof_begin(idx, &stop, 3));
+        VSC_TRY(enqueue_rethreshold(ctl, idx->ws.hits_a(), idx->ws.hits_b(), (unsigned long long)K, idx->stream));
+        VSC_TRY(prof_end(idx, stop, 0.0, 3));
+        *open = false;
+    } else if (!(h.floor < INFINITY)) {
+        *open = false;
+    }
+    return VSC_OK;
+}
+
 int init_ctl(vsc_index* idx, float radius_score_space) {
     return launch_ctl_init(idx->ws.ctl.as<SelectCtl>(), radius_score_space, idx->stream);
 }
@@ -339,8 +461,12 @@
     cap = std::min<int64_t>(cap, cap_max);
     SelectCtl h;
     bool allow_i8 = i8_usable(idx);
+    const bool can_defer = idx->defer > 0 && !seeded && ip && idx->sort_hits && idx->hit_cap_user <= 0 && idx->rescore_by_ref && K >= 1;
     for (;;) {
         bool used_i8 = false;
+        bool d_open = false;
+        bool no_event_left = false;
+        idx->stat_deferred = idx->stat_defer_forced = idx->stat_defer_events_ok = idx->stat_defer_events_forced = 0;
         VSC_TRY(ensure_hit_buffers(idx, cap));
         VSC_TRY(init_ctl(idx, seeded ? (ip ? radius0 : -radius0) : -1e10f));
         SelectCtl* ctl = idx->ws.ctl.as<SelectCtl>();
@@ -353,8 +479,15 @@
             const bool f16 = idx->prefilter_force || (idx->prefilter && (seen > 0 || idx->density_hint > 0.0) && dens < idx->prefilter_density);
             const bool i8 = f16 && allow_i8 && (idx->i8_mode == 2 || dens < idx->i8_density);
             used_i8 |= i8;
-            VSC_TRY(enqueue_batch(idx, qp, i0, i1, cap, f16, i8));
-            if (i1 < nq) {
+            const bool defers = can_defer && !no_event_left && f16 && (i8 ? idx->defer_i8 : idx->frag);
+            if (defers && !d_open) VSC_TRY(choose_floor(idx, K, nq, i0, i1, bs, &d_open, &no_event_left));
+            idx->defer_now = defers && d_open;
+            const int rc_batch = enqueue_batch(idx, qp, i0, i1, cap, f16, i8);
+            idx->defer_now = false;
+            VSC_TRY(rc_batch);
+            if (d_open) {
+                VSC_TRY(deferred_event(idx, qp, K, cap, &d_open));
+            } else if (i1 < nq) {
                 hipEvent_t stop;
                 VSC_TRY(prof_begin(idx, &stop, 3));
                 VSC_TRY(enqueue_rethreshold(ctl, idx->ws.hits_a(), idx->ws.hits_b(), (unsigned long long)K, idx->stream));
@@ -365,6 +498,11 @@
         }
         VSC_HIP(hipMemcpyAsync(&h, ctl, sizeof(h), hipMemcpyDeviceToHost, idx->stream));
         VSC_HIP(hipStreamSynchronize(idx->stream));
+        if (d_open && !h.overflow) {
+            VSC_TRY(force_deferred(idx, qp, cap, h.n_d, h.n));
+            VSC_HIP(hipMemcpyAsync(&h, ctl, sizeof(h), hipMemcpyDeviceToHost, idx->stream));
+            VSC_HIP(hipStreamSynchronize(idx->stream));
+        }
         if (!h.overflow && h.n > 2ull * (unsigned long long)K) {
             hipEvent_t stop;
             VSC_TRY(prof_begin(idx, &stop, 3));
@@ -373,6 +511,14 @@
             VSC_HIP(hipMemcpyAsync(&h, ctl, sizeof(h), hipMemcpyDeviceToHost, idx->stream));
             VSC_HIP(hipStreamSynchronize(idx->stream));
         }
+        idx->stat_deferred = h.n_deferred;
+        idx->stat_defer_events_ok = h.ev_ok;
+        idx->stat_n_rethreshold = h.n_rethreshold;
+        if (idx->debug_i8 && can_defer)
+            fprintf(stderr, "[vscmi] deferred rescoring (defer %d, margin %g): %llu of %llu candidates deferred, %llu re-scored after all; "
+                    "%llu events decided without them, %llu needed them (%llu events)\n", idx->defer, idx->defer_margin,
+                    idx->stat_deferred, h.n_cand_total, idx->stat_defer_forced, idx->stat_defer_events_ok,
+                    idx->stat_defer_events_forced, idx->stat_n_rethreshold);
         VSC_TRY(prof_collect(idx));
         idx->stat_candidates = h.n_cand_total;
         if (!h.overflow) break;
diff --git a/vsc2022_amd/csrc/kernels.h b/vsc2022_amd/csrc/kernels.h
--- a/vsc2022_amd/csrc/kernels.h
+++ b/vsc2022_amd/csrc/kernels.h
@@ -45,6 +45,7 @@
     float c1, c2, c3;
     const float* radius; const float* row_thr;
     CandList list;
+    const float* floor = nullptr;
 };
 constexpr int I8P_MAX_DPAD8 = 1024;
 constexpr int I8_MAX_EXCLUDED = 8;
@@ -71,6 +72,7 @@
     const float* radius; const float* row_thr;
     CandList list;
 };
+constexpr uint32_t DEFER_MARK = 0x80000000u;
 struct RescoreArgs {
     const float* Q; const float* R; int dpad;
     CandList list;
@@ -81,6 +83,8 @@
     const float* row_thr;
     int j0 = 0;
     const _Float16* Rh = nullptr; int dpadh = 0; int rsrc = 0;
+    int32_t* d_i = nullptr; int32_t* d_j = nullptr; unsigned long long* d_count = nullptr; unsigned long long* d_total = nullptr;
+    long long d_cap = 0;
 };
 struct ScreenArgs {
     const _Float16* Qh; const float* qn;
@@ -91,7 +95,10 @@
     const uint32_t* sj; const uint32_t* si; long long n;
     uint32_t* out_j; uint32_t* out_i; unsigned long long* n_out;
     unsigned long long* n_cand_total;
-    const int* overflow;
+    int* overflow;
+    const float* floor = nullptr;
+    int32_t* d_i = nullptr; int32_t* d_j = nullptr; unsigned long long* d_count = nullptr; unsigned long long* d_total = nullptr;
+    long long d_cap = 0;
 };
 struct SimKnnArgs {
     const float* Q; const float* R; int dpad; int nq; int nr; int tq; int tr; int nchunk; int k;
@@ -113,6 +120,12 @@
     unsigned long long n_rethreshold;
     unsigned long long n_cand_total;
     unsigned long long n_tail;
+    unsigned long long n_d;
+    unsigned long long n_deferred;
+    float floor;
+    int need_force;
+    unsigned int ev_ok;
+    unsigned int pad_;
 };
 struct TnPairArgs {
     const float* qfeat; const float* rfeat; const int64_t* q_off; const int64_t* r_off; int dpad;
@@ -232,6 +245,9 @@
 int launch_matrix_knn(const MatKnnArgs&, hipStream_t);
 int set_thresh_kernel_attrs();
 int enqueue_rethreshold(SelectCtl*, HitView, HitView, unsigned long long, hipStream_t);
+int enqueue_rethreshold_deferred(SelectCtl*, HitView, HitView, unsigned long long, hipStream_t);
+int enqueue_floor_select(SelectCtl*, const float*, unsigned long long, hipStream_t);
+int launch_defer_reset(SelectCtl*, hipStream_t);
 int sort_hits_topk(ConstHitView, int64_t, int64_t, int64_t, int64_t, SortScratch&, HitView, int, int64_t*, hipStream_t);
 int sort_hits_rowcol(ConstHitView, int64_t, SortScratch&, HitView, int, hipStream_t);
 int pair_max_device(const int32_t*, const int32_t*, const float*, int64_t, const int32_t*, const int32_t*, int64_t, int64_t,
diff --git a/vsc2022_amd/csrc/rescore.hip b/vsc2022_amd/csrc/rescore.hip
--- a/vsc2022_amd/csrc/rescore.hip
+++ b/vsc2022_amd/csrc/rescore.hip
@@ -165,6 +165,58 @@
         cj = a.list.j + a.list.tail_base + (chunk << a.list.tail_shift);
     }
     if (n <= 0) return;
+    if (a.d_i) {
+        __shared__ unsigned int marked_sh, cur_sh[2];
+        __shared__ unsigned long long base_d_sh;
+        if (threadIdx.x == 0) { marked_sh = 0; cur_sh[0] = 0; cur_sh[1] = 0; }
+        __syncthreads();
+        unsigned int mine = 0;
+        for (int x = threadIdx.x; x < n; x += 256) mine += (uint32_t)ci[x] >> 31;
+#pragma unroll
+        for (int off = 32; off > 0; off >>= 1) mine += __shfl_xor(mine, off);
+        if ((threadIdx.x & 63) == 0 && mine) atomicAdd(&marked_sh, mine);
+        __syncthreads();
+        const unsigned int nm = marked_sh;
+        if (threadIdx.x == 0) {
+            base_sh = atomicAdd(n_out, (unsigned long long)(n - (int)nm));
+            base_d_sh = nm ? atomicAdd(a.d_count, (unsigned long long)nm) : 0ull;
+            if (nm) {
+                atomicAdd(a.d_total, (unsigned long long)nm);
+                atomicAdd(a.n_cand_total, (unsigned long long)nm);
+            }
+        }
+        __syncthreads();
+        const unsigned long long base = base_sh, base_d = base_d_sh;
+        const bool d_fits = (long long)(base_d + nm) <= a.d_cap;
+        if (!d_fits && threadIdx.x == 0) atomicOr(a.list.overflow, 1);
+        const int lane = threadIdx.x & 63;
+        for (int x0 = 0; x0 < n; x0 += 256) {
+            const int x = x0 + threadIdx.x;
+            const bool valid = x < n;
+            const uint32_t v = valid ? (uint32_t)ci[x] : 0u;
+            const bool marked = valid && (v & DEFER_MARK) != 0u, plain = valid && !marked;
+            const unsigned long long bm = __ballot(marked), bp = __ballot(plain);
+            unsigned int pm = 0, pp = 0;
+            if (lane == 0) {
+                if (bm) pm = atomicAdd(&cur_sh[1], (unsigned int)__popcll(bm));
+                if (bp) pp = atomicAdd(&cur_sh[0], (unsigned int)__popcll(bp));
+            }
+            pm = __shfl(pm, 0);
+            pp = __shfl(pp, 0);
+            int i = (int)(v & ~DEFER_MARK);
+            if (a.perm && valid) i = a.perm_i0 + a.perm[i - a.perm_i0];
+            if (plain) {
+                const unsigned long long p = base + pp + lanes_below(bp);
+                key_j[p] = (uint32_t)(cj[x] + a.j0);
+                val_i[p] = (uint32_t)i;
+            } else if (marked && d_fits) {
+                const unsigned long long p = base_d + pm + lanes_below(bm);
+                a.d_i[p] = i;
+                a.d_j[p] = cj[x] + a.j0;
+            }
+        }
+        return;
+    }
     if (threadIdx.x == 0) base_sh = atomicAdd(n_out, (unsigned long long)n);
     __syncthreads();
     const unsigned long long base = base_sh;
@@ -184,13 +236,16 @@
 template <bool FRAG>
 __global__ __launch_bounds__(256) void f16_screen_kernel(ScreenArgs a) {
     if (*a.overflow) return;
-    __shared__ WavePairs wave_pairs[4];
+    __shared__ WavePairs wave_pairs[4], wave_defer[4];
     WavePairs& buf = wave_pairs[threadIdx.x >> 6];
-    int pend = 0;
+    WavePairs& dbuf = wave_defer[threadIdx.x >> 6];
+    int pend = 0, dpend = 0;
     const int lane = threadIdx.x & 63, g = lane & 3;
     const long long n_thr = (4 * a.n + 63) & ~63ll;
     const int npiece = a.dpadh / 8, nks = a.dpadh / 16;
     const float radius = a.row_thr ? 0.0f : *a.radius;
+    const float floor_v = !a.row_thr && a.floor ? *a.floor : INFINITY;
+    const bool defer_on = floor_v < INFINITY;
     const f16x8* __restrict__ Rp = reinterpret_cast<const f16x8*>(a.Rh);
     auto flush = [&]() {
         if (pend == 0) return;
@@ -204,6 +259,24 @@
         }
         asm volatile("s_waitcnt lgkmcnt(0)" ::: "memory");
         pend = 0;
+    };
+    auto flush_defer = [&]() {
+        if (dpend == 0) return;
+        asm volatile("s_waitcnt lgkmcnt(0)" ::: "memory");
+        unsigned long long base = 0;
+        if (lane == 0) {
+            base = atomicAdd(a.d_count, (unsigned long long)dpend);
+            atomicAdd(a.d_total, (unsigned long long)dpend);
+        }
+        base = __shfl(base, 0);
+        if ((long long)(base + dpend) > a.d_cap) {
+            if (lane == 0) atomicOr(a.overflow, 1);
+        } else if (lane < dpend) {
+            a.d_i[base + lane] = (int32_t)dbuf.i[lane];
+            a.d_j[base + lane] = (int32_t)dbuf.j[lane];
+        }
+        asm volatile("s_waitcnt lgkmcnt(0)" ::: "memory");
+        dpend = 0;
     };
     for (long long x = (long long)blockIdx.x * 256 + threadIdx.x; x < n_thr; x += (long long)gridDim.x * 256) {
         const long long c = x >> 2;
@@ -227,8 +300,21 @@
         acc += __shfl_xor(acc, 1);
         acc += __shfl_xor(acc, 2);
         const float eps = (a.c1 * a.qn[i] * a.rn[j] + a.c2 * (a.qn[i] + a.rn[j]) + a.c3) * 1.001f;
-        const bool pass = valid && g == 0 &&
-                          (!(eps < INFINITY) || (a.row_thr ? acc >= candidate_edge(a.row_thr[i], eps) : acc > candidate_edge(radius, eps)));
+        bool pass = valid && g == 0 &&
+                    (!(eps < INFINITY) || (a.row_thr ? acc >= candidate_edge(a.row_thr[i], eps) : acc > candidate_edge(radius, eps)));
+        if (defer_on) {
+            const float lo = (radius + eps) + 2.4e-7f * (fabsf(radius) + eps);
+            const bool defer = pass && acc > lo && acc <= candidate_edge(floor_v, eps);
+            pass = pass && !defer;
+            const unsigned long long md = __ballot(defer);
+            if (defer) {
+                const int p = dpend + __popcll(md & ((1ull << lane) - 1));
+                dbuf.i[p] = i;
+                dbuf.j[p] = j;
+            }
+            dpend += __popcll(md);
+            if (dpend > 48) flush_defer();
+        }
         const unsigned long long m = __ballot(pass);
         if (pass) {
             const int p = pend + __popcll(m & ((1ull << lane) - 1));
@@ -239,6 +325,7 @@
         if (pend > 48) flush();
     }
     flush();
+    flush_defer();
     if (blockIdx.x == 0 && threadIdx.x == 0) atomicAdd(a.n_cand_total, (unsigned long long)a.n);
 }
 
diff --git a/vsc2022_amd/csrc/select.hip b/vsc2022_amd/csrc/select.hip
--- a/vsc2022_amd/csrc/select.hip
+++ b/vsc2022_amd/csrc/select.hip
@@ -57,7 +57,8 @@
     if (lh[threadIdx.x]) atomicAdd(&c->hist[threadIdx.x], lh[threadIdx.x]);
 }
 
-__global__ void select_pick_kernel(SelectCtl* c, int shift) {
+enum { PICK_RADIUS = 0, PICK_TRIAL = 1, PICK_FLOOR = 2 };
+__global__ void select_pick_kernel(SelectCtl* c, int shift, int mode) {
     if (!c->active) return;
     __shared__ unsigned int h[256];
     h[threadIdx.x] = c->hist[threadIdx.x];
@@ -72,10 +73,58 @@
         c->rank = rank;
         c->prefix |= (unsigned int)d << shift;
         c->prefix_mask |= 255u << shift;
-        if (shift == 0) c->radius = key2f(c->prefix);
+        if (shift == 0) {
+            const float v = key2f(c->prefix);
+            if (mode == PICK_FLOOR) {
+                c->floor = v;
+            } else if (mode == PICK_TRIAL && c->n_d > 0 && !(v >= c->floor)) {
+                c->need_force = 1;
+            } else {
+                c->radius = v;
+                if (mode == PICK_TRIAL) {
+                    c->n_rethreshold += 1;
+                    c->ev_ok += c->n_d > 0 ? 1u : 0u;
+                    c->n_d = 0;
+                }
+                c->floor = INFINITY;
+            }
+        }
     }
     __syncthreads();
     c->hist[threadIdx.x] = 0;
+    if (shift == 0 && mode == PICK_TRIAL && threadIdx.x == 0 && c->need_force) c->active = 0;
+}
+
+__global__ void select_begin_defer_kernel(SelectCtl* c, unsigned long long max_results, unsigned long long min_results) {
+    if (threadIdx.x < 256) c->hist[threadIdx.x] = 0;
+    if (threadIdx.x == 0) {
+        const bool pred = !c->overflow && c->n + c->n_d > max_results;
+        const bool can = c->n > min_results;
+        c->active = pred && can ? 1 : 0;
+        c->need_force = pred && !can ? 1 : 0;
+        c->prefix = 0;
+        c->prefix_mask = 0;
+        c->rank = min_results;
+        c->n_tmp = 0;
+    }
+}
+
+__global__ void select_begin_floor_kernel(SelectCtl* c, unsigned long long rank) {
+    if (threadIdx.x < 256) c->hist[threadIdx.x] = 0;
+    if (threadIdx.x == 0) {
+        c->active = !c->overflow && c->n > rank ? 1 : 0;
+        c->floor = INFINITY;
+        c->prefix = 0;
+        c->prefix_mask = 0;
+        c->rank = rank;
+        c->n_tmp = 0;
+    }
+}
+
+__global__ void defer_reset_kernel(SelectCtl* c) {
+    c->n_d = 0;
+    c->need_force = 0;
+    c->floor = INFINITY;
 }
 
 __global__ __launch_bounds__(256) void select_compact_kernel(SelectCtl* c, const int32_t* ai,
@@ -152,7 +201,10 @@
     unsigned int* w = reinterpret_cast<unsigned int*>(c);
     for (unsigned x = threadIdx.x; x < sizeof(SelectCtl) / 4; x += blockDim.x) w[x] = 0u;
     __syncthreads();
-    if (threadIdx.x == 0) c->radius = radius;
+    if (threadIdx.x == 0) {
+        c->radius = radius;
+        c->floor = INFINITY;
+    }
 }
 int launch_ctl_init(SelectCtl* ctl, float radius, hipStream_t stream) {
     static_assert(sizeof(SelectCtl) % 4 == 0, "SelectCtl is cleared word by word");
@@ -166,11 +218,42 @@
     hipLaunchKernelGGL(select_begin_kernel, dim3(1), dim3(256), 0, stream, ctl, 2 * K, K);
     for (int shift = 24; shift >= 0; shift -= 8) {
         hipLaunchKernelGGL(select_hist_kernel, dim3(GRID), dim3(256), 0, stream, ctl, a.s, shift);
-        hipLaunchKernelGGL(select_pick_kernel, dim3(1), dim3(256), 0, stream, ctl, shift);
+        hipLaunchKernelGGL(select_pick_kernel, dim3(1), dim3(256), 0, stream, ctl, shift, (int)PICK_RADIUS);
     }
     hipLaunchKernelGGL(select_compact_kernel, dim3(GRID), dim3(256), 0, stream, ctl, a.i, a.j, a.s, b.i, b.j, b.s);
     hipLaunchKernelGGL(select_copyback_kernel, dim3(GRID), dim3(256), 0, stream, ctl, b.i, b.j, b.s, a.i, a.j, a.s);
     hipLaunchKernelGGL(select_end_kernel, dim3(1), dim3(1), 0, stream, ctl);
+    VSC_HIP(hipGetLastError());
+    return VSC_OK;
+}
+
+int enqueue_rethreshold_deferred(SelectCtl* ctl, HitView a, HitView b, unsigned long long K, hipStream_t stream) {
+    constexpr int GRID = 1024;
+    hipLaunchKernelGGL(select_begin_defer_kernel, dim3(1), dim3(256), 0, stream, ctl, 2 * K, K);
+    for (int shift = 24; shift >= 0; shift -= 8) {
+        hipLaunchKernelGGL(select_hist_kernel, dim3(GRID), dim3(256), 0, stream, ctl, a.s, shift);
+        hipLaunchKernelGGL(select_pick_kernel, dim3(1), dim3(256), 0, stream, ctl, shift, (int)PICK_TRIAL);
+    }
+    hipLaunchKernelGGL(select_compact_kernel, dim3(GRID), dim3(256), 0, stream, ctl, a.i, a.j, a.s, b.i, b.j, b.s);
+    hipLaunchKernelGGL(select_copyback_kernel, dim3(GRID), dim3(256), 0, stream, ctl, b.i, b.j, b.s, a.i, a.j, a.s);
+    hipLaunchKernelGGL(select_end_kernel, dim3(1), dim3(1), 0, stream, ctl);
+    VSC_HIP(hipGetLastError());
+    return VSC_OK;
+}
+
+int enqueue_floor_select(SelectCtl* ctl, const float* s, unsigned long long rank, hipStream_t stream) {
+    constexpr int GRID = 1024;
+    hipLaunchKernelGGL(select_begin_floor_kernel, dim3(1), dim3(256), 0, stream, ctl, rank);
+    for (int shift = 24; shift >= 0; shift -= 8) {
+        hipLaunchKernelGGL(select_hist_kernel, dim3(GRID), dim3(256), 0, stream, ctl, s, shift);
+        hipLaunchKernelGGL(select_pick_kernel, dim3(1), dim3(256), 0, stream, ctl, shift, (int)PICK_FLOOR);
+    }
+    VSC_HIP(hipGetLastError());
+    return VSC_OK;
+}
+
+int launch_defer_reset(SelectCtl* ctl, hipStream_t stream) {
+    hipLaunchKernelGGL(defer_reset_kernel, dim3(1), dim3(1), 0, stream, ctl);
     VSC_HIP(hipGetLastError());
     return VSC_OK;
 }
diff --git a/vsc2022_amd/csrc/sim_f16p.hip b/vsc2022_amd/csrc/sim_f16p.hip
--- a/vsc2022_amd/csrc/sim_f16p.hip
+++ b/vsc2022_amd/csrc/sim_f16p.hip
@@ -43,11 +43,18 @@
     }
 }
 
+__device__ __forceinline__ void defer_band(float radius, float floor_v, float thr, float& lo, float& hi) {
+    const float e = (radius - thr) * 1.000001f;
+    lo = (radius + e) + 2.4e-7f * (fabsf(radius) + e);
+    hi = candidate_edge(floor_v, e);
+}
+
 template <bool ROWTHR>
 __device__ __forceinline__ void emit_candidates(const SimF16PArgs& a, const bool (&all)[2], const float (&thr)[2],
                                                 const float (&eps)[2], const float* rt, const float (&rtmin)[4],
                                                 int row0, int col0, bool interior, const f32x16 (&acc)[4][2],
-                                                const float (&bm)[4][2], int64_t seg_base, int& count, TailExt* ext) {
+                                                const float (&bm)[4][2], int64_t seg_base, int& count, TailExt* ext,
+                                                float radius, float floor_v) {
 #pragma unroll
     for (int m = 0; m < 4; ++m)
 #pragma unroll
@@ -55,6 +62,8 @@
             const bool blk = all[n] || (ROWTHR ? bm[m][n] >= candidate_edge(rtmin[m], eps[n]) : bm[m][n] > thr[n]);
             if (!__any(blk)) continue;
             const int ln_blk = ROWTHR ? lane_now() : 0;
+            float dlo = INFINITY, dhi = -INFINITY;
+            if (!ROWTHR) defer_band(radius, floor_v, thr[n], dlo, dhi);
 #pragma unroll
             for (int r = 0; r < 16; ++r) {
                 const int rb = m * 32 + (r & 3) + 8 * (r >> 2);
@@ -77,7 +86,8 @@
                 if (!cand_reserve(a.list, seg_base, count, total, ln, ext, pos)) continue;
                 if (mine) {
                     pos += lanes_below(ok);
-                    a.list.i[pos] = a.i0 + i;
+                    const bool defer = !ROWTHR && acc[m][n][r] > dlo && acc[m][n][r] <= dhi;
+                    a.list.i[pos] = (a.i0 + i) | (defer ? (int)DEFER_MARK : 0);
                     a.list.j[pos] = j;
                 }
             }
@@ -86,7 +96,8 @@
 
 __device__ __forceinline__ void emit_candidates_seg(const SimF16PArgs& a, const float (&thr)[2], int row0, int col0,
                                                     const f32x16 (&acc)[4][2], const float (&bm)[4][2],
-                                                    __amdgpu_buffer_rsrc_t rs_i, __amdgpu_buffer_rsrc_t rs_j, int& count) {
+                                                    __amdgpu_buffer_rsrc_t rs_i, __amdgpu_buffer_rsrc_t rs_j, int& count,
+                                                    float radius, float floor_v) {
 #pragma unroll
     for (int m = 0; m < 4; ++m)
 #pragma unroll
@@ -95,6 +106,8 @@
             const int ln = lane_now();
             const int ibase = a.i0 + row0 + m * 32 + 4 * (ln >> 5);
             const int j = col0 + n * 32 + (ln & 31);
+            float dlo, dhi;
+            defer_band(radius, floor_v, thr[n], dlo, dhi);
 #pragma unroll
             for (int r = 0; r < 16; ++r) {
                 const bool cand = acc[m][n][r] > thr[n];
@@ -102,7 +115,8 @@
                 if (hits == 0ull) continue;
                 if (cand) {
                     const int off = (count + (int)lanes_below(hits)) << 2;
-                    __builtin_amdgcn_raw_buffer_store_b32(ibase + (r & 3) + 8 * (r >> 2), rs_i, off, 0, 0);
+                    const bool defer = acc[m][n][r] > dlo && acc[m][n][r] <= dhi;
+                    __builtin_amdgcn_raw_buffer_store_b32((ibase + (r & 3) + 8 * (r >> 2)) | (defer ? (int)DEFER_MARK : 0), rs_i, off, 0, 0);
                     __builtin_amdgcn_raw_buffer_store_b32(j, rs_j, off, 0, 0);
                 }
                 count += __popcll(hits);
@@ -133,6 +147,7 @@
         for (int u = 0; u < 8; ++u) abase[u] = rl * 256 + ((((2 * u) | hi) ^ r15) << 4);
     }
     const float radius = ROWTHR ? 0.0f : *a.radius;
+    const float floor_v = !ROWTHR && a.floor ? *a.floor : INFINITY;
     const int seg = blockIdx.x * 8 + wave;
     const int64_t seg_base = (int64_t)seg * a.list.seg_cap;
     int count = 0;
@@ -259,10 +274,10 @@
             if (__any(any_blk)) {
                 const bool interior = panel * PR + PR <= a.nq && col0 + 64 <= a.nr;
                 if (!ROWTHR && interior && !all[0] && !all[1] && count + 8192 <= a.list.seg_cap)
-                    emit_candidates_seg(a, thr, panel * PR, col0, acc, bm, rs_ci, rs_cj, count);
+                    emit_candidates_seg(a, thr, panel * PR, col0, acc, bm, rs_ci, rs_cj, count, radius, floor_v);
                 else
                     emit_candidates<ROWTHR>(a, all, thr, eps, rt_sh, rtmin, panel * PR, col0, interior, acc, bm,
-                                            seg_base, count, &tail_sh[wave]);
+                                            seg_base, count, &tail_sh[wave], radius, floor_v);
             }
         }
     }
diff --git a/vsc2022_amd/vsc/index.py b/vsc2022_amd/vsc/index.py
--- a/vsc2022_amd/vsc/index.py
+++ b/vsc2022_amd/vsc/index.py
@@ -311,6 +311,8 @@
         cand, hits = ctypes.c_int64(0), ctypes.c_int64(0)
         _lib.check(_lib.lib().vsc_index_search_stats(self._h, ctypes.byref(cand), ctypes.byref(hits)))
         out["candidates"] = cand.value
+        for name in ("deferred", "defer_forced", "defer_events_ok", "defer_events_forced"):
+            out[name] = int(self.get_option(name))
         return out
 
 
```

After: 20520 query-videos/s, median of 6. 1.02x the previous value.
